# WangFeng18/3d-gaussian-splatting

Measured on NVIDIA H100. Metric: render+backward FPS @1080p (2.4M Gaussians), higher is better.
Workload: dtype f32

## Files before the change

3d-gaussian-splatting_b200/csrc/bindings.cpp:

```cpp
#include <ATen/cuda/CUDAContext.h>
#include <c10/cuda/CUDACachingAllocator.h>
#include <c10/cuda/CUDAGuard.h>
#include <torch/extension.h>

#include <string>
#include <vector>

#include "../../include/gs_b200.h"

namespace gsb200 {

#define GS_CHECK_F32(x)                                                                         \
  TORCH_CHECK((x).is_cuda(), #x " must be a CUDA tensor");                                      \
  TORCH_CHECK((x).is_contiguous(), #x " must be contiguous");                                   \
  TORCH_CHECK((x).scalar_type() == at::kFloat, #x " must be float32")
#define GS_CHECK_I32(x)                                                                         \
  TORCH_CHECK((x).is_cuda(), #x " must be a CUDA tensor");                                      \
  TORCH_CHECK((x).is_contiguous(), #x " must be contiguous");                                   \
  TORCH_CHECK((x).scalar_type() == at::kInt, #x " must be int32")
#define GS_CHECK_I64(x)                                                                         \
  TORCH_CHECK((x).is_cuda(), #x " must be a CUDA tensor");                                      \
  TORCH_CHECK((x).is_contiguous(), #x " must be contiguous");                                   \
  TORCH_CHECK((x).scalar_type() == at::kLong, #x " must be int64")

// ... 463 lines not shown
      GS_CHECK_F32(*g_pos); GS_CHECK_F32(*g_rgb); GS_CHECK_F32(*g_opa); GS_CHECK_F32(*g_quat); GS_CHECK_F32(*g_scale);
      TORCH_CHECK(g_pos->numel() == pos.numel() && g_rgb->numel() == rgb.numel() && g_opa->numel() == opa.numel() &&
                      g_quat->numel() == quat.numel() && g_scale->numel() == scale.numel(),
                  "RenderContext.backward_cam_into: gradient buffers must match their parameters");
      TORCH_CHECK(reinterpret_cast<uintptr_t>(g_quat->data_ptr()) % 16 == 0, "grad_quat must be 16-byte aligned");
    }
    auto opt = [](std::optional<torch::Tensor>& t) { return t ? fpm(*t) : nullptr; };
    c10::cuda::CUDAGuard guard(pos.device());
    auto gi = grad_image.contiguous();
    torch::Tensor ga;
    if (grad_aux) ga = grad_aux->contiguous();
    check_rc(gs_render_backward_cam(ctx, fp(pos), fp(rgb), fp(opa), fp(quat), fp(scale), fp(raw), fp(gi),
                                    grad_is_final ? 1 : 0, aux ? fp(*aux) : nullptr, grad_aux ? fp(ga) : nullptr, opt(g_pos),
                                    opt(g_rgb), opt(g_opa), opt(g_quat), opt(g_scale), fpm(grad_cam), cur_stream()),
             "gs_render_backward_cam");
  }

  int64_t last_instances() { return (int64_t)gs_frame_instances(ctx); }

  py::dict stats() {
    gs_frame_info fi{};
    check_rc(gs_frame_stats(ctx, &fi, cur_stream()), "gs_frame_stats");
    py::dict d;
    d["n_gaussians"] = fi.n_gaussians;
    d["n_visible"] = fi.n_visible;
    d["n_instances"] = fi.n_instances;
    d["n_instances_eff"] = fi.n_instances_eff;
    d["width_padded"] = fi.width_padded;
    d["height_padded"] = fi.height_padded;
    d["n_tiles"] = fi.n_tiles;
    d["max_tile_count"] = fi.max_tile_count;
    d["n_instances_eff_bwd"] = fi.n_instances_eff_bwd;
    return d;
  }

  std::tuple<torch::Tensor, torch::Tensor> sorted_instances() {
    gs_frame_info fi{};
    check_rc(gs_frame_stats(ctx, &fi, cur_stream()), "gs_frame_stats");
    auto opts = torch::TensorOptions().device(torch::kCUDA, device).dtype(at::kInt);
    auto idx = torch::empty({(int64_t)fi.n_instances}, opts);
    auto accum = torch::empty({(int64_t)fi.n_tiles + 1}, opts);
    check_rc(gs_frame_sorted(ctx, idx.data_ptr<int>(), fi.n_instances, accum.data_ptr<int>(), cur_stream()),
             "gs_frame_sorted");
    return {idx, accum};
  }

  torch::Tensor tile_consumed() {
    gs_frame_info fi{};
    check_rc(gs_frame_stats(ctx, &fi, cur_stream()), "gs_frame_stats");
    auto out = torch::empty({(int64_t)fi.n_tiles}, torch::TensorOptions().device(torch::kCUDA, device).dtype(at::kInt));
    check_rc(gs_frame_tile_consumed(ctx, out.data_ptr<int>(), cur_stream()), "gs_frame_tile_consumed");
    return out;
  }
};

void adam_step(torch::Tensor param, torch::Tensor grad, torch::Tensor exp_avg, torch::Tensor exp_avg_sq,
               std::vector<int64_t> seg_ends, std::vector<double> lrs, double beta1, double beta2, double eps,
               int64_t step) {
  GS_CHECK_F32(param); GS_CHECK_F32(grad); GS_CHECK_F32(exp_avg); GS_CHECK_F32(exp_avg_sq);
  int64_t n = param.numel();
  TORCH_CHECK(grad.numel() == n && exp_avg.numel() == n && exp_avg_sq.numel() == n, "adam_step: size mismatch");
  TORCH_CHECK(seg_ends.size() == lrs.size() && !seg_ends.empty() && seg_ends.back() == n,
              "adam_step: segments must cover the flat buffer");
  for (auto* t : {&param, &grad, &exp_avg, &exp_avg_sq})
    TORCH_CHECK(reinterpret_cast<uintptr_t>(t->data_ptr()) % 16 == 0, "adam_step: buffers must be 16-byte aligned");
  std::vector<long long> ends(seg_ends.begin(), seg_ends.end());
  std::vector<float> lr(lrs.begin(), lrs.end());
  c10::cuda::CUDAGuard guard(param.device());
  check_rc(gs_adam_step(fpm(param), fp(grad), fpm(exp_avg), fpm(exp_avg_sq), n, ends.data(), lr.data(), (int)ends.size(),
                        (float)beta1, (float)beta2, (float)eps, (int)step, cur_stream()),
           "gs_adam_step");
}

std::tuple<torch::Tensor, torch::Tensor> loss_l1_ssim(torch::Tensor image, torch::Tensor target, double w_l1,
                                                      double w_ssim, double bias, bool want_grad) {
  GS_CHECK_F32(image);
  TORCH_CHECK(target.is_cuda() && target.is_contiguous() &&
                  (target.scalar_type() == at::kFloat || target.scalar_type() == at::kHalf),
              "loss_l1_ssim: target must be a contiguous float32 / float16 CUDA tensor");
  TORCH_CHECK(image.dim() == 3 && image.size(2) == 3 && target.sizes() == image.sizes(),
              "loss_l1_ssim: image and target must both be [H, W, 3]");
  TORCH_CHECK(image.size(0) > 10 && image.size(1) > 10, "loss_l1_ssim: the image must be larger than the 11x11 window");
  c10::cuda::CUDAGuard guard(image.device());
  const int h = (int)image.size(0), w = (int)image.size(1);
  auto ws = torch::empty({(int64_t)gs_loss_workspace_bytes(h, w)}, image.options().dtype(at::kByte));
  auto out3 = torch::empty({3}, image.options());
  torch::Tensor grad = want_grad ? torch::empty_like(image) : torch::Tensor();
  check_rc(gs_loss_l1_ssim(fp(image), target.data_ptr(), target.scalar_type() == at::kHalf ? 1 : 0, h, w, (float)w_l1,
                           (float)w_ssim, (float)bias, want_grad ? fpm(grad) : nullptr, fpm(out3), ws.data_ptr(),
                           (size_t)ws.numel(), cur_stream()),
           "gs_loss_l1_ssim");
  return {out3, grad};
}

std::tuple<std::vector<torch::Tensor>, std::vector<int64_t>> densify(
    torch::Tensor pos, torch::Tensor rgb, torch::Tensor opa, torch::Tensor quat, torch::Tensor scale, torch::Tensor grad,
    int scale_activation, double opa_logit_min, double delete_thresh, double grad_thresh, bool grad_agg_max, double tau,
    bool use_clone, bool use_split, double clone_dt, c10::optional<at::Generator> gen) {
  GS_CHECK_F32(pos); GS_CHECK_F32(rgb); GS_CHECK_F32(opa); GS_CHECK_F32(quat); GS_CHECK_F32(scale); GS_CHECK_F32(grad);
  const int64_t n = pos.size(0);
  TORCH_CHECK(pos.dim() == 2 && pos.size(1) == 3 && rgb.dim() == 2 && rgb.size(0) == n && opa.numel() == n &&
                  quat.numel() == 4 * n && scale.numel() == 3 * n && grad.numel() == 3 * n && n < (int64_t(1) << 31),
              "densify: bad shapes");
  c10::cuda::CUDAGuard guard(pos.device());
  auto bopt = pos.options().dtype(at::kByte);
  auto code = torch::empty({n + 1}, bopt);
// ... 76 lines not shown
      .def_readwrite("left", &TilesPy::left)
      .def_readwrite("right", &TilesPy::right);

  py::class_<Gaussian3dsPy>(m, "Gaussian3ds")
      .def(py::init<>())
      .def_readwrite("pos", &Gaussian3dsPy::pos)
      .def_readwrite("rgb", &Gaussian3dsPy::rgb)
      .def_readwrite("opa", &Gaussian3dsPy::opa)
      .def_readwrite("quat", &Gaussian3dsPy::quat)
      .def_readwrite("scale", &Gaussian3dsPy::scale)
      .def_readwrite("cov", &Gaussian3dsPy::cov);

  m.def("calc_tile_list", &calc_tile_list, "calc tile list (CUDA)");
  m.def("gather_gaussians", &gather_gaussians, "gather gaussian (CUDA)");
  m.def("draw", &draw, "draw (CUDA)");
  m.def("draw_backward", &draw_backward, "draw backward (CUDA)");
  m.def("global_culling", &global_culling, "global culling (CUDA)");
  m.def("global_culling_backward", &global_culling_backward, "global culling backward (CUDA)");

  py::class_<RenderContext>(m, "RenderContext")
      .def(py::init<>())
      .def("forward", &RenderContext::forward)
      .def("backward", &RenderContext::backward)
      .def("backward_into", &RenderContext::backward_into, py::arg("pos"), py::arg("rgb"), py::arg("opa"),
           py::arg("quat"), py::arg("scale"), py::arg("image"), py::arg("grad_image"), py::arg("g_pos"),
           py::arg("g_rgb"), py::arg("g_opa"), py::arg("g_quat"), py::arg("g_scale"), py::arg("expected_frame") = -1)
      .def("forward_final", &RenderContext::forward_final)
      .def("backward_final_into", &RenderContext::backward_final_into, py::arg("pos"), py::arg("rgb"),
           py::arg("opa"), py::arg("quat"), py::arg("scale"), py::arg("raw"), py::arg("grad_final"),
           py::arg("g_pos"), py::arg("g_rgb"), py::arg("g_opa"), py::arg("g_quat"), py::arg("g_scale"),
           py::arg("expected_frame") = -1)
      .def("forward_aux", &RenderContext::forward_aux, py::arg("pos"), py::arg("rgb"), py::arg("opa"), py::arg("quat"),
           py::arg("scale"), py::arg("width"), py::arg("height"), py::arg("fx"), py::arg("fy"), py::arg("rot"),
           py::arg("tran"), py::arg("near"), py::arg("thresh"), py::arg("scale_activation"),
           py::arg("background") = py::none(), py::arg("final") = true)
      .def("backward_aux_into", &RenderContext::backward_aux_into, py::arg("pos"), py::arg("rgb"), py::arg("opa"),
           py::arg("quat"), py::arg("scale"), py::arg("raw"), py::arg("grad_image"), py::arg("grad_is_final"),
           py::arg("aux"), py::arg("grad_aux"), py::arg("g_pos"), py::arg("g_rgb"), py::arg("g_opa"),
           py::arg("g_quat"), py::arg("g_scale"), py::arg("expected_frame") = -1)
      .def("backward_cam_into", &RenderContext::backward_cam_into, py::arg("pos"), py::arg("rgb"), py::arg("opa"),
           py::arg("quat"), py::arg("scale"), py::arg("raw"), py::arg("grad_image"), py::arg("grad_is_final"),
           py::arg("aux"), py::arg("grad_aux"), py::arg("g_pos"), py::arg("g_rgb"), py::arg("g_opa"),
           py::arg("g_quat"), py::arg("g_scale"), py::arg("grad_cam"), py::arg("expected_frame") = -1)
      .def("frame_id", &RenderContext::frame_id)
      .def("last_instances", &RenderContext::last_instances)
      .def("stats", &RenderContext::stats)
      .def("set_sh_eval", &RenderContext::set_sh_eval, py::arg("mode"))
      .def("set_filter2d", &RenderContext::set_filter2d, py::arg("mode"), py::arg("variance") = 0.3)
      .def("set_timing", &RenderContext::set_timing)
      .def("set_grad_push", &RenderContext::set_grad_push)
      .def("clear_grad_push", &RenderContext::clear_grad_push)
      .def("stage_ms", &RenderContext::stage_ms)
      .def("sorted_instances", &RenderContext::sorted_instances)
      .def("tile_consumed", &RenderContext::tile_consumed);
  m.def("allreduce_push_finish", &allreduce_push_finish, "second half of the pushed gradient exchange");
  m.def("allreduce_push_finish_mc", &allreduce_push_finish_mc,
        "second half of the pushed gradient exchange, broadcast through the NVSwitch (multimem.st)");
  m.def("allreduce_p2p", &allreduce_p2p, "peer-to-peer two-shot in-place all-reduce of a symmetric buffer");
  m.def("allreduce_multimem", &allreduce_multimem, "NVLS multimem in-place all-reduce of a symmetric buffer");
  m.def("densify", &densify, "prune / clone / split on the device (reference splatter.py:122-228)", py::arg("pos"),
        py::arg("rgb"), py::arg("opa"), py::arg("quat"), py::arg("scale"), py::arg("grad"), py::arg("scale_activation"),
        py::arg("opa_logit_min"), py::arg("delete_thresh"), py::arg("grad_thresh"), py::arg("grad_agg_max"), py::arg("tau"),
        py::arg("use_clone"), py::arg("use_split"), py::arg("clone_dt"), py::arg("generator") = py::none());
  m.def("loss_l1_ssim", &loss_l1_ssim, "fused L1 + SSIM loss, forward + image gradient (CUDA)");
  m.def("adam_step", &adam_step, "fused Adam over flat parameter / gradient buffers (CUDA)");
  m.def("tune", [](const std::string& name, int value) { check_rc(gs_tune(name.c_str(), value), "gs_tune"); },
        "set an A/B tuning knob of the blend kernels (see include/gs_b200.h gs_tune)");
  m.def("kernel_launches", []() { return (int64_t)gs_kernel_launches(); },
        "kernels of libgs_b200 launched by this process so far");
  m.attr("abi_version") = gs_abi_version();
  m.attr("SH_EVAL_PIXEL") = GS_SH_EVAL_PIXEL;
  m.attr("SH_EVAL_GAUSSIAN") = GS_SH_EVAL_GAUSSIAN;
  m.attr("FILTER2D_NONE") = GS_FILTER2D_NONE;
  m.attr("FILTER2D_DILATE") = GS_FILTER2D_DILATE;
  m.attr("FILTER2D_ANTIALIAS") = GS_FILTER2D_ANTIALIAS;
}
```

3d-gaussian-splatting_b200/csrc/binning.cu:

```cuda
#include "internal.h"

namespace {

constexpr int kBlock = 256;

__device__ __forceinline__ void append_to_tile(int* tile_n_point, int* list, int max_per_tile, uint32_t tid,
                                               uint32_t pid) {
  int old = atomicAdd(tile_n_point + tid, 1);
  if (old < max_per_tile) list[(size_t)max_per_tile * tid + old] = (int)pid;
}

__global__ void tile_list_dist_kernel(const float* __restrict__ pos, const float* __restrict__ top,
                                      const float* __restrict__ bottom, const float* __restrict__ left,
                                      const float* __restrict__ right, int* tile_n_point, int* list, uint32_t n,
                                      uint32_t n_tiles, int max_per_tile, float thresh) {
  uint32_t pid = blockDim.x * blockIdx.x + threadIdx.x;
  uint32_t tid = blockDim.y * blockIdx.y + threadIdx.y;
  if (pid >= n || tid >= n_tiles) return;
  float cy = (top[tid] + bottom[tid]) / 2;
  float cx = (left[tid] + right[tid]) / 2;
  float d1 = pos[3 * pid] - cx, d2 = pos[3 * pid + 1] - cy;
  if (d1 * d1 + d2 * d2 < thresh) append_to_tile(tile_n_point, list, max_per_tile, tid, pid);
}

// ... 132 lines not shown
  const long long t = (long long)blockIdx.x * kBlock + threadIdx.x;
  const long long i = t >> 3;
  const int sub = (int)(t & 7);
  if (i >= m) return;
  const uint32_t tile = keys[i];
  const uint32_t g = vals[i];
  if (sub == 0) {
    if (i == 0) {
      for (uint32_t tt = 0; tt <= tile; ++tt) tile_accum[tt] = 0;
    } else {
      uint32_t prev = keys[i - 1];
      for (uint32_t tt = prev + 1; tt <= tile; ++tt) tile_accum[tt] = (int)i;
    }
    if (i == m - 1)
      for (uint32_t tt = tile + 1; tt <= (uint32_t)n_tiles; ++tt) tile_accum[tt] = (int)m;
    const GsRec* r = rec + g;
    float4 a = r->a, b = r->b, c = r->c;
    uint32_t rxy = __float_as_uint(c.z), rwh = __float_as_uint(c.w);
    uint32_t tx = tile % ntx, ty = tile / ntx;
    uint32_t slot = offsets_g[g] + (ty - (rxy >> 16)) * (rwh & 0xffffu) + (tx - (rxy & 0xffffu));
    pA[i] = a;
    pB[i] = make_float2(b.x, b.y);
    pS[(size_t)i * sw + d] = __uint_as_float(slot);
  }
  float* row = pS + (size_t)i * sw;
  const float* src = rgb + (size_t)g * d;
  for (int q = sub; q < d; q += 8) row[q] = src[q];
}

template <typename KeyT>
__global__ void __launch_bounds__(kBlock) tile_ranges_kernel(const KeyT* __restrict__ keys, long long m, int n_tiles,
                                                              int* __restrict__ tile_accum) {
  const long long i0 = ((long long)blockIdx.x * kBlock + threadIdx.x) * 8;
  if (i0 >= m) return;
  uint32_t prev = i0 > 0 ? (uint32_t)keys[i0 - 1] : 0u;
  if (i0 == 0) tile_accum[0] = 0;
#pragma unroll
  for (int u = 0; u < 8; ++u) {
    const long long i = i0 + u;
    if (i >= m) break;
    const uint32_t tile = keys[i];
    for (uint32_t t = prev + 1; t <= tile; ++t) tile_accum[t] = (int)i;
    if (i == 0)
      for (uint32_t t = 1; t <= tile; ++t) tile_accum[t] = 0;
    prev = tile;
    if (i == m - 1)
      for (uint32_t t = tile + 1; t <= (uint32_t)n_tiles; ++t) tile_accum[t] = (int)m;
  }
}

__global__ void __launch_bounds__(kBlock) iota_kernel(uint32_t* out, int n) {
  int i = blockIdx.x * kBlock + threadIdx.x;
  if (i < n) out[i] = (uint32_t)i;
}

}

cudaError_t gs_launch_pack_sorted_sh(const void* keys, int key_bytes, const uint32_t* vals, long long m, int n_tiles,
                                     int ntx, const GsRec* rec, const uint32_t* offsets_g, const float* rgb, int d,
                                     int sw, float4* pA, float2* pB, float* pS, int* tile_accum, cudaStream_t st) {
  if (m == 0) return cudaMemsetAsync(tile_accum, 0, sizeof(int) * (size_t)(n_tiles + 1), st);
  const unsigned grid = (unsigned)((m * 8 + kBlock - 1) / kBlock);
  if (key_bytes == 2)
    pack_sorted_sh_kernel<uint16_t><<<grid, kBlock, 0, st>>>(static_cast<const uint16_t*>(keys), vals, m, n_tiles,
                                                             ntx, rec, offsets_g, rgb, d, sw, pA, pB, pS, tile_accum);
  else
    pack_sorted_sh_kernel<uint32_t><<<grid, kBlock, 0, st>>>(static_cast<const uint32_t*>(keys), vals, m, n_tiles,
                                                             ntx, rec, offsets_g, rgb, d, sw, pA, pB, pS, tile_accum);
  return cudaGetLastError();
}

cudaError_t gs_launch_iota(uint32_t* out, int n, cudaStream_t st) {
  if (n == 0) return cudaSuccess;
  iota_kernel<<<(n + kBlock - 1) / kBlock, kBlock, 0, st>>>(out, n);
  return cudaGetLastError();
}

extern "C" int gs_tile_list(const float* pos, const float* cov, int n, const float* tile_top,
                            const float* tile_bottom, const float* tile_left, const float* tile_right, int n_tiles,
                            int* tile_n_point, int* tile_gaussian_list, int max_per_tile, float thresh, int method,
                            float tile_length_x, float tile_length_y, int n_tiles_x, int n_tiles_y, float leftmost,
                            float topmost, gs_stream_t stream) {
  if (n < 0 || n_tiles < 0 || max_per_tile < 0) return gs_set_error_msg(GS_ERR_INVALID_ARG, "gs_tile_list: negative size");
  if (n == 0 || n_tiles == 0) return 0;
  cudaStream_t st = (cudaStream_t)stream;
  if (method == 0 || method == 1) {
    dim3 block(32, 8), grid((n + 31) / 32, (n_tiles + 7) / 8);
    if (grid.y > 65535) return gs_set_error_msg(GS_ERR_INVALID_ARG, "gs_tile_list: too many tiles for method 0/1");
    if (method == 0)
      tile_list_dist_kernel<<<grid, block, 0, st>>>(pos, tile_top, tile_bottom, tile_left, tile_right, tile_n_point,
                                                    tile_gaussian_list, n, n_tiles, max_per_tile, thresh);
    else
      tile_list_prob_kernel<<<grid, block, 0, st>>>(pos, cov, tile_top, tile_bottom, tile_left, tile_right,
                                                    tile_n_point, tile_gaussian_list, n, n_tiles, max_per_tile,
                                                    thresh);
  } else {
    GsTileGrid g;
    g.lx = tile_length_x;
    g.ly = tile_length_y;
    g.leftmost = leftmost;
    g.topmost = topmost;
    g.t2 = 0.f;
    g.ntx = n_tiles_x;
    g.nty = n_tiles_y;
    tile_list_prob2_kernel<<<(n + kBlock - 1) / kBlock, kBlock, 0, st>>>(pos, cov, g, tile_n_point,
                                                                        tile_gaussian_list, n, max_per_tile, thresh);
// ... 3 lines not shown
  return 0;
}

extern "C" int gs_gather(const int* tile_n_point_accum, const int* tile_gaussian_list, int n_tiles, int list_stride,
                         int max_points_for_tile, int* gathered_list, int* tile_ids_for_points,
                         gs_stream_t stream) {
  (void)max_points_for_tile;
  if (n_tiles < 0) return gs_set_error_msg(GS_ERR_INVALID_ARG, "gs_gather: n_tiles < 0");
  if (n_tiles == 0) return 0;
  int warps = kBlock / 32;
  gather_kernel<<<(n_tiles + warps - 1) / warps, kBlock, 0, (cudaStream_t)stream>>>(
      tile_n_point_accum, tile_gaussian_list, n_tiles, list_stride, gathered_list, tile_ids_for_points);
  GS_CUDA_TRY(cudaGetLastError());
  gs_count_launch();
  return 0;
}

cudaError_t gs_launch_emit_keys(const GsRec* rec, const uint32_t* perm, const uint32_t* offsets_sorted, int n, int ntx,
                                void* keys, int key_bytes, uint32_t* vals, cudaStream_t st) {
  if (n == 0) return cudaSuccess;
  if (key_bytes == 2)
    emit_keys_kernel<uint16_t><<<(n + kBlock - 1) / kBlock, kBlock, 0, st>>>(rec, perm, offsets_sorted, n, ntx,
                                                                             static_cast<uint16_t*>(keys), vals);
  else
    emit_keys_kernel<uint32_t><<<(n + kBlock - 1) / kBlock, kBlock, 0, st>>>(rec, perm, offsets_sorted, n, ntx,
                                                                             static_cast<uint32_t*>(keys), vals);
  return cudaGetLastError();
}

cudaError_t gs_launch_tile_ranges(const void* keys, int key_bytes, long long m, int n_tiles, int* tile_accum,
                                  cudaStream_t st) {
  if (m == 0) return cudaMemsetAsync(tile_accum, 0, sizeof(int) * (size_t)(n_tiles + 1), st);
  const unsigned grid = (unsigned)((m + 8LL * kBlock - 1) / (8LL * kBlock));
  if (key_bytes == 2)
    tile_ranges_kernel<uint16_t><<<grid, kBlock, 0, st>>>(static_cast<const uint16_t*>(keys), m, n_tiles, tile_accum);
  else
    tile_ranges_kernel<uint32_t><<<grid, kBlock, 0, st>>>(static_cast<const uint32_t*>(keys), m, n_tiles, tile_accum);
  return cudaGetLastError();
}

cudaError_t gs_launch_pack_sorted(const void* keys, int key_bytes, const uint32_t* vals, long long m, int n_tiles,
                                  int ntx, const GsRec* rec, const uint32_t* offsets_g, float4* pA, float2* pB,
                                  float4* pC, int* tile_accum, cudaStream_t st) {
  if (m == 0) return cudaMemsetAsync(tile_accum, 0, sizeof(int) * (size_t)(n_tiles + 1), st);
  const unsigned grid = (unsigned)((m + kBlock - 1) / kBlock);
  if (key_bytes == 2)
    pack_sorted_kernel<uint16_t><<<grid, kBlock, 0, st>>>(static_cast<const uint16_t*>(keys), vals, m, n_tiles, ntx,
                                                          rec, offsets_g, pA, pB, pC, tile_accum);
  else
    pack_sorted_kernel<uint32_t><<<grid, kBlock, 0, st>>>(static_cast<const uint32_t*>(keys), vals, m, n_tiles, ntx,
                                                          rec, offsets_g, pA, pB, pC, tile_accum);
  return cudaGetLastError();
}
```

3d-gaussian-splatting_b200/csrc/blend.cu:

```cuda
#include <cstdlib>
#include <type_traits>

#include "internal.h"

namespace {

constexpr int FWD_THREADS = 64;
constexpr int FWD_PX = 4;
constexpr int FWD_STAGES = 2;

template <int FWD_CH>
struct FwdSmem {
  float4 A[FWD_STAGES][FWD_CH];
  float4 C[FWD_STAGES][FWD_CH];
  float2 B[FWD_STAGES][FWD_CH + 2];
  uint64_t full[FWD_STAGES];
};

template <typename SM, int CH>
__device__ __forceinline__ void issue_chunk(SM& sm, int stage, const float4* __restrict__ pA,
                                            const float2* __restrict__ pB, const float4* __restrict__ pC,
                                            int base, int n, int shift) {
  uint32_t bytes_a = (uint32_t)n * 16u;
  uint32_t nb = (uint32_t)(n + shift + 1) & ~1u;
// ... 37 lines not shown
    return off + ((uint32_t)ty - (rxy >> 16)) * (rwh & 0xffffu) + ((uint32_t)tx - (rxy & 0xffffu));
  }
};

template <int CH, int STAGES, int RECW>
struct GatherRing {
  float4 rec[STAGES][CH * RECW];
  uint64_t full[STAGES];
};

template <int NT, int CH>
struct GatherIds {
  uint32_t id[(CH + NT - 1) / NT];
  __device__ __forceinline__ void load(const uint32_t* __restrict__ ids, int base, int n, int tid) {
#pragma unroll
    for (int u = 0; u < (CH + NT - 1) / NT; ++u) {
      const int i = tid + u * NT;
      id[u] = i < n ? __ldg(ids + base + i) : 0u;
    }
  }
};

template <typename SM, int NT, int CH, int RECW>
__device__ __forceinline__ void gather_issue(SM& sm, int stage, const GsRec* __restrict__ grec,
                                             const uint32_t* __restrict__ goff, const GatherIds<NT, CH>& g, int n,
                                             int tid) {
#pragma unroll
  for (int u = 0; u < (CH + NT - 1) / NT; ++u) {
    const int i = tid + u * NT;
    if (i < n) {
      const float4* src = reinterpret_cast<const float4*>(grec + g.id[u]);
      const uint32_t dst = gs_smem_u32(&sm.rec[stage][i * RECW]);
#pragma unroll
      for (int q = 0; q < 3; ++q)
        asm volatile("cp.async.cg.shared.global [%0], [%1], 16;" ::"r"(dst + 16u * q), "l"(src + q) : "memory");
      if (RECW == 4)
        asm volatile("cp.async.ca.shared.global [%0], [%1], 4;" ::"r"(dst + 48u), "l"(goff + g.id[u]) : "memory");
    }
  }
  asm volatile("cp.async.mbarrier.arrive.noinc.shared::cta.b64 [%0];" ::"r"(gs_smem_u32(&sm.full[stage])) : "memory");
}

template <int FWD_CH, int PX, bool GATHER, bool AUX = false>
__global__ void __launch_bounds__(256 / PX) blend_fwd_kernel(const float4* __restrict__ pA,
                                                                 const float2* __restrict__ pB,
                                                                 const float4* __restrict__ pC,
                                                                 const GsRec* __restrict__ grec,
                                                                 const uint32_t* __restrict__ ids,
                                                                 const int* __restrict__ tile_accum, int wp, int hp,
                                                                 int ntx, float fx, float fy,
                                                                 float* __restrict__ image,
                                                                 int* __restrict__ tile_neff,
                                                                 float* __restrict__ final_img, GsCrop crop,
                                                                 GsAuxOut aux) {
  static_assert(!AUX || GATHER, "the aux outputs read |p_c| from the gathered records");
  using Smem = typename std::conditional<GATHER, GatherRing<FWD_CH, FWD_STAGES, 3>, FwdSmem<FWD_CH>>::type;
  __shared__ __align__(16) Smem sm;
  const int tile = blockIdx.x;
  const int tid = threadIdx.x;
  const int tx = tile % ntx, ty = tile / ntx;
  constexpr int FWD_PX = PX, TPR = GS_TILE / PX, NTHREADS = 256 / PX;
  const int ix0 = tx * GS_TILE + (tid % TPR) * FWD_PX;
  const int iy = ty * GS_TILE + (tid / TPR);
  float px[FWD_PX];
#pragma unroll
  for (int p = 0; p < FWD_PX; ++p) px[p] = gs_pixel_coord(ix0 + p, wp, fx);
  const float py = gs_pixel_coord(iy, hp, fy);

  const int start = tile_accum[tile];
  const int cnt = tile_accum[tile + 1] - start;
  const int shift = start & 1;
  const int nchunks = (cnt + FWD_CH - 1) / FWD_CH;

  if (tid == 0) {
    for (int s = 0; s < FWD_STAGES; ++s) gs_mbar_init(&sm.full[s], GATHER ? NTHREADS : 1);
    gs_fence_barrier_init();
  }
  __syncthreads();
  GatherIds<NTHREADS, FWD_CH> gid;
  if constexpr (GATHER) {
    for (int k = 0; k < FWD_STAGES && k < nchunks; ++k) {
      gid.load(ids, start + k * FWD_CH, min(FWD_CH, cnt - k * FWD_CH), tid);
      gather_issue<Smem, NTHREADS, FWD_CH, 3>(sm, k, grec, nullptr, gid, min(FWD_CH, cnt - k * FWD_CH), tid);
    }
    if (FWD_STAGES < nchunks) gid.load(ids, start + FWD_STAGES * FWD_CH, min(FWD_CH, cnt - FWD_STAGES * FWD_CH), tid);
  } else if (tid == 0) {
    for (int k = 0; k < FWD_STAGES && k < nchunks; ++k)
      issue_chunk<Smem, FWD_CH>(sm, k, pA, pB, pC, start + k * FWD_CH, min(FWD_CH, cnt - k * FWD_CH), shift);
  }

  float T[FWD_PX], cr[FWD_PX], cg[FWD_PX], cb[FWD_PX], dep[FWD_PX];
#pragma unroll
  for (int p = 0; p < FWD_PX; ++p) {
    T[p] = 1.f;
    cr[p] = cg[p] = cb[p] = 0.f;
    dep[p] = 0.f;
  }
  int consumed = cnt;
  int k = 0;
  for (; k < nchunks; ++k) {
    const int stage = k % FWD_STAGES;
    gs_mbar_wait(&sm.full[stage], (uint32_t)((k / FWD_STAGES) & 1));
    const int n = min(FWD_CH, cnt - k * FWD_CH);
    StageView<GATHER> sv;
    if constexpr (GATHER) {
      sv.R = sm.rec[stage];
      sv.recw = 3;
    } else {
      sv.A = sm.A[stage];
      sv.C = sm.C[stage];
      sv.B = sm.B[stage] + shift;
// ... 79 lines not shown
      for (int q = 0; q < FWD_PX / 2; ++q) o[q] = make_float4(ab[4 * q], ab[4 * q + 1], ab[4 * q + 2], ab[4 * q + 3]);
    }
    if (aux.aux_final) {
#pragma unroll
      for (int p = 0; p < FWD_PX; ++p) {
        const int x = ix0 + p - crop.left, y = iy - crop.top;
        if (x >= 0 && x < crop.width && y >= 0 && y < crop.height)
          *reinterpret_cast<float2*>(aux.aux_final + ((size_t)y * crop.width + x) * 2) = make_float2(ab[2 * p], ab[2 * p + 1]);
      }
    }
  }
  {
    float ob[FWD_PX * 3];
#pragma unroll
    for (int p = 0; p < FWD_PX; ++p) {
      ob[3 * p] = cr[p];
      ob[3 * p + 1] = cg[p];
      ob[3 * p + 2] = cb[p];
    }
    float4* o = reinterpret_cast<float4*>(image + ((size_t)iy * wp + ix0) * 3);
#pragma unroll
    for (int q = 0; q < FWD_PX * 3 / 4; ++q) o[q] = make_float4(ob[4 * q], ob[4 * q + 1], ob[4 * q + 2], ob[4 * q + 3]);
  }
  if (final_img) {
#pragma unroll
    for (int p = 0; p < FWD_PX; ++p)
      gs_store_final(final_img, ix0 + p, iy, crop.left, crop.top, crop.width, crop.height, cr[p], cg[p], cb[p]);
  }
  if (tile_neff && tid == 0) tile_neff[tile] = consumed;
}

constexpr int BWD_STAGES = 2;
constexpr int BWD_NV = 9;

template <int WARPS, int BWD_CH>
struct BwdSmem {
  float4 A[BWD_STAGES][BWD_CH];
  float4 C[BWD_STAGES][BWD_CH];
  float2 B[BWD_STAGES][BWD_CH + 2];
  uint64_t full[BWD_STAGES];
  float partial[WARPS][BWD_CH * BWD_NV];
};

template <int WARPS, int BWD_CH>
__global__ void __launch_bounds__(32 * WARPS) blend_bwd_kernel(const float4* __restrict__ pA,
                                                                const float2* __restrict__ pB,
                                                                const float4* __restrict__ pC,
                                                                const int* __restrict__ tile_accum, int wp, int hp,
                                                                int ntx, float fx, float fy,
                                                                const float* __restrict__ image,
                                                                const float* __restrict__ grad_image,
                                                                float* __restrict__ grad_inst, int grad_is_final,
                                                                GsCrop crop, uint32_t* __restrict__ row_epoch,
                                                                uint32_t epoch, int* __restrict__ tile_neff_b) {
  constexpr int THREADS = 32 * WARPS;
  constexpr int PX = 256 / THREADS;
  constexpr int TPR = GS_TILE / PX;
  using Smem = BwdSmem<WARPS, BWD_CH>;
  __shared__ __align__(16) Smem sm;
  const int tile = blockIdx.x;
  const int tid = threadIdx.x, warp = tid >> 5, lane = tid & 31;
  const int tx = tile % ntx, ty = tile / ntx;
  const int start = tile_accum[tile];
  const int cnt = tile_accum[tile + 1] - start;
  if (cnt == 0) return;
  const int shift = start & 1;
  const int nchunks = (cnt + BWD_CH - 1) / BWD_CH;

  const int ix0 = tx * GS_TILE + (tid % TPR) * PX;
  const int iy = ty * GS_TILE + (tid / TPR);
  float px[PX];
#pragma unroll
  for (int p = 0; p < PX; ++p) px[p] = gs_pixel_coord(ix0 + p, wp, fx);
  const float py = gs_pixel_coord(iy, hp, fy);

  float T[PX], R[PX], gr[PX], gg[PX], gb[PX];
  {
    const size_t off = ((size_t)iy * wp + ix0) * 3;
    const float4* im = reinterpret_cast<const float4*>(image + off);
    float gbuf[PX * 3], ibuf[PX * 3];
#pragma unroll
    for (int q = 0; q < PX * 3 / 4; ++q) {
      const float4 i4 = im[q];
      ibuf[4 * q] = i4.x; ibuf[4 * q + 1] = i4.y; ibuf[4 * q + 2] = i4.z; ibuf[4 * q + 3] = i4.w;
    }
    if (!grad_is_final) {
      const float4* gi = reinterpret_cast<const float4*>(grad_image + off);
#pragma unroll
      for (int q = 0; q < PX * 3 / 4; ++q) {
        const float4 g4 = gi[q];
        gbuf[4 * q] = g4.x; gbuf[4 * q + 1] = g4.y; gbuf[4 * q + 2] = g4.z; gbuf[4 * q + 3] = g4.w;
      }
    } else {
#pragma unroll
      for (int p = 0; p < PX; ++p)
        gs_load_final_grad(grad_image, ibuf + 3 * p, ix0 + p, iy, crop.left, crop.top, crop.width, crop.height,
                           gbuf[3 * p], gbuf[3 * p + 1], gbuf[3 * p + 2]);
    }
#pragma unroll
    for (int p = 0; p < PX; ++p) {
      gr[p] = gbuf[3 * p];
      gg[p] = gbuf[3 * p + 1];
      gb[p] = gbuf[3 * p + 2];
      R[p] = gr[p] * ibuf[3 * p] + gg[p] * ibuf[3 * p + 1] + gb[p] * ibuf[3 * p + 2];
      T[p] = 1.f;
    }
  }

  if (tid == 0) {
    for (int s = 0; s < BWD_STAGES; ++s) gs_mbar_init(&sm.full[s], 1);
    gs_fence_barrier_init();
  }
  __syncthreads();
// ... 141 lines not shown
}

constexpr int WS_CH = 64;

template <int STAGES>
struct WsRing {
  float4 A[STAGES][WS_CH];
  float4 C[STAGES][WS_CH];
  float2 B[STAGES][WS_CH + 2];
  uint64_t full[STAGES], empty[STAGES], done;
  volatile int stop, consumed_chunks;
};

template <typename SM, int STAGES>
__device__ __forceinline__ void ws_init(SM& sm, int tid) {
  if (tid == 0) {
    for (int s = 0; s < STAGES; ++s) {
      gs_mbar_init(&sm.full[s], 1);
      gs_mbar_init(&sm.empty[s], 1);
    }
    gs_mbar_init(&sm.done, 1);
    sm.stop = 0;
    sm.consumed_chunks = 0;
    gs_fence_barrier_init();
  }
  __syncthreads();
}

template <typename SM, int STAGES>
__device__ __forceinline__ void ws_producer(SM& sm, const float4* __restrict__ pA, const float2* __restrict__ pB,
                                            const float4* __restrict__ pC, int start, int cnt, int nchunks) {
  const int shift = start & 1;
  int k = 0;
  for (; k < nchunks; ++k) {
    const int s = k % STAGES;
    if (k >= STAGES) gs_mbar_wait(&sm.empty[s], (uint32_t)(((k / STAGES) - 1) & 1));
    if (sm.stop) break;
    issue_chunk<SM, WS_CH>(sm, s, pA, pB, pC, start + k * WS_CH, min(WS_CH, cnt - k * WS_CH), shift);
  }
  gs_mbar_wait(&sm.done, 0u);
  for (int kk = sm.consumed_chunks; kk < k; ++kk) gs_mbar_wait(&sm.full[kk % STAGES], (uint32_t)((kk / STAGES) & 1));
}

constexpr int WSF_STAGES = 4;
constexpr int WSF_CONS = 64;

__global__ void __launch_bounds__(WSF_CONS + 32) blend_fwd_ws_kernel(const float4* __restrict__ pA,
                                                                      const float2* __restrict__ pB,
                                                                      const float4* __restrict__ pC,
                                                                      const int* __restrict__ tile_accum, int wp,
                                                                      int hp, int ntx, float fx, float fy,
                                                                      float* __restrict__ image,
                                                                      int* __restrict__ tile_neff,
                                                                      float* __restrict__ final_img, GsCrop crop) {
  using Smem = WsRing<WSF_STAGES>;
  __shared__ __align__(16) Smem sm;
  const int tile = blockIdx.x;
  const int tid = threadIdx.x;
  const int start = tile_accum[tile];
  const int cnt = tile_accum[tile + 1] - start;
  const int nchunks = (cnt + WS_CH - 1) / WS_CH;
  ws_init<Smem, WSF_STAGES>(sm, tid);
  if (tid >= WSF_CONS) {
    if (tid == WSF_CONS && nchunks > 0) ws_producer<Smem, WSF_STAGES>(sm, pA, pB, pC, start, cnt, nchunks);
    return;
  }
  const int tx = tile % ntx, ty = tile / ntx;
  const int ix0 = tx * GS_TILE + (tid & 3) * FWD_PX;
  const int iy = ty * GS_TILE + (tid >> 2);
  float px[FWD_PX];
#pragma unroll
  for (int p = 0; p < FWD_PX; ++p) px[p] = gs_pixel_coord(ix0 + p, wp, fx);
  const float py = gs_pixel_coord(iy, hp, fy);
  const int shift = start & 1;

  float T[FWD_PX], cr[FWD_PX], cg[FWD_PX], cb[FWD_PX];
#pragma unroll
  for (int p = 0; p < FWD_PX; ++p) {
    T[p] = 1.f;
    cr[p] = cg[p] = cb[p] = 0.f;
  }
  int consumed = cnt;
  for (int k = 0; k < nchunks; ++k) {
    const int stage = k % WSF_STAGES;
    gs_mbar_wait(&sm.full[stage], (uint32_t)((k / WSF_STAGES) & 1));
    const int n = min(WS_CH, cnt - k * WS_CH);
    const float4* __restrict__ sA = sm.A[stage];
    const float4* __restrict__ sC = sm.C[stage];
    const float2* __restrict__ sB = sm.B[stage] + shift;
#define GS_FWD_BODY(J)                                                                      \
  {                                                                                         \
    const float4 a = sA[J];                                                                 \
    const float2 b = sB[J];                                                                 \
    const float4 c = sC[J];                                                                 \
    const float dy = py - a.y;                                                              \
    const float m1 = a.w * dy;                                                              \
    const float ev = fmaf(-b.x * dy, dy, b.y);                                              \
    _Pragma("unroll") for (int p = 0; p < FWD_PX; ++p) {                                    \
      const float dx = px[p] - a.x;                                                         \
      const float eu = fmaf(a.z, dx, -m1);                                                  \
      const float alpha = gs_ex2(fmaf(-dx, eu, ev));                                        \
      const float w = (T[p] > GS_T_STOP) ? alpha * T[p] : 0.f;                              \
      cr[p] = fmaf(c.x, w, cr[p]);                                                          \
      cg[p] = fmaf(c.y, w, cg[p]);                                                          \
      cb[p] = fmaf(c.z, w, cb[p]);                                                          \
      T[p] -= w;                                                                            \
    }                                                                                       \
  }
    int j = 0;
    bool warp_dead = false;
// ... 160 lines not shown
    }
  lsrc[lane] = 0;
  lcnt[lane] = 0;
  lrow[lane] = GS_TILE;
  lpy[lane] = 0.f;
  const int nl = (live + ns - 1) / ns;
  int sc = (nl << 16) | live;
#pragma unroll
  for (int o = 1; o < 32; o <<= 1) {
    const int t = __shfl_up_sync(0xffffffffu, sc, o);
    if (lane >= o) sc += t;
  }
  sc -= (nl << 16) | live;
  __syncwarp();
  for (int q = 0; q < nl; ++q) {
    const int l = (sc >> 16) + q;
    lsrc[l] = (sc & 0xffff) + q * ns;
    lcnt[l] = min(ns, live - q * ns);
    lrow[l] = lane;
    lpy[l] = pyt[lane];
  }
  __syncwarp();
  const int src = lsrc[lane], n = lcnt[lane];
  prow = lrow[lane];
  py = lpy[lane];
#pragma unroll
  for (int p = 0; p < PX; ++p) {
    const bool v = p < n;
    px[p] = v ? st[src + p] : 0.f;
    T[p] = v ? st[256 + src + p] : 0.f;
    Rr[p] = v ? st[512 + src + p] : 0.f;
    gr[p] = v ? st[768 + src + p] : 0.f;
    gg[p] = v ? st[1024 + src + p] : 0.f;
    gb[p] = v ? st[1280 + src + p] : 0.f;
    if constexpr (AUX) {
      gD[p] = v ? st[1536 + src + p] : 0.f;
      gA[p] = v ? st[1792 + src + p] : 0.f;
    }
  }
  __syncwarp();
  st[bwd_lane_y<SQ, QS>(lane)] = py;
  S = ns;
}

template <int PX, bool WS, int UNR, int STAGES, int MINB, int RQ, bool GATHER, int CH, bool AUX = false,
          bool REPACK = false>
__global__ void __launch_bounds__(256 / PX + (WS ? 32 : 0), MINB)
    blend_bwd2_kernel(const float4* __restrict__ pA, const float2* __restrict__ pB, const float4* __restrict__ pC,
                      const GsRec* __restrict__ grec, const uint32_t* __restrict__ ids,
                      const uint32_t* __restrict__ goff, const int* __restrict__ tile_accum, int wp, int hp, int ntx, float fx, float fy,
                      const float* __restrict__ image, const float* __restrict__ grad_image,
                      float* __restrict__ grad_inst, int grad_is_final, GsCrop crop, uint32_t* __restrict__ row_epoch,
                      uint32_t epoch, int* __restrict__ tile_neff_b, const float* __restrict__ aux,
                      const float* __restrict__ grad_aux) {
  using Cfg = Bwd2Cfg<PX, STAGES, RQ>;
  constexpr int NT = Cfg::NT, TPR = Cfg::TPR, R = Cfg::R, SQ = Cfg::SQ, QS = Cfg::QS, IS = Cfg::IS, ROWS = Cfg::ROWS;
  static_assert(IS % 2 == 0 && QS % 2 == 0 && IS % 32 == 2 && QS % 32 == 32 / RQ, "partial buffer strides");
  static_assert(!(WS && GATHER), "the gather path issues its copies from all consumer threads");
  static_assert(GATHER || CH == WS_CH, "the packed ring is sized for CH instances per stage");
  static_assert(!AUX || GATHER, "the aux terms read |p_c| from the gathered records");
  static_assert(!REPACK || (NT == 32 && PX == 8), "the repack deals one warp's 256 pixels into slots of at most 8");
  static_assert(!REPACK || R * IS >= RP_END, "the partial buffer holds the repack's planes and tables");
  using Smem = typename std::conditional<AUX, Bwd2SmemAux<PX, STAGES, RQ, GATHER, CH>,
                                         Bwd2Smem<PX, STAGES, RQ, GATHER, CH>>::type;
  __shared__ __align__(16) Smem sm;
  const int tile = blockIdx.x;
  const int tid = threadIdx.x, warp = tid >> 5, lane = tid & 31;
  const int start = tile_accum[tile];
  const int cnt = tile_accum[tile + 1] - start;
  if (cnt == 0) return;
  const int nchunks = (cnt + CH - 1) / CH;
  const int tx = tile % ntx, ty = tile / ntx;
  const int shift = start & 1;
  if (tid < GS_TILE) sm.pyt[tid] = gs_pixel_coord(ty * GS_TILE + tid, hp, fy);
  if constexpr (GATHER) {
    if (tid == 0) {
      for (int s = 0; s < STAGES; ++s) gs_mbar_init(&sm.full[s], NT);
      gs_fence_barrier_init();
    }
    __syncthreads();
  } else {
    ws_init<Smem, STAGES>(sm, tid);
    if (WS) {
      if (tid >= NT) {
        if (tid == NT) ws_producer<Smem, STAGES>(sm, pA, pB, pC, start, cnt, nchunks);
        return;
      }
    } else if (tid == 0) {
      for (int k = 0; k < STAGES && k < nchunks; ++k)
        issue_chunk<Smem, CH>(sm, k, pA, pB, pC, start + k * CH, min(CH, cnt - k * CH), shift);
    }
  }
  GatherIds<NT, CH> gid;
  if constexpr (GATHER) {
    for (int k = 0; k < STAGES && k < nchunks; ++k) {
      gid.load(ids, start + k * CH, min(CH, cnt - k * CH), tid);
      gather_issue<Smem, NT, CH, 4>(sm, k, grec, goff, gid, min(CH, cnt - k * CH), tid);
    }
    if (STAGES < nchunks) gid.load(ids, start + STAGES * CH, min(CH, cnt - STAGES * CH), tid);
  }
  const int ix0 = tx * GS_TILE + (tid % TPR) * PX;
  const int iy = ty * GS_TILE + (tid / TPR);
  float px[PX];
#pragma unroll
  for (int p = 0; p < PX; ++p) px[p] = gs_pixel_coord(ix0 + p, wp, fx);
  float py = sm.pyt[tid / TPR];
  int S = PX, prow = tid / TPR;

  float T[PX], Rr[PX], gr[PX], gg[PX], gb[PX];
  {
    const size_t off = ((size_t)iy * wp + ix0) * 3;
    const float4* im = reinterpret_cast<const float4*>(image + off);
    float gbuf[PX * 3], ibuf[PX * 3];
#pragma unroll
    for (int q = 0; q < PX * 3 / 4; ++q) {
      const float4 i4 = im[q];
      ibuf[4 * q] = i4.x; ibuf[4 * q + 1] = i4.y; ibuf[4 * q + 2] = i4.z; ibuf[4 * q + 3] = i4.w;
    }
    if (!grad_is_final) {
// ... 332 lines not shown
  int i = blockIdx.x * 256 + threadIdx.x;
  if (i >= m) return;
  const float* row = grad_inst + (size_t)i * gw;
  float4 cv = reinterpret_cast<const float4*>(cov)[i];
  float det = cv.x * cv.w - cv.y * cv.z;
  double pn = 2.0 * (double)det + 1e-14;
  float sc = (float)((double)GS_LOG2E / pn);
  float kk = 2.f * sc * sc / GS_LOG2E;
  float d_ca = row[2], d_cb = row[3], d_cc = row[4];
  float gsc = d_ca * cv.w + d_cb * (cv.y + cv.z) + d_cc * cv.x;
  g_pos[3 * i] = row[0];
  g_pos[3 * i + 1] = row[1];
  reinterpret_cast<float4*>(g_cov)[i] = make_float4(d_cc * sc - gsc * kk * cv.w, d_cb * sc + gsc * kk * cv.z,
                                                    d_cb * sc + gsc * kk * cv.y, d_ca * sc - gsc * kk * cv.x);
  g_opa[i] = opa[i] > 0.f ? row[5] / (opa[i] * GS_LN2) : 0.f;
  for (int q = 0; q < d; ++q) g_rgb[(size_t)i * d + q] = row[6 + q];
}

struct LegacyWs {
  float4* pA;
  float2* pB;
  float4* pC;
  float* grad_inst;
};

inline size_t align_up(size_t x, size_t a) { return (x + a - 1) / a * a; }

inline size_t legacy_ws_layout(int m, int d, LegacyWs* ws, char* base) {
  size_t off = 0;
  size_t mm = (size_t)(m > 0 ? m : 0);
  size_t crow = d == 3 ? 16 : (size_t)gs_sh_stream_width(d) * 4;
  size_t grow = d == 3 ? (size_t)GS_GREC * 4 : (size_t)gs_sh_grad_width(d) * 4;
  if (ws) ws->pA = reinterpret_cast<float4*>(base + off);
  off += align_up(mm * 16, 256);
  if (ws) ws->pC = reinterpret_cast<float4*>(base + off);
  off += align_up(mm * crow + 16, 256);
  if (ws) ws->pB = reinterpret_cast<float2*>(base + off);
  off += align_up((mm + 2) * 8, 256);
  if (ws) ws->grad_inst = reinterpret_cast<float*>(base + off);
  off += align_up(mm * grow, 256);
  return off;
}

}

cudaError_t gs_launch_blend_fwd(const float4* pA, const float2* pB, const float4* pC, const GsRec* grec,
                                const uint32_t* ids, const int* tile_accum, const GsFrameGeom& g, float* image,
                                int* tile_neff, float* final_img, const GsCrop& crop, cudaStream_t st,
                                const GsAuxOut* aux) {
  const GsTuning& tn = gs_tuning();
  const bool gather = grec != nullptr;
  if (aux) {
    blend_fwd_kernel<128, 4, true, true><<<g.n_tiles, 64, 0, st>>>(pA, pB, pC, grec, ids, tile_accum, g.wp, g.hp, g.ntx,
                                                                  g.fx, g.fy, image, tile_neff, final_img, crop, *aux);
    return cudaGetLastError();
  }
  if (!gather && tn.fwd_kernel != 0) {
    blend_fwd_ws_kernel<<<g.n_tiles, WSF_CONS + 32, 0, st>>>(pA, pB, pC, tile_accum, g.wp, g.hp, g.ntx, g.fx, g.fy, image,
                                                             tile_neff, final_img, crop);
    return cudaGetLastError();
  }
  const int ch = tn.fwd_ch;
#define GS_FWD_LAUNCH(CH, PX, GA)                                                                                   \
  blend_fwd_kernel<CH, PX, GA><<<g.n_tiles, 256 / PX, 0, st>>>(pA, pB, pC, grec, ids, tile_accum, g.wp, g.hp, g.ntx, \
                                                               g.fx, g.fy, image, tile_neff, final_img, crop, GsAuxOut{})
#define GS_FWD_CH(PX, GA)                     \
  if (ch == 64) GS_FWD_LAUNCH(64, PX, GA);    \
  else if (ch == 256) GS_FWD_LAUNCH(256, PX, GA); \
  else GS_FWD_LAUNCH(128, PX, GA)
  if (gather) {
    if (tn.fwd_px == 8) { GS_FWD_CH(8, true); } else { GS_FWD_CH(4, true); }
  } else {
    if (tn.fwd_px == 8) { GS_FWD_CH(8, false); } else { GS_FWD_CH(4, false); }
  }
#undef GS_FWD_CH
#undef GS_FWD_LAUNCH
  return cudaGetLastError();
}

cudaError_t gs_launch_blend_bwd(const float4* pA, const float2* pB, const float4* pC, const GsRec* grec,
                                const uint32_t* ids, const uint32_t* goff, const int* tile_accum, const GsFrameGeom& g,
                                const float* image,
                                const float* grad_image, float* grad_inst, int grad_is_final, const GsCrop& crop,
                                uint32_t* row_epoch, uint32_t epoch, int* tile_neff_b, cudaStream_t st,
                                const float* aux, const float* grad_aux) {
  const GsTuning& tn = gs_tuning();
  const bool gather = grec != nullptr;
  if (gather && !row_epoch) return cudaErrorInvalidValue;
  if (grad_aux) {
    if (!gather || !aux) return cudaErrorInvalidValue;
#define GS_BWD2_AUX(RP)                                                                                            \
  blend_bwd2_kernel<8, false, 4, 3, 10, 4, true, 32, true, RP><<<g.n_tiles, 32, 0, st>>>(                           \
      pA, pB, pC, grec, ids, goff, tile_accum, g.wp, g.hp, g.ntx, g.fx, g.fy, image, grad_image, grad_inst,         \
      grad_is_final, crop, row_epoch, epoch, tile_neff_b, aux, grad_aux)
    if (tn.blend_repack) GS_BWD2_AUX(true);
    else GS_BWD2_AUX(false);
#undef GS_BWD2_AUX
    return cudaGetLastError();
  }
  if (tn.bwd_kernel != 0 || gather) {
#define GS_BWD2C(PX, WS, UNR, ST, MINB, RQ, GA, CH)                                                                 \
  blend_bwd2_kernel<PX, WS, UNR, ST, MINB, RQ, GA, CH><<<g.n_tiles, 256 / PX + (WS ? 32 : 0), 0, st>>>(              \
      pA, pB, pC, grec, ids, goff, tile_accum, g.wp, g.hp, g.ntx, g.fx, g.fy, image, grad_image, grad_inst,          \
      grad_is_final,                                                                                                 \
      crop, row_epoch, epoch, tile_neff_b, nullptr, nullptr)
#define GS_BWD2(PX, WS, UNR, ST, MINB, RQ, GA) GS_BWD2C(PX, WS, UNR, ST, MINB, RQ, GA, 64)
    const int key = ((((tn.bwd_px * 10 + tn.bwd_ws) * 10 + tn.bwd_unroll) * 10 + tn.bwd_stages) * 10 + tn.bwd_rq) * 100 +
                    tn.bwd_minb;
    if (gather && tn.bwd_ch == 32) {
#define GS_BWD2_SHIPPED()                                                                                          \
  if (tn.blend_repack)                                                                                             \
    blend_bwd2_kernel<8, false, 4, 3, 10, 4, true, 32, false, true><<<g.n_tiles, 32, 0, st>>>(                      \
        pA, pB, pC, grec, ids, goff, tile_accum, g.wp, g.hp, g.ntx, g.fx, g.fy, image, grad_image, grad_inst,       \
        grad_is_final, crop, row_epoch, epoch, tile_neff_b, nullptr, nullptr);                                     \
  else                                                                                                             \
    GS_BWD2C(8, false, 4, 3, 10, 4, true, 32)
      switch (key) {
        case 8022416: GS_BWD2C(8, false, 2, 2, 16, 4, true, 32); break;
        case 8023416: GS_BWD2C(8, false, 2, 3, 16, 4, true, 32); break;
        case 8042410: GS_BWD2C(8, false, 4, 2, 10, 4, true, 32); break;
        case 8043410: GS_BWD2_SHIPPED(); break;
        default:
          if (gs_tuning().strict) return cudaErrorInvalidValue;
          GS_BWD2_SHIPPED();
          break;
      }
#undef GS_BWD2_SHIPPED
      return cudaGetLastError();
    }
    if (gather) {
      switch (key) {
        case 8012410: GS_BWD2(8, false, 1, 2, 10, 4, true); break;
        case 8022416: GS_BWD2(8, false, 2, 2, 16, 4, true); break;
        case 8022410: GS_BWD2(8, false, 2, 2, 10, 4, true); break;
        case 8042410: GS_BWD2(8, false, 4, 2, 10, 4, true); break;
        case 8023416: GS_BWD2(8, false, 2, 3, 16, 4, true); break;
        case 8012416: GS_BWD2(8, false, 1, 2, 16, 4, true); break;
        case 8012420: GS_BWD2(8, false, 1, 2, 20, 4, true); break;
        case 8012820: GS_BWD2(8, false, 1, 2, 20, 8, true); break;
        case 8013416: GS_BWD2(8, false, 1, 3, 16, 4, true); break;
        case 4012401: GS_BWD2(4, false, 1, 2, 1, 4, true); break;
        case 4042401: GS_BWD2(4, false, 4, 2, 1, 4, true); break;
        default: return gs_tuning().strict ? cudaErrorInvalidValue : (GS_BWD2(8, false, 2, 2, 16, 4, true), cudaGetLastError());
      }
      return cudaGetLastError();
    }
    switch (key) {
      case 4113401: GS_BWD2(4, true, 1, 3, 1, 4, false); break;
      case 4143408: GS_BWD2(4, true, 4, 3, 8, 4, false); break;
      case 4012401: GS_BWD2(4, false, 1, 2, 1, 4, false); break;
      case 4042401: GS_BWD2(4, false, 4, 2, 1, 4, false); break;
      case 4042810: GS_BWD2(4, false, 4, 2, 10, 8, false); break;
      case 8012410: GS_BWD2(8, false, 1, 2, 10, 4, false); break;
      case 8012416: GS_BWD2(8, false, 1, 2, 16, 4, false); break;
      case 8012420: GS_BWD2(8, false, 1, 2, 20, 4, false); break;
      case 8013416: GS_BWD2(8, false, 1, 3, 16, 4, false); break;
      case 8022416: GS_BWD2(8, false, 2, 2, 16, 4, false); break;
      case 8022410: GS_BWD2(8, false, 2, 2, 10, 4, false); break;
      case 8042410: GS_BWD2(8, false, 4, 2, 10, 4, false); break;
      case 8012816: GS_BWD2(8, false, 1, 2, 16, 8, false); break;
      case 8012820: GS_BWD2(8, false, 1, 2, 20, 8, false); break;
      case 8112410: GS_BWD2(8, true, 1, 2, 10, 4, false); break;
      case 8012424: GS_BWD2(8, false, 1, 2, 24, 4, false); break;
      case 8012824: GS_BWD2(8, false, 1, 2, 24, 8, false); break;
      default: return gs_tuning().strict ? cudaErrorInvalidValue : (GS_BWD2(8, false, 2, 2, 16, 4, false), cudaGetLastError());
    }
#undef GS_BWD2
#undef GS_BWD2C
    return cudaGetLastError();
  }
  const int warps = tn.bwd_px == 8 ? 1 : 2;
  const int ch = 64;
#define GS_BWD_LAUNCH(W, CH)                                                                                         \
  blend_bwd_kernel<W, CH><<<g.n_tiles, 32 * W, 0, st>>>(pA, pB, pC, tile_accum, g.wp, g.hp, g.ntx, g.fx, g.fy, image, \
                                                        grad_image, grad_inst, grad_is_final, crop, row_epoch, epoch, \
                                                        tile_neff_b)
  if (warps == 1) GS_BWD_LAUNCH(1, 64);
  else if (ch == 32) GS_BWD_LAUNCH(2, 32);
  else if (ch == 128) GS_BWD_LAUNCH(2, 128);
  else GS_BWD_LAUNCH(2, 64);
#undef GS_BWD_LAUNCH
  return cudaGetLastError();
}

int gs_blend_aux_supported(int d, bool forward, bool backward) {
  const GsTuning& tn = gs_tuning();
  if (!tn.gather)
    return gs_set_error_msg(GS_ERR_UNSUPPORTED, "depth / alpha / background: the packed path (gs_tune(\"gather\", 0)) has no aux kernel");
  if (d != 3) {
    if (backward && (gs_sh_tc_mode(d) & 6) == 6)
      return gs_set_error_msg(GS_ERR_UNSUPPORTED,
                              "depth / alpha gradients: the two-pixel tensor-core SH backward (sh_tc bit 2) has no aux kernel");
    return 0;
  }
  if (forward && (tn.fwd_kernel != 0 || tn.fwd_ch != 128 || tn.fwd_px != 4))
    return gs_set_error_msg(GS_ERR_UNSUPPORTED,
                            "depth / alpha / background: only the shipped forward blend knobs (fwd_kernel 0, fwd_ch 128, fwd_px 4) have an aux kernel");
  if (backward && (tn.bwd_kernel == 0 || tn.bwd_px != 8 || tn.bwd_ws != 0 || tn.bwd_unroll != 4 || tn.bwd_stages != 3 ||
                   tn.bwd_rq != 4 || tn.bwd_minb != 10 || tn.bwd_ch != 32))
    return gs_set_error_msg(GS_ERR_UNSUPPORTED,
                            "depth / alpha gradients: only the shipped backward blend knobs have an aux kernel");
  return 0;
}

extern "C" size_t gs_draw_workspace_bytes(int m, int d) {
  if (d != 3 && gs_sh_basis_count(d) == 0) return 0;
  return legacy_ws_layout(m, d, nullptr, nullptr);
}

static int check_draw_args(const char* fn, int m, int d, int wp, int hp, int weight_normalize, int sigmoid,
                           size_t ws_bytes, void* ws) {
  if (m < 0 || wp <= 0 || hp <= 0 || (wp % GS_TILE) || (hp % GS_TILE))
    return gs_set_error_msg(GS_ERR_INVALID_ARG, fn);
  if (weight_normalize || sigmoid || (d != 3 && gs_sh_basis_count(d) == 0)) return gs_set_error_msg(GS_ERR_UNSUPPORTED, fn);
  if (m > 0 && (ws == nullptr || ws_bytes < gs_draw_workspace_bytes(m, d)))
    return gs_set_error_msg(GS_ERR_INVALID_ARG, fn);
  return 0;
}

extern "C" int gs_draw_fwd(const float* pos, const float* rgb, const float* opa, const float* cov,
                           const int* tile_n_point_accum, int m, int d, int width_padded, int height_padded,
                           float focal_x, float focal_y, int weight_normalize, int sigmoid, const float* rays_o,
                           const float* lefttop, const float* vec_dx, const float* vec_dy, float* image,
                           void* workspace, size_t workspace_bytes, gs_stream_t stream) {
  int rc = check_draw_args("gs_draw_fwd: bad/unsupported arguments", m, d, width_padded, height_padded,
                           weight_normalize, sigmoid, workspace_bytes, workspace);
  if (rc) return rc;
  if (d != 3 && (!rays_o || !lefttop || !vec_dx || !vec_dy))
    return gs_set_error_msg(GS_ERR_INVALID_ARG, "gs_draw_fwd: SH colour needs rays_o / lefttop / vec_dx / vec_dy");
// ... 83 lines not shown
```

3d-gaussian-splatting_b200/csrc/blend_sh.cu:

```cuda
#include <type_traits>

#include "internal.h"
#include "sh_common.cuh"

namespace {

using namespace gs_sh;

template <int K, int CH, int STAGES>
struct ShStage {
  float4 A[STAGES][CH];
  float2 B[STAGES][CH + 2];
  float S[STAGES][CH * sh_sw(K)];
  uint64_t full[STAGES];
};

template <int K, typename SM>
__device__ __forceinline__ void issue_sh(SM& sm, int stage, const float4* __restrict__ pA,
                                         const float2* __restrict__ pB, const float* __restrict__ pS, int base,
                                         int n, int shift) {
  const uint32_t bytes_a = (uint32_t)n * 16u;
  const uint32_t bytes_s = (uint32_t)n * (uint32_t)(sh_sw(K) * 4);
  const uint32_t nb = (uint32_t)(n + shift + 1) & ~1u;
  const uint32_t bytes_b = nb * 8u;
// ... 30 lines not shown
      for (int q = 0; q < D / 4; ++q)
        asm volatile("cp.async.cg.shared.global [%0], [%1], 16;" ::"r"(ds + 16u * q), "l"(src + 4 * q) : "memory");
    } else {
#pragma unroll
      for (int q = 0; q < D; ++q)
        asm volatile("cp.async.ca.shared.global [%0], [%1], 4;" ::"r"(ds + 4u * q), "l"(src + q) : "memory");
    }
  }
  asm volatile("cp.async.mbarrier.arrive.noinc.shared::cta.b64 [%0];" ::"r"(gs_smem_u32(&sm.full[stage])) : "memory");
}

template <int K, bool GATHER>
struct ShView;
template <int K>
struct ShView<K, false> {
  const float4* A;
  const float2* B;
  const float* S;
  __device__ __forceinline__ float4 a(int j) const { return A[j]; }
  __device__ __forceinline__ float2 b(int j) const { return B[j]; }
  __device__ __forceinline__ const float* coef(int j) const { return S + j * sh_sw(K); }
  __device__ __forceinline__ uint32_t slot(int j, int, int) const { return __float_as_uint(S[j * sh_sw(K) + 3 * K]); }
};
template <int K>
struct ShView<K, true> {
  const float4* R;
  const float* S;
  __device__ __forceinline__ float4 a(int j) const { return R[4 * j]; }
  __device__ __forceinline__ float2 b(int j) const {
    const float4 t = R[4 * j + 1];
    return make_float2(t.x, t.y);
  }
  __device__ __forceinline__ const float* coef(int j) const { return S + j * sh_sw(K); }
  __device__ __forceinline__ float depth(int j) const { return R[4 * j + 2].y; }
  __device__ __forceinline__ uint32_t slot(int j, int tx, int ty) const {
    const float4 cc = R[4 * j + 2];
    const uint32_t rxy = __float_as_uint(cc.z), rwh = __float_as_uint(cc.w);
    return __float_as_uint(R[4 * j + 3].x) + ((uint32_t)ty - (rxy >> 16)) * (rwh & 0xffffu) + ((uint32_t)tx - (rxy & 0xffffu));
  }
};

template <int K, bool GATHER, bool AUX = false>
__global__ void __launch_bounds__(64) blend_sh_fwd_kernel(const float4* __restrict__ pA, const float2* __restrict__ pB,
                                                           const float* __restrict__ pS,
                                                           const GsRec* __restrict__ grec, const float* __restrict__ rgb,
                                                           const uint32_t* __restrict__ ids,
                                                           const uint32_t* __restrict__ goff,
                                                           const int* __restrict__ tile_accum, int wp, int hp, int ntx,
                                                           float fx, float fy, const float* __restrict__ rays_o,
                                                           const float* __restrict__ lefttop,
                                                           const float* __restrict__ vdx,
                                                           const float* __restrict__ vdy, float* __restrict__ image,
                                                           int* __restrict__ tile_neff,
                                                           float* __restrict__ final_img, GsCrop crop, GsAuxOut aux) {
  constexpr int CH = 64, STAGES = 2, PX = 4, SW = sh_sw(K), NT = 64;
  static_assert(!AUX || GATHER, "the aux outputs read |p_c| from the gathered records");
  using SM = typename std::conditional<GATHER, ShGatherStage<K, CH, STAGES>, ShStage<K, CH, STAGES>>::type;
  __shared__ __align__(16) SM sm;
  const int tile = blockIdx.x, tid = threadIdx.x;
  const int tx = tile % ntx, ty = tile / ntx;
  const int ix0 = tx * GS_TILE + (tid & 3) * PX;
  const int iy = ty * GS_TILE + (tid >> 2);
  float px[PX], sh[PX][K];
#pragma unroll
  for (int p = 0; p < PX; ++p) {
    px[p] = gs_pixel_coord(ix0 + p, wp, fx);
    pixel_sh<K>(ix0 + p, iy, rays_o, lefttop, vdx, vdy, sh[p]);
  }
  const float py = gs_pixel_coord(iy, hp, fy);
  const int start = tile_accum[tile];
  const int cnt = tile_accum[tile + 1] - start;
  const int shift = start & 1;
  const int nchunks = (cnt + CH - 1) / CH;
  if (tid == 0) {
    for (int s = 0; s < STAGES; ++s) gs_mbar_init(&sm.full[s], GATHER ? NT : 1);
    gs_fence_barrier_init();
  }
  __syncthreads();
  if constexpr (GATHER) {
    for (int k = 0; k < STAGES && k < nchunks; ++k)
      issue_sh_gather<K, NT>(sm, k, grec, rgb, ids, goff, start + k * CH, min(CH, cnt - k * CH), tid);
  } else if (tid == 0) {
    for (int k = 0; k < STAGES && k < nchunks; ++k)
      issue_sh<K>(sm, k, pA, pB, pS, start + k * CH, min(CH, cnt - k * CH), shift);
  }

  float T[PX], cr[PX], cg[PX], cb[PX], dep[PX];
#pragma unroll
  for (int p = 0; p < PX; ++p) {
    T[p] = 1.f;
    cr[p] = cg[p] = cb[p] = 0.f;
    dep[p] = 0.f;
  }
  int consumed = cnt, k = 0;
  for (; k < nchunks; ++k) {
    const int stage = k % STAGES;
    gs_mbar_wait(&sm.full[stage], (uint32_t)((k / STAGES) & 1));
    const int n = min(CH, cnt - k * CH);
    ShView<K, GATHER> sv;
    if constexpr (GATHER) {
      sv.R = sm.R[stage];
    } else {
      sv.A = sm.A[stage];
      sv.B = sm.B[stage] + shift;
    }
    sv.S = sm.S[stage];
    for (int j = 0; j < n; ++j) {
      if ((j & 3) == 0) {
        const bool dead = !(T[0] > GS_T_STOP) && !(T[1] > GS_T_STOP) && !(T[2] > GS_T_STOP) && !(T[3] > GS_T_STOP);
        if (__all_sync(0xffffffffu, dead)) break;
      }
      const float4 a = sv.a(j);
// ... 57 lines not shown
      if constexpr (GATHER)
        issue_sh_gather<K, NT>(sm, stage, grec, rgb, ids, goff, start + kn * CH, min(CH, cnt - kn * CH), tid);
      else if (tid == 0)
        issue_sh<K>(sm, stage, pA, pB, pS, start + kn * CH, min(CH, cnt - kn * CH), shift);
    }
  }
  if (tid == 0 && k < nchunks)
    for (int kk = k + 1; kk < nchunks && kk < k + STAGES; ++kk)
      gs_mbar_wait(&sm.full[kk % STAGES], (uint32_t)((kk / STAGES) & 1));
  if constexpr (AUX) {
#pragma unroll
    for (int p = 0; p < PX; ++p) {
      cr[p] = fmaf(T[p], aux.bg[0], cr[p]);
      cg[p] = fmaf(T[p], aux.bg[1], cg[p]);
      cb[p] = fmaf(T[p], aux.bg[2], cb[p]);
      gs_store_aux(aux, ix0 + p, iy, wp, crop, dep[p], 1.f - T[p]);
    }
  }
  float4* o = reinterpret_cast<float4*>(image + ((size_t)iy * wp + ix0) * 3);
  o[0] = make_float4(cr[0], cg[0], cb[0], cr[1]);
  o[1] = make_float4(cg[1], cb[1], cr[2], cg[2]);
  o[2] = make_float4(cb[2], cr[3], cg[3], cb[3]);
  if (final_img) {
#pragma unroll
    for (int p = 0; p < PX; ++p)
      gs_store_final(final_img, ix0 + p, iy, crop.left, crop.top, crop.width, crop.height, cr[p], cg[p], cb[p]);
  }
  if (tile_neff && tid == 0) tile_neff[tile] = consumed;
}

template <int K, bool GATHER>
struct ShBwdSmem {
  typename std::conditional<GATHER, ShGatherStage<K, 32, 2>, ShStage<K, 32, 2>>::type st;
  float partial[2][32 * sh_nvp(K)];
};

template <int K, bool GATHER, bool AUX = false>
__global__ void __launch_bounds__(64) blend_sh_bwd_kernel(const float4* __restrict__ pA, const float2* __restrict__ pB,
                                                           const float* __restrict__ pS,
                                                           const GsRec* __restrict__ grec, const float* __restrict__ rgb,
                                                           const uint32_t* __restrict__ ids,
                                                           const uint32_t* __restrict__ goff,
                                                           const int* __restrict__ tile_accum, int wp, int hp, int ntx,
                                                           float fx, float fy, const float* __restrict__ rays_o,
                                                           const float* __restrict__ lefttop,
                                                           const float* __restrict__ vdx,
                                                           const float* __restrict__ vdy,
                                                           const float* __restrict__ image,
                                                           const float* __restrict__ grad_image,
                                                           float* __restrict__ grad_inst, int grad_is_final,
                                                           GsCrop crop, uint32_t* __restrict__ row_epoch,
                                                           uint32_t epoch, int* __restrict__ tile_neff_b,
                                                           const float* __restrict__ aux,
                                                           const float* __restrict__ grad_aux) {
  constexpr int CH = 32, STAGES = 2, PX = 4, SW = sh_sw(K), NV = sh_nv(K), NVP = sh_nvp(K), THREADS = 64;
  constexpr int GREC = (NV + 3) / 4 * 4;
  static_assert(!AUX || (GATHER && NV < NVP && NV < GREC), "d_t needs a pad slot in the partial and gradient rows");
  __shared__ __align__(16) ShBwdSmem<K, GATHER> smem;
  auto& sm = smem.st;
  const int tile = blockIdx.x, tid = threadIdx.x, warp = tid >> 5, lane = tid & 31;
  const int tx = tile % ntx, ty = tile / ntx;
  const int start = tile_accum[tile];
  const int cnt = tile_accum[tile + 1] - start;
  if (cnt == 0) return;
  const int shift = start & 1;
  const int nchunks = (cnt + CH - 1) / CH;
  const int ix0 = tx * GS_TILE + (tid & 3) * PX;
  const int iy = ty * GS_TILE + (tid >> 2);
  float px[PX], sh[PX][K];
#pragma unroll
  for (int p = 0; p < PX; ++p) {
    px[p] = gs_pixel_coord(ix0 + p, wp, fx);
    pixel_sh<K>(ix0 + p, iy, rays_o, lefttop, vdx, vdy, sh[p]);
  }
  const float py = gs_pixel_coord(iy, hp, fy);
  float T[PX], R[PX], gr[PX], gg[PX], gb[PX];
  {
    const size_t off = ((size_t)iy * wp + ix0) * 3;
    const float4* im = reinterpret_cast<const float4*>(image + off);
    const float4 i0 = im[0], i1 = im[1], i2 = im[2];
    if (!grad_is_final) {
      const float4* gi = reinterpret_cast<const float4*>(grad_image + off);
      const float4 g0 = gi[0], g1 = gi[1], g2 = gi[2];
      gr[0] = g0.x; gg[0] = g0.y; gb[0] = g0.z; gr[1] = g0.w;
      gg[1] = g1.x; gb[1] = g1.y; gr[2] = g1.z; gg[2] = g1.w;
      gb[2] = g2.x; gr[3] = g2.y; gg[3] = g2.z; gb[3] = g2.w;
    } else {
      const float raw[12] = {i0.x, i0.y, i0.z, i0.w, i1.x, i1.y, i1.z, i1.w, i2.x, i2.y, i2.z, i2.w};
#pragma unroll
      for (int p = 0; p < PX; ++p)
        gs_load_final_grad(grad_image, raw + 3 * p, ix0 + p, iy, crop.left, crop.top, crop.width, crop.height, gr[p],
                           gg[p], gb[p]);
    }
    R[0] = gr[0] * i0.x + gg[0] * i0.y + gb[0] * i0.z;
    R[1] = gr[1] * i0.w + gg[1] * i1.x + gb[1] * i1.y;
    R[2] = gr[2] * i1.z + gg[2] * i1.w + gb[2] * i2.x;
    R[3] = gr[3] * i2.y + gg[3] * i2.z + gb[3] * i2.w;
#pragma unroll
    for (int p = 0; p < PX; ++p) T[p] = 1.f;
  }
  float gD[PX], gA[PX];
  if constexpr (AUX) gs_load_aux_grad<PX>(aux, grad_aux, grad_is_final, ix0, iy, wp, crop, gD, gA, R);
  if (tid == 0) {
    for (int s = 0; s < STAGES; ++s) gs_mbar_init(&sm.full[s], GATHER ? THREADS : 1);
    gs_fence_barrier_init();
  }
  __syncthreads();
  if constexpr (GATHER) {
    for (int k = 0; k < STAGES && k < nchunks; ++k)
      issue_sh_gather<K, THREADS>(sm, k, grec, rgb, ids, goff, start + k * CH, min(CH, cnt - k * CH), tid);
  } else if (tid == 0) {
    for (int k = 0; k < STAGES && k < nchunks; ++k)
      issue_sh<K>(sm, k, pA, pB, pS, start + k * CH, min(CH, cnt - k * CH), shift);
// ... 107 lines not shown
      out[0] = GS_LN2 * (2.f * a.z * s[0] - a.w * s[1]);
      out[1] = GS_LN2 * (2.f * b.x * s[1] - a.w * s[0]);
      out[2] = -GS_LN2 * s[2];
      out[3] = GS_LN2 * s[3];
      out[4] = -GS_LN2 * s[4];
      out[5] = GS_LN2 * s[5];
      for (int u = 6; u < NV; ++u) out[u] = p0[u] + p1[u];
      if constexpr (AUX) out[NV] = p0[NV] + p1[NV];
      if (row_epoch) row_epoch[slot] = epoch;
    }
    const bool dead = !(T[0] > GS_T_STOP) && !(T[1] > GS_T_STOP) && !(T[2] > GS_T_STOP) && !(T[3] > GS_T_STOP);
    if (__syncthreads_and(dead)) {
      consumed = min(cnt, (k + 1) * CH);
      break;
    }
    if (k + STAGES < nchunks) {
      const int kn = k + STAGES;
      if constexpr (GATHER)
        issue_sh_gather<K, THREADS>(sm, stage, grec, rgb, ids, goff, start + kn * CH, min(CH, cnt - kn * CH), tid);
      else if (tid == 0)
        issue_sh<K>(sm, stage, pA, pB, pS, start + kn * CH, min(CH, cnt - kn * CH), shift);
    }
  }
  if (tid == 0 && k < nchunks)
    for (int kk = k + 1; kk < nchunks && kk < k + STAGES; ++kk)
      gs_mbar_wait(&sm.full[kk % STAGES], (uint32_t)((kk / STAGES) & 1));
  if (tile_neff_b && tid == 0) tile_neff_b[tile] = consumed;
  if (row_epoch || GATHER) return;
  for (int t = consumed + tid; t < cnt; t += THREADS) {
    const uint32_t slot = __float_as_uint(pS[(size_t)(start + t) * SW + 3 * K]);
    float* out = grad_inst + (size_t)slot * GREC;
    for (int u = 0; u < NV; ++u) out[u] = 0.f;
  }
}

}

int gs_sh_basis_count(int d) { return d == 27 ? 9 : (d == 48 ? 16 : 0); }
int gs_sh_stream_width(int d) { return d == 27 ? sh_sw(9) : sh_sw(16); }
int gs_sh_grad_width(int d) { return d == 27 ? (sh_nv(9) + 3) / 4 * 4 : (sh_nv(16) + 3) / 4 * 4; }
int gs_sh_tc_mode(int d) {
  const int t = gs_tuning().sh_tc;
  return t >= 0 ? t : (d == 48 ? 3 : 0);
}

cudaError_t gs_launch_blend_sh_fwd(const float4* pA, const float2* pB, const float* pS, const GsRec* grec,
                                   const float* rgb, const uint32_t* ids, const uint32_t* goff, int d,
                                   const int* tile_accum,
                                   const GsFrameGeom& g, const GsRayPtrs& r, float* image, int* tile_neff,
                                   float* final_img, const GsCrop& crop, cudaStream_t st, const GsAuxOut* aux) {
#define GS_SHF_A(K, GA, AX, AV)                                                                                     \
  blend_sh_fwd_kernel<K, GA, AX><<<g.n_tiles, 64, 0, st>>>(pA, pB, pS, grec, rgb, ids, goff, tile_accum, g.wp, g.hp,   \
                                                           g.ntx, g.fx, g.fy, r.rays_o, r.lefttop, r.dx, r.dy, image,  \
                                                           tile_neff, final_img, crop, AV)
#define GS_SHF(K, GA) GS_SHF_A(K, GA, false, GsAuxOut{})
  if ((grec || aux) && (gs_sh_tc_mode(d) & 1))
    return gs_launch_blend_sh_fwd_tc(grec, rgb, ids, d, tile_accum, g, r, image, tile_neff, final_img, crop, st, aux);
  if (aux) {
    if (d == 27) GS_SHF_A(9, true, true, *aux); else GS_SHF_A(16, true, true, *aux);
  } else if (grec) {
    if (d == 27) GS_SHF(9, true); else GS_SHF(16, true);
  } else {
    if (d == 27) GS_SHF(9, false); else GS_SHF(16, false);
  }
#undef GS_SHF
#undef GS_SHF_A
  return cudaGetLastError();
}

cudaError_t gs_launch_blend_sh_bwd(const float4* pA, const float2* pB, const float* pS, const GsRec* grec,
                                   const float* rgb, const uint32_t* ids, const uint32_t* goff, int d,
                                   const int* tile_accum,
                                   const GsFrameGeom& g, const GsRayPtrs& r, const float* image,
                                   const float* grad_image, float* grad_inst, int grad_is_final, const GsCrop& crop,
                                   uint32_t* row_epoch, uint32_t epoch, int* tile_neff_b, cudaStream_t st,
                                   const float* aux, const float* grad_aux) {
  if (grec && !row_epoch) return cudaErrorInvalidValue;
  if (grad_aux && (!grec || !aux)) return cudaErrorInvalidValue;
  if (grec && (gs_sh_tc_mode(d) & 2))
    return gs_launch_blend_sh_bwd_tc(grec, rgb, ids, goff, d, tile_accum, g, r, image, grad_image, grad_inst, grad_is_final,
                                     crop, row_epoch, epoch, tile_neff_b, st, aux, grad_aux);
#define GS_SHB_A(K, GA, AX)                                                                                         \
  blend_sh_bwd_kernel<K, GA, AX><<<g.n_tiles, 64, 0, st>>>(pA, pB, pS, grec, rgb, ids, goff, tile_accum, g.wp, g.hp,   \
                                                           g.ntx, g.fx, g.fy, r.rays_o, r.lefttop, r.dx, r.dy, image,  \
                                                           grad_image, grad_inst, grad_is_final, crop, row_epoch,      \
                                                           epoch, tile_neff_b, aux, grad_aux)
#define GS_SHB(K, GA) GS_SHB_A(K, GA, false)
  if (grad_aux) {
    if (d == 27) GS_SHB_A(9, true, true); else GS_SHB_A(16, true, true);
  } else if (grec) {
    if (d == 27) GS_SHB(9, true); else GS_SHB(16, true);
  } else {
    if (d == 27) GS_SHB(9, false); else GS_SHB(16, false);
  }
#undef GS_SHB
#undef GS_SHB_A
  return cudaGetLastError();
}
```

3d-gaussian-splatting_b200/csrc/blend_sh_tc.cu:

```cuda
#include <cstddef>

#include "internal.h"
#include "sh_common.cuh"
#include "tc_common.cuh"

namespace {

using namespace gs_sh;
using namespace gs_tc;

constexpr int TC_J = 16;
constexpr int TC_NT = 256;
constexpr int TC_LGS = 24;

__device__ __forceinline__ int tc_lgs_off(int row, int col) {
  return row * TC_LGS + (((col >> 2) ^ ((row >> 2) & 1)) << 2) + (col & 3);
}

__device__ __forceinline__ int tc_row(int p) {
  return (p >> 7) * 128 + ((p >> 4) & 1) * 64 + ((p >> 5) & 3) * 16 + (p & 15);
}

template <int K, int STAGES>
struct TcStage {
// ... 97 lines not shown
#pragma unroll
  for (int b = 0; b < NB; ++b)
#pragma unroll
    for (int r = 0; r < 2; ++r) {
      const int row = (b0 + b) * 64 + wq * 16 + (lane >> 2) + 8 * r;
#pragma unroll
      for (int c = 0; c < 3; ++c)
        *reinterpret_cast<float2*>(lgs + tc_lgs_off(row, c * 8 + 2 * (lane & 3))) =
            make_float2(acc[b][4 * c + 2 * r], acc[b][4 * c + 2 * r + 1]);
    }
  __syncwarp();
}

__device__ __forceinline__ void tc_read_logits(const float* lgs, int row, float* lr, float* lg, float* lb) {
  float* dst[3] = {lr, lg, lb};
#pragma unroll
  for (int c = 0; c < 3; ++c) {
    const float4 u = *reinterpret_cast<const float4*>(lgs + tc_lgs_off(row, c * 8));
    const float4 v = *reinterpret_cast<const float4*>(lgs + tc_lgs_off(row, c * 8 + 4));
    dst[c][0] = u.x; dst[c][1] = u.y; dst[c][2] = u.z; dst[c][3] = u.w;
    dst[c][4] = v.x; dst[c][5] = v.y; dst[c][6] = v.z; dst[c][7] = v.w;
  }
}

__device__ __forceinline__ void tc_colours(float v0, float v1, float v2, float* col) {
  const float d0 = 1.f + gs_ex2(fminf(v0, 40.f)), d1 = 1.f + gs_ex2(fminf(v1, 40.f)), d2 = 1.f + gs_ex2(fminf(v2, 40.f));
  const float d01 = d0 * d1;
  const float r = gs_rcp(d01 * d2);
  col[2] = r * d01;
  const float r2 = r * d2;
  col[0] = r2 * d1;
  col[1] = r2 * d0;
}

template <int K>
struct TcFwdSmem {
  uint4 img_hi[2 * 256];
  uint4 img_lo[2 * 256];
  uint4 bc_hi[2][2 * 48];
  uint4 bc_lo[2][2 * 48];
  float lgs[256 * TC_LGS];
  TcStage<K, 4> st;
};

template <int K, bool AUX = false>
__global__ void __launch_bounds__(TC_NT) blend_sh_fwd_tc_kernel(const GsRec* __restrict__ grec, const float* __restrict__ rgb,
                                                                const uint32_t* __restrict__ ids,
                                                                const int* __restrict__ tile_accum, int wp, int hp, int ntx,
                                                                float fx, float fy, const float* __restrict__ rays_o,
                                                                const float* __restrict__ lefttop,
                                                                const float* __restrict__ vdx, const float* __restrict__ vdy,
                                                                float* __restrict__ image, int* __restrict__ tile_neff,
                                                                float* __restrict__ final_img, GsCrop crop,
                                                                GsAuxOut aux) {
  constexpr int STAGES = 4;
  extern __shared__ __align__(128) uint8_t tc_smem_raw[];
  TcFwdSmem<K>& sm = *reinterpret_cast<TcFwdSmem<K>*>(tc_smem_raw);
  const int tile = blockIdx.x, tid = threadIdx.x, warp = tid >> 5, lane = tid & 31;
  const int tx = tile % ntx, ty = tile / ntx;
  const int ix = tx * GS_TILE + (tid & 15), iy = ty * GS_TILE + (tid >> 4);
  const int start = tile_accum[tile];
  const int cnt = tile_accum[tile + 1] - start;
  float T = 1.f, cr = 0.f, cg = 0.f, cb = 0.f, dep = 0.f;
  int consumed = cnt;
  if (cnt > 0) {
    const int nchunks = (cnt + TC_J - 1) / TC_J;
    if (tid == 0) {
      for (int s = 0; s < STAGES; ++s) gs_mbar_init(&sm.st.full[s], TC_NT);
      gs_fence_barrier_init();
    }
    {
      float sh[16];
      pixel_sh<K>(ix, iy, rays_o, lefttop, vdx, vdy, sh);
      tc_store_basis<K>(sh, sm.img_hi, sm.img_lo, tid);
    }
    if (tid < 192) {
      sm.bc_hi[tid / 96][tid % 96] = make_uint4(0, 0, 0, 0);
      sm.bc_lo[tid / 96][tid % 96] = make_uint4(0, 0, 0, 0);
    }
    __syncthreads();
    const int row = tc_row(tid);
    const float px = gs_pixel_coord(ix, wp, fx), py = gs_pixel_coord(iy, hp, fy);
    for (int k = 0; k < STAGES - 1 && k < nchunks; ++k)
      tc_gather<K, STAGES, false>(sm.st, k, grec, rgb, ids, nullptr, start + k * TC_J, min(TC_J, cnt - k * TC_J), tid);

    for (int k = 0; k < nchunks; ++k) {
      const int stage = k % STAGES;
      gs_mbar_wait(&sm.st.full[stage], (uint32_t)((k / STAGES) & 1));
      const int n = min(TC_J, cnt - k * TC_J);
      uint4* bc_hi = sm.bc_hi[k & 1];
      uint4* bc_lo = sm.bc_lo[k & 1];
      tc_split_coefs<K>(sm.st.S[stage], bc_hi, bc_lo, tid);
      fence_smem_to_async();
      if (__syncthreads_and(!(T > GS_T_STOP))) {
        consumed = k * TC_J;
        break;
      }
      if (k + STAGES - 1 < nchunks) {
        const int kn = k + STAGES - 1;
        tc_gather<K, STAGES, false>(sm.st, kn % STAGES, grec, rgb, ids, nullptr, start + kn * TC_J,
                                    min(TC_J, cnt - kn * TC_J), tid);
      }
      const float4* R = sm.st.R[stage];
#pragma unroll 1
      for (int h = 0; h < 2; ++h) {
        if (h * 8 >= n) break;
        tc_logits_half<2>(2 * (warp >> 2), h, sm.img_hi, sm.img_lo, bc_hi, bc_lo, sm.lgs, warp & 3, lane);
        if (__all_sync(0xffffffffu, !(T > GS_T_STOP))) continue;
        float lr[8], lg[8], lb[8];
        tc_read_logits(sm.lgs, row, lr, lg, lb);
        const float4* Rh = R + 32 * h;
// ... 118 lines not shown
    }
  }
}

template <int NW, int GREC, int DT = 0>
__device__ __forceinline__ void tc_geom_row(int j, const float (*part)[TC_J][8], const float4* Rr, int tx, int ty,
                                            float* __restrict__ grad_inst, uint32_t* __restrict__ row_epoch,
                                            uint32_t epoch) {
  float s[6];
#pragma unroll
  for (int u = 0; u < 6; ++u) {
    float t = 0.f;
#pragma unroll
    for (int w8 = 0; w8 < NW; ++w8) t += part[w8][j][u];
    s[u] = t;
  }
  const float4 a = Rr[4 * j];
  const float4 b4 = Rr[4 * j + 1];
  const float4 cc = Rr[4 * j + 2];
  const uint32_t rxy = __float_as_uint(cc.z), rwh = __float_as_uint(cc.w);
  const uint32_t slot = __float_as_uint(Rr[4 * j + 3].x) + ((uint32_t)ty - (rxy >> 16)) * (rwh & 0xffffu) +
                        ((uint32_t)tx - (rxy & 0xffffu));
  float* out = grad_inst + (size_t)slot * GREC;
  out[0] = GS_LN2 * (2.f * a.z * s[0] - a.w * s[1]);
  out[1] = GS_LN2 * (2.f * b4.x * s[1] - a.w * s[0]);
  out[2] = -GS_LN2 * s[2];
  out[3] = GS_LN2 * s[3];
  out[4] = -GS_LN2 * s[4];
  out[5] = GS_LN2 * s[5];
  if constexpr (DT > 0) {
    static_assert(DT < GREC, "d_t needs a pad column");
    float t = 0.f;
#pragma unroll
    for (int w8 = 0; w8 < NW; ++w8) t += part[w8][j][6];
    out[DT] = t;
  }
  row_epoch[slot] = epoch;
}


template <int K, bool AUX = false>
__global__ void __launch_bounds__(TC_NT, 2) blend_sh_bwd_tc_kernel(const GsRec* __restrict__ grec, const float* __restrict__ rgb,
                                                                const uint32_t* __restrict__ ids,
                                                                const uint32_t* __restrict__ goff,
                                                                const int* __restrict__ tile_accum, int wp, int hp, int ntx,
                                                                float fx, float fy, const float* __restrict__ rays_o,
                                                                const float* __restrict__ lefttop,
                                                                const float* __restrict__ vdx, const float* __restrict__ vdy,
                                                                const float* __restrict__ image,
                                                                const float* __restrict__ grad_image,
                                                                float* __restrict__ grad_inst, int grad_is_final, GsCrop crop,
                                                                uint32_t* __restrict__ row_epoch, uint32_t epoch,
                                                                int* __restrict__ tile_neff_b, const float* __restrict__ aux,
                                                                const float* __restrict__ grad_aux) {
  constexpr int STAGES = 3, NV = sh_nv(K), GREC = (NV + 3) / 4 * 4;
  static_assert(offsetof(TcBwdSmem<K>, img_hi) == 12 * 256 * 16 && offsetof(TcBwdSmem<K>, img_lo) == 14 * 256 * 16,
                "the basis image must follow the gradient operand: descriptors address both as one region");
  extern __shared__ __align__(128) uint8_t tc_smem_raw[];
  TcBwdSmem<K>& sm = *reinterpret_cast<TcBwdSmem<K>*>(tc_smem_raw);
  const int tile = blockIdx.x, tid = threadIdx.x, warp = tid >> 5, lane = tid & 31, wg = warp >> 2, wq = warp & 3;
  const int tx = tile % ntx, ty = tile / ntx;
  const int ix = tx * GS_TILE + (tid & 15), iy = ty * GS_TILE + (tid >> 4);
  const int start = tile_accum[tile];
  const int cnt = tile_accum[tile + 1] - start;
  if (cnt == 0) return;
  const int nchunks = (cnt + TC_J - 1) / TC_J;
  if (tid == 0) {
    for (int s = 0; s < STAGES; ++s) gs_mbar_init(&sm.st.full[s], TC_NT);
    gs_fence_barrier_init();
  }
  {
    float sh[16];
    pixel_sh<K>(ix, iy, rays_o, lefttop, vdx, vdy, sh);
    tc_store_basis<K>(sh, sm.img_hi, sm.img_lo, tid);
  }
  if (tid < 96) {
    sm.bc_hi[tid] = make_uint4(0, 0, 0, 0);
    sm.bc_lo[tid] = make_uint4(0, 0, 0, 0);
  }
  float T = 1.f, R, gr, gg, gb;
  {
    const size_t off = ((size_t)iy * wp + ix) * 3;
    const float raw[3] = {image[off], image[off + 1], image[off + 2]};
    if (!grad_is_final) {
      gr = grad_image[off];
      gg = grad_image[off + 1];
      gb = grad_image[off + 2];
    } else {
      gs_load_final_grad(grad_image, raw, ix, iy, crop.left, crop.top, crop.width, crop.height, gr, gg, gb);
    }
    R = gr * raw[0] + gg * raw[1] + gb * raw[2];
  }
  float gD = 0.f, gA = 0.f;
  if constexpr (AUX) {
    float gd1[1], ga1[1], r1[1] = {R};
    gs_load_aux_grad<1>(aux, grad_aux, grad_is_final, ix, iy, wp, crop, gd1, ga1, r1);
    gD = gd1[0];
    gA = ga1[0];
    R = r1[0];
  }
  __syncthreads();
  const int row = tc_row(tid);
  const float px = gs_pixel_coord(ix, wp, fx), py = gs_pixel_coord(iy, hp, fy);
  for (int k = 0; k < STAGES - 1 && k < nchunks; ++k)
    tc_gather<K, STAGES, true>(sm.st, k, grec, rgb, ids, goff, start + k * TC_J, min(TC_J, cnt - k * TC_J), tid);

  auto pair = [&](const float4 a, const float4 b4, float l0, float l1, float l2, float* dc, float* v, float t) {
    const float dx = px - a.x, dy = py - a.y;
    const float eu = fmaf(a.z, dx, -a.w * dy);
    const float ev = fmaf(-b4.x * dy, dy, b4.y);
    const float alpha = gs_ex2(fmaf(-dx, eu, ev));
    const bool live = T > GS_T_STOP;
    const float w = live ? alpha * T : 0.f;
// ... 79 lines not shown
        }
      } else {
#pragma unroll
        for (int c = 0; c < 3; ++c)
#pragma unroll
          for (int q = 0; q < 4; ++q) hw[c][q] = lw[c][q] = 0u;
        part[h * 8 + (lane >> 2)][lane & 3] = 0.f;
        part[h * 8 + (lane >> 2)][4 + (lane & 3)] = 0.f;
      }
#pragma unroll
      for (int c = 0; c < 3; ++c) {
        sm.dct[(c * 2 + h) * 256 + row] = make_uint4(hw[c][0], hw[c][1], hw[c][2], hw[c][3]);
        sm.dct[(6 + c * 2 + h) * 256 + row] = make_uint4(lw[c][0], lw[c][1], lw[c][2], lw[c][3]);
      }
    }
    fence_smem_to_async();
    const bool done = __syncthreads_and(!(T > GS_T_STOP)) != 0;
    float acc[1][16];
    tc_contract_issue<1>(wg, sm.dct, sm.img_hi, acc);
    if (tid >= 128 && tid < 128 + n)
      tc_geom_row<8, GREC, AUX ? NV : 0>(tid - 128, sm.part, Rr, tx, ty, grad_inst, row_epoch, epoch);
    n_prev = n;
    st_prev = stage;
    if (!done && k + STAGES - 1 < nchunks) {
      const int kn = k + STAGES - 1;
      tc_gather<K, STAGES, true>(sm.st, kn % STAGES, grec, rgb, ids, goff, start + kn * TC_J, min(TC_J, cnt - kn * TC_J),
                                 tid);
    }
    tc_contract_finish<1>(wg, acc, sm.epi, hs, wq, lane);
    if (done) {
      consumed = min(cnt, (k + 1) * TC_J);
      break;
    }
  }
  __syncthreads();
  if (n_prev > 0 && tid < 96) tc_coef_rows<K, GREC>(n_prev, sm.st.R[st_prev], sm.epi, hs, wq, lane, tx, ty, grad_inst);
  asm volatile("cp.async.wait_all;" ::: "memory");
  if (tile_neff_b && tid == 0) tile_neff_b[tile] = consumed;
}


template <int K>
__global__ void __launch_bounds__(128) blend_sh_bwd_tc2_kernel(const GsRec* __restrict__ grec, const float* __restrict__ rgb,
                                                               const uint32_t* __restrict__ ids,
                                                               const uint32_t* __restrict__ goff,
                                                               const int* __restrict__ tile_accum, int wp, int hp, int ntx,
                                                               float fx, float fy, const float* __restrict__ rays_o,
                                                               const float* __restrict__ lefttop,
                                                               const float* __restrict__ vdx, const float* __restrict__ vdy,
                                                               const float* __restrict__ image,
                                                               const float* __restrict__ grad_image,
                                                               float* __restrict__ grad_inst, int grad_is_final, GsCrop crop,
                                                               uint32_t* __restrict__ row_epoch, uint32_t epoch,
                                                               int* __restrict__ tile_neff_b) {
  constexpr int NT = 128, STAGES = 3, NV = sh_nv(K), GREC = (NV + 3) / 4 * 4;
  extern __shared__ __align__(128) uint8_t tc_smem_raw[];
  TcBwdSmem<K>& sm = *reinterpret_cast<TcBwdSmem<K>*>(tc_smem_raw);
  const int tile = blockIdx.x, tid = threadIdx.x, warp = tid >> 5, lane = tid & 31;
  const int tx = tile % ntx, ty = tile / ntx;
  const int ix = tx * GS_TILE + (tid & 15), iy0 = ty * GS_TILE + (tid >> 4), iy1 = iy0 + 8;
  const int start = tile_accum[tile];
  const int cnt = tile_accum[tile + 1] - start;
  if (cnt == 0) return;
  const int nchunks = (cnt + TC_J - 1) / TC_J;
  if (tid == 0) {
    for (int s = 0; s < STAGES; ++s) gs_mbar_init(&sm.st.full[s], NT);
    gs_fence_barrier_init();
  }
  {
    float sh[16];
    pixel_sh<K>(ix, iy0, rays_o, lefttop, vdx, vdy, sh);
    tc_store_basis<K>(sh, sm.img_hi, sm.img_lo, tid);
    pixel_sh<K>(ix, iy1, rays_o, lefttop, vdx, vdy, sh);
    tc_store_basis<K>(sh, sm.img_hi, sm.img_lo, tid + 128);
  }
  if (tid < 96) {
    sm.bc_hi[tid] = make_uint4(0, 0, 0, 0);
    sm.bc_lo[tid] = make_uint4(0, 0, 0, 0);
  }
  float T[2] = {1.f, 1.f}, R[2], gr[2], gg[2], gb[2];
#pragma unroll
  for (int p = 0; p < 2; ++p) {
    const int iy = p ? iy1 : iy0;
    const size_t off = ((size_t)iy * wp + ix) * 3;
    const float raw[3] = {image[off], image[off + 1], image[off + 2]};
    if (!grad_is_final) {
      gr[p] = grad_image[off];
      gg[p] = grad_image[off + 1];
      gb[p] = grad_image[off + 2];
    } else {
      gs_load_final_grad(grad_image, raw, ix, iy, crop.left, crop.top, crop.width, crop.height, gr[p], gg[p], gb[p]);
    }
    R[p] = gr[p] * raw[0] + gg[p] * raw[1] + gb[p] * raw[2];
  }
  __syncthreads();
  const int row[2] = {tc_row(tid), tc_row(tid + 128)};
  const float px = gs_pixel_coord(ix, wp, fx);
  const float py[2] = {gs_pixel_coord(iy0, hp, fy), gs_pixel_coord(iy1, hp, fy)};
  for (int k = 0; k < STAGES - 1 && k < nchunks; ++k)
    tc_gather<K, STAGES, true, NT>(sm.st, k, grec, rgb, ids, goff, start + k * TC_J, min(TC_J, cnt - k * TC_J), tid);

  auto pair2 = [&](const float4 a, const float4 b4, const float* l0, const float* l1, float (*dc)[3], float* v) {
    const float dx = px - a.x;
    const float adx = a.z * dx;
    float e2[2], ey2[2];
#pragma unroll
    for (int p = 0; p < 2; ++p) {
      const float dy = py[p] - a.y;
      const float eu = fmaf(-a.w, dy, adx);
      const float ev = fmaf(-b4.x * dy, dy, b4.y);
      const float alpha = gs_ex2(fmaf(-dx, eu, ev));
// ... 78 lines not shown
#pragma unroll
          for (int c = 0; c < 3; ++c)
#pragma unroll
            for (int q = 0; q < 4; ++q) hw[p][c][q] = lw[p][c][q] = 0u;
        part[h * 8 + (lane >> 2)][lane & 3] = 0.f;
        part[h * 8 + (lane >> 2)][4 + (lane & 3)] = 0.f;
      }
#pragma unroll
      for (int p = 0; p < 2; ++p)
#pragma unroll
        for (int c = 0; c < 3; ++c) {
          sm.dct[(c * 2 + h) * 256 + row[p]] = make_uint4(hw[p][c][0], hw[p][c][1], hw[p][c][2], hw[p][c][3]);
          sm.dct[(6 + c * 2 + h) * 256 + row[p]] = make_uint4(lw[p][c][0], lw[p][c][1], lw[p][c][2], lw[p][c][3]);
        }
    }
    fence_smem_to_async();
    const bool done = __syncthreads_and(!(T[0] > GS_T_STOP) && !(T[1] > GS_T_STOP)) != 0;
    float acc[2][16];
    tc_contract_issue<2>(0, sm.dct, sm.img_hi, acc);
    if (tid >= 96 && tid < 96 + n) tc_geom_row<4, GREC>(tid - 96, sm.part, Rr, tx, ty, grad_inst, row_epoch, epoch);
    n_prev = n;
    st_prev = stage;
    if (!done && k + STAGES - 1 < nchunks) {
      const int kn = k + STAGES - 1;
      tc_gather<K, STAGES, true, NT>(sm.st, kn % STAGES, grec, rgb, ids, goff, start + kn * TC_J, min(TC_J, cnt - kn * TC_J),
                                     tid);
    }
    tc_contract_finish<2>(0, acc, sm.epi, hs, warp, lane);
    if (done) {
      consumed = min(cnt, (k + 1) * TC_J);
      break;
    }
  }
  __syncthreads();
  if (n_prev > 0 && tid < 96) tc_coef_rows<K, GREC>(n_prev, sm.st.R[st_prev], sm.epi, hs, warp, lane, tx, ty, grad_inst);
  asm volatile("cp.async.wait_all;" ::: "memory");
  if (tile_neff_b && tid == 0) tile_neff_b[tile] = consumed;
}

}

cudaError_t gs_launch_blend_sh_fwd_tc(const GsRec* grec, const float* rgb, const uint32_t* ids, int d,
                                      const int* tile_accum, const GsFrameGeom& g, const GsRayPtrs& r, float* image,
                                      int* tile_neff, float* final_img, const GsCrop& crop, cudaStream_t st,
                                      const GsAuxOut* aux) {
#define GS_SHF_TC(K, AX)                                                                                              \
  do {                                                                                                                \
                            \
    cudaError_t e = cudaFuncSetAttribute(blend_sh_fwd_tc_kernel<K, AX>, cudaFuncAttributeMaxDynamicSharedMemorySize,  \
                                         (int)sizeof(TcFwdSmem<K>));                                                  \
    if (e != cudaSuccess) return e;                                                                                   \
    blend_sh_fwd_tc_kernel<K, AX><<<g.n_tiles, TC_NT, sizeof(TcFwdSmem<K>), st>>>(                                     \
        grec, rgb, ids, tile_accum, g.wp, g.hp, g.ntx, g.fx, g.fy, r.rays_o, r.lefttop, r.dx, r.dy, image, tile_neff,  \
        final_img, crop, aux ? *aux : GsAuxOut{});                                                                    \
  } while (0)
  if (aux) {
    if (d == 27) GS_SHF_TC(9, true); else GS_SHF_TC(16, true);
  } else {
    if (d == 27) GS_SHF_TC(9, false); else GS_SHF_TC(16, false);
  }
#undef GS_SHF_TC
  return cudaGetLastError();
}

cudaError_t gs_launch_blend_sh_bwd_tc(const GsRec* grec, const float* rgb, const uint32_t* ids, const uint32_t* goff, int d,
                                      const int* tile_accum, const GsFrameGeom& g, const GsRayPtrs& r, const float* image,
                                      const float* grad_image, float* grad_inst, int grad_is_final, const GsCrop& crop,
                                      uint32_t* row_epoch, uint32_t epoch, int* tile_neff_b, cudaStream_t st,
                                      const float* aux, const float* grad_aux) {
  if (!row_epoch) return cudaErrorInvalidValue;
  const bool two_px = (gs_sh_tc_mode(d) & 4) != 0;
  if (grad_aux) {
    if (two_px || !aux) return cudaErrorInvalidValue;
#define GS_SHB_TC_AUX(K)                                                                                              \
  do {                                                                                                                \
    cudaError_t e = cudaFuncSetAttribute(blend_sh_bwd_tc_kernel<K, true>, cudaFuncAttributeMaxDynamicSharedMemorySize, \
                                         (int)sizeof(TcBwdSmem<K>));                                                  \
    if (e != cudaSuccess) return e;                                                                                   \
    blend_sh_bwd_tc_kernel<K, true><<<g.n_tiles, TC_NT, sizeof(TcBwdSmem<K>), st>>>(                                   \
        grec, rgb, ids, goff, tile_accum, g.wp, g.hp, g.ntx, g.fx, g.fy, r.rays_o, r.lefttop, r.dx, r.dy, image,       \
        grad_image, grad_inst, grad_is_final, crop, row_epoch, epoch, tile_neff_b, aux, grad_aux);                    \
  } while (0)
    if (d == 27) GS_SHB_TC_AUX(9); else GS_SHB_TC_AUX(16);
#undef GS_SHB_TC_AUX
    return cudaGetLastError();
  }
#define GS_SHB_TC(K)                                                                                                  \
  do {                                                                                                                \
    cudaError_t e = two_px ? cudaFuncSetAttribute(blend_sh_bwd_tc2_kernel<K>, cudaFuncAttributeMaxDynamicSharedMemorySize, \
                                                  (int)sizeof(TcBwdSmem<K>))                                          \
                           : cudaFuncSetAttribute(blend_sh_bwd_tc_kernel<K>, cudaFuncAttributeMaxDynamicSharedMemorySize, \
                                                  (int)sizeof(TcBwdSmem<K>));                                         \
    if (e != cudaSuccess) return e;                                                                                   \
    if (two_px)                                                                                                       \
      blend_sh_bwd_tc2_kernel<K><<<g.n_tiles, 128, sizeof(TcBwdSmem<K>), st>>>(                                        \
          grec, rgb, ids, goff, tile_accum, g.wp, g.hp, g.ntx, g.fx, g.fy, r.rays_o, r.lefttop, r.dx, r.dy, image,     \
          grad_image, grad_inst, grad_is_final, crop, row_epoch, epoch, tile_neff_b);                                 \
    else                                                                                                              \
      blend_sh_bwd_tc_kernel<K><<<g.n_tiles, TC_NT, sizeof(TcBwdSmem<K>), st>>>(                                        \
          grec, rgb, ids, goff, tile_accum, g.wp, g.hp, g.ntx, g.fx, g.fy, r.rays_o, r.lefttop, r.dx, r.dy, image,     \
          grad_image, grad_inst, grad_is_final, crop, row_epoch, epoch, tile_neff_b, nullptr, nullptr);               \
  } while (0)
  if (d == 27) GS_SHB_TC(9); else GS_SHB_TC(16);
#undef GS_SHB_TC
  return cudaGetLastError();
}
```

3d-gaussian-splatting_b200/csrc/internal.h:

```cpp
#pragma once
#include <cuda_runtime.h>
#include <stdint.h>

#include "../../include/gs_b200.h"
#include "project.cuh"

#define GS_GREC 12

struct GsFrameGeom {
  int width, height, wp, hp, ntx, nty, n_tiles;
  float fx, fy;
};

struct GsCrop {
  int left, top, width, height;
};

struct GsAuxOut {
  float bg[3];
  float* aux;
  float* aux_final;
};

#ifdef __CUDACC__
__device__ __forceinline__ void gs_store_aux(const GsAuxOut& ax, int ix, int iy, int wp, const GsCrop& crop,
                                             float depth, float alpha) {
  if (ax.aux) *reinterpret_cast<float2*>(ax.aux + ((size_t)iy * wp + ix) * 2) = make_float2(depth, alpha);
  const int x = ix - crop.left, y = iy - crop.top;
  if (ax.aux_final && x >= 0 && x < crop.width && y >= 0 && y < crop.height)
    *reinterpret_cast<float2*>(ax.aux_final + ((size_t)y * crop.width + x) * 2) = make_float2(depth, alpha);
}
template <int PX>
__device__ __forceinline__ void gs_load_aux_grad(const float* __restrict__ aux, const float* __restrict__ grad_aux,
                                                 int grad_is_final, int ix0, int iy, int wp, const GsCrop& crop,
                                                 float (&gD)[PX], float (&gA)[PX], float (&R)[PX]) {
#pragma unroll
  for (int p = 0; p < PX; ++p) {
    const size_t off = ((size_t)iy * wp + ix0 + p) * 2;
    const float2 da = *reinterpret_cast<const float2*>(aux + off);
    float2 g = make_float2(0.f, 0.f);
    if (!grad_is_final) {
      g = *reinterpret_cast<const float2*>(grad_aux + off);
    } else {
      const int x = ix0 + p - crop.left, y = iy - crop.top;
      if (x >= 0 && x < crop.width && y >= 0 && y < crop.height)
        g = *reinterpret_cast<const float2*>(grad_aux + ((size_t)y * crop.width + x) * 2);
    }
    gD[p] = g.x;
    gA[p] = g.y;
    R[p] = fmaf(g.x, da.x, fmaf(g.y, da.y, R[p]));
  }
}
#endif

struct GsRayPtrs {
  const float *rays_o, *lefttop, *dx, *dy;
};

struct GsTuning {
  int fwd_kernel;
  int fwd_ch;
  int bwd_kernel;
  int bwd_px;
  int bwd_ws;
  int bwd_unroll;
  int bwd_stages;
  int bwd_minb;
  int bwd_rq;
  int fwd_px;
  int bwd_ch;
  int strict;
  int gather;
  int sh_tc;
  int blend_repack;
};
GsTuning& gs_tuning();

void gs_count_launch(int n = 1);

int gs_sh_basis_count(int d);
int gs_sh_stream_width(int d);
int gs_sh_grad_width(int d);
int gs_sh_tc_mode(int d);
cudaError_t gs_launch_blend_sh_fwd(const float4* pA, const float2* pB, const float* pS, const GsRec* grec,
                                   const float* rgb, const uint32_t* ids, const uint32_t* goff , int d,
                                   const int* tile_accum,
                                   const GsFrameGeom& g, const GsRayPtrs& r, float* image, int* tile_neff,
                                   float* final_img, const GsCrop& crop, cudaStream_t st,
                                   const GsAuxOut* aux = nullptr );
cudaError_t gs_launch_blend_sh_bwd(const float4* pA, const float2* pB, const float* pS, const GsRec* grec,
                                   const float* rgb, const uint32_t* ids, const uint32_t* goff , int d,
                                   const int* tile_accum,
                                   const GsFrameGeom& g, const GsRayPtrs& r, const float* image,
                                   const float* grad_image, float* grad_inst, int grad_is_final, const GsCrop& crop,
                                   uint32_t* row_epoch, uint32_t epoch, int* tile_neff_b, cudaStream_t st,
                                   const float* aux = nullptr, const float* grad_aux = nullptr );

cudaError_t gs_launch_blend_sh_fwd_tc(const GsRec* grec, const float* rgb, const uint32_t* ids, int d,
                                      const int* tile_accum, const GsFrameGeom& g, const GsRayPtrs& r, float* image,
                                      int* tile_neff, float* final_img, const GsCrop& crop, cudaStream_t st,
                                      const GsAuxOut* aux = nullptr);
cudaError_t gs_launch_blend_sh_bwd_tc(const GsRec* grec, const float* rgb, const uint32_t* ids, const uint32_t* goff, int d,
                                      const int* tile_accum, const GsFrameGeom& g, const GsRayPtrs& r, const float* image,
                                      const float* grad_image, float* grad_inst, int grad_is_final, const GsCrop& crop,
                                      uint32_t* row_epoch, uint32_t epoch, int* tile_neff_b, cudaStream_t st,
                                      const float* aux = nullptr, const float* grad_aux = nullptr);

cudaError_t gs_launch_fused_project(const float* pos, const float* rgb, const float* opa, const float* quat,
                                    const float* scale, int n, int d, int scale_act, const GsCam& cam,
                                    const GsTileGrid& grid, float near_plane, float half_w, float half_h,
                                    GsRec* rec, uint32_t* count, uint32_t* dkey, int64_t* mask,
                                    unsigned int* n_visible, cudaStream_t st,
                                    bool sh_gaussian = false ,
                                    const GsFilter2d* filt = nullptr );

struct GsGradPush {
  float* bucket;
  float* staging[GS_MAX_PEERS];
  uint32_t per;
  int rank, world;
};

cudaError_t gs_launch_fused_project_bwd(const float* pos, const float* rgb, const float* opa, const float* quat,
                                        const float* scale, int n, int d, int scale_act, const GsCam& cam,
                                        float near_plane, float half_w, float half_h, const uint32_t* offsets_g,
                                        const uint32_t* count, const float* grad_inst, const uint32_t* row_epoch, uint32_t epoch,
                                        float* g_pos, float* g_rgb, float* g_opa,
                                        float* g_quat, float* g_scale, const GsGradPush& push, cudaStream_t st,
                                        bool depth_grad = false ,
                                        bool sh_gaussian = false ,
                                        const GsFilter2d* filt = nullptr );
size_t gs_cam_grad_workspace_bytes(int n);
cudaError_t gs_launch_fused_project_bwd_cam(const float* pos, const float* rgb, const float* opa, const float* quat,
                                            const float* scale, int n, int d, int scale_act, const GsCam& cam,
                                            float near_plane, float half_w, float half_h, const uint32_t* offsets_g,
                                            const uint32_t* count, const float* grad_inst, const uint32_t* row_epoch,
                                            uint32_t epoch, float* g_pos, float* g_rgb, float* g_opa, float* g_quat,
                                            float* g_scale, float* cam_part, float* grad_cam, cudaStream_t st,
                                            bool depth_grad, bool sh_gaussian, const GsFilter2d* filt = nullptr);

cudaError_t gs_launch_emit_keys(const GsRec* rec, const uint32_t* perm, const uint32_t* offsets_sorted, int n, int ntx,
                                void* keys, int key_bytes, uint32_t* vals, cudaStream_t st);
cudaError_t gs_launch_tile_ranges(const void* keys, int key_bytes, long long m, int n_tiles, int* tile_accum,
                                  cudaStream_t st);

cudaError_t gs_launch_pack_sorted(const void* keys, int key_bytes, const uint32_t* vals, long long m, int n_tiles,
                                  int ntx, const GsRec* rec, const uint32_t* offsets_g, float4* pA, float2* pB, float4* pC,
                                  int* tile_accum, cudaStream_t st);

cudaError_t gs_launch_pack_sorted_sh(const void* keys, int key_bytes, const uint32_t* vals, long long m, int n_tiles,
                                     int ntx, const GsRec* rec, const uint32_t* offsets_g, const float* rgb, int d, int sw,
                                     float4* pA, float2* pB, float* pS, int* tile_accum, cudaStream_t st);
cudaError_t gs_launch_iota(uint32_t* out, int n, cudaStream_t st);

cudaError_t gs_launch_blend_fwd(const float4* pA, const float2* pB, const float4* pC, const GsRec* grec,
                                const uint32_t* ids, const int* tile_accum, const GsFrameGeom& g, float* image,
                                int* tile_neff, float* final_img, const GsCrop& crop, cudaStream_t st,
                                const GsAuxOut* aux = nullptr );

cudaError_t gs_launch_blend_bwd(const float4* pA, const float2* pB, const float4* pC, const GsRec* grec,
                                const uint32_t* ids, const uint32_t* goff ,
                                const int* tile_accum, const GsFrameGeom& g, const float* image,
                                const float* grad_image, float* grad_inst ,
                                int grad_is_final, const GsCrop& crop, uint32_t* row_epoch ,
                                uint32_t epoch, int* tile_neff_b ,
                                cudaStream_t st, const float* aux = nullptr ,
                                const float* grad_aux = nullptr );
int gs_blend_aux_supported(int d, bool forward, bool backward);
```

3d-gaussian-splatting_b200/csrc/render.cu:

```cuda
#include <cub/device/device_radix_sort.cuh>
#include <cub/device/device_scan.cuh>
#include <cub/iterator/counting_input_iterator.cuh>
#include <cub/iterator/transform_input_iterator.cuh>

#include <cmath>
#include <cstdio>
#include <cstdlib>
#include <cstring>
#include <new>

#include "internal.h"

struct GsCountInSortedOrder {
  const uint32_t* count;
  const uint32_t* perm;
  uint32_t n;
  __host__ __device__ __forceinline__ uint32_t operator()(uint32_t i) const { return i < n ? count[perm[i]] : 0u; }
};

static thread_local char g_err[512] = {0};

int gs_set_error(cudaError_t e, const char* what) {
  snprintf(g_err, sizeof(g_err), "CUDA error %d (%s) at %s", (int)e, cudaGetErrorString(e), what);
  return (int)e;
}
int gs_set_error_msg(int code, const char* what) {
  snprintf(g_err, sizeof(g_err), "%s", what);
  return code;
}
extern "C" const char* gs_last_error(void) { return g_err; }
extern "C" int gs_abi_version(void) { return 2; }

static int tune_env(const char* name, int dflt) {
  const char* e = getenv(name);
  return e ? atoi(e) : dflt;
}
GsTuning& gs_tuning() {
  static GsTuning t = {tune_env("GS_TUNE_FWD_KERNEL", 0),  tune_env("GS_TUNE_FWD_CH", 128),   tune_env("GS_TUNE_BWD_KERNEL", 1),
                       tune_env("GS_TUNE_BWD_PX", 8),      tune_env("GS_TUNE_BWD_WS", 0),     tune_env("GS_TUNE_BWD_UNROLL", 4),
                       tune_env("GS_TUNE_BWD_STAGES", 3),  tune_env("GS_TUNE_BWD_MINB", 10),  tune_env("GS_TUNE_BWD_RQ", 4),
                       tune_env("GS_TUNE_FWD_PX", 4),      tune_env("GS_TUNE_BWD_CH", 32),    tune_env("GS_TUNE_STRICT", 0),
                       tune_env("GS_TUNE_GATHER", 1),      tune_env("GS_TUNE_SH_TC", -1),     tune_env("GS_TUNE_BLEND_REPACK", 1)};
  return t;
}
extern "C" int gs_tune(const char* name, int value) {
  if (!name) return gs_set_error_msg(GS_ERR_INVALID_ARG, "gs_tune: null name");
  GsTuning& t = gs_tuning();
  struct { const char* k; int* v; } tab[] = {{"fwd_kernel", &t.fwd_kernel}, {"fwd_ch", &t.fwd_ch},
                                             {"bwd_kernel", &t.bwd_kernel}, {"bwd_px", &t.bwd_px},
                                             {"bwd_ws", &t.bwd_ws},         {"bwd_unroll", &t.bwd_unroll},
                                             {"bwd_stages", &t.bwd_stages}, {"bwd_minb", &t.bwd_minb},
                                             {"bwd_rq", &t.bwd_rq},         {"fwd_px", &t.fwd_px},
                                             {"gather", &t.gather},         {"bwd_ch", &t.bwd_ch},
                                             {"strict", &t.strict},         {"sh_tc", &t.sh_tc},
                                             {"blend_repack", &t.blend_repack}};
  for (auto& e : tab)
    if (!strcmp(e.k, name)) {
      *e.v = value;
      return 0;
    }
  return gs_set_error_msg(GS_ERR_INVALID_ARG, "gs_tune: unknown knob");
}

#include <atomic>
static std::atomic<unsigned long long> g_launches{0};
void gs_count_launch(int n) { g_launches.fetch_add((unsigned long long)n, std::memory_order_relaxed); }
extern "C" unsigned long long gs_kernel_launches(void) { return g_launches.load(std::memory_order_relaxed); }

struct GsAllocator {
  gs_alloc_fn alloc = nullptr;
  gs_free_fn free = nullptr;
  void* user = nullptr;
};
static thread_local const GsAllocator* g_cur_alloc = nullptr;

struct DevBuf {
  void* p = nullptr;
  size_t cap = 0;
  const GsAllocator* owner = nullptr;
  void drop(cudaStream_t st, bool sync) {
    if (!p) return;
    if (owner && owner->free) {
      owner->free(p, owner->user);
    } else {
      if (sync) cudaStreamSynchronize(st);
      cudaFree(p);
    }
    p = nullptr;
    cap = 0;
  }
  cudaError_t reserve(size_t bytes, cudaStream_t st) {
    if (bytes <= cap) return cudaSuccess;
    drop(st, true);
    size_t want = bytes + bytes / 8 + 256;
    const GsAllocator* a = g_cur_alloc;
    if (a && a->alloc) {
      p = a->alloc(want, a->user, (gs_stream_t)st);
      if (!p) return cudaErrorMemoryAllocation;
      owner = a;
    } else {
      cudaError_t e = cudaMalloc(&p, want);
      if (e != cudaSuccess) return e;
      owner = nullptr;
    }
    cap = want;
    return cudaSuccess;
  }
  void release() { drop(nullptr, false); }
  template <typename T>
  T* as() const { return static_cast<T*>(p); }
};

struct gs_ctx {
  int device = 0;
  GsAllocator allocator{};
  DevBuf rec, count, offsets, dkey_in, dkey_out, perm, iota, offsets_g;
  size_t iota_n = 0;
  DevBuf keys_in, keys_out, vals_in, vals_out, pA, pB, pC, grad_inst, row_epoch;
  uint32_t epoch = 0;
  DevBuf tile_accum, tile_neff, tile_neff_b, cub_tmp, counters, img_dev, gimg_dev, rays;
  DevBuf cam_part;
  float* host_rays = nullptr;
  unsigned long long* host_m = nullptr;
  cudaEvent_t ev_m = nullptr;
  bool have_forward = false, have_backward = false, gather = false;
  bool have_aux = false;
  bool sh_gaussian = false;
  int n = 0, d = 3, scale_act = 0;
  long long m = 0;
  GsCam cam{};
  GsTileGrid grid{};
  GsFrameGeom geom{};
  float near_plane = 0.f, half_w = 0.f, half_h = 0.f;
  int64_t* mask_ptr = nullptr;
  bool timing = false;
  cudaEvent_t ev[GS_N_STAGES + 2] = {};
  bool ev_ok = false;
  bool ev_fwd_valid = false, ev_bwd_valid = false;
  GsGradPush push{};
  int sh_eval = GS_SH_EVAL_PIXEL;
  int filter2d = GS_FILTER2D_NONE;
  float filter2d_var = 0.3f;
  bool filt_on = false;
  GsFilter2d filt{};
};

static inline void gs_mark(gs_ctx* c, int i, cudaStream_t st) {
  if (c->timing && c->ev_ok) cudaEventRecord(c->ev[i], st);
}

extern "C" int gs_ctx_create(gs_ctx** out) {
  if (!out) return gs_set_error_msg(GS_ERR_INVALID_ARG, "gs_ctx_create: null out");
  gs_ctx* c = new (std::nothrow) gs_ctx();
  if (!c) return gs_set_error_msg(GS_ERR_INVALID_ARG, "gs_ctx_create: out of host memory");
  GS_CUDA_TRY(cudaGetDevice(&c->device));
  cudaError_t e = cudaMallocHost(reinterpret_cast<void**>(&c->host_m), 64);
  if (e == cudaSuccess) e = cudaMallocHost(reinterpret_cast<void**>(&c->host_rays), 64);
  if (e == cudaSuccess) e = cudaEventCreateWithFlags(&c->ev_m, cudaEventDisableTiming);
  if (e != cudaSuccess) {
    delete c;
    return gs_set_error(e, "cudaMallocHost");
  }
  *out = c;
  return 0;
}

extern "C" void gs_ctx_destroy(gs_ctx* c) {
  if (!c) return;
  int cur = -1;
  const bool switched = cudaGetDevice(&cur) == cudaSuccess && cur != c->device && cudaSetDevice(c->device) == cudaSuccess;
  cudaDeviceSynchronize();
  DevBuf* bufs[] = {&c->rec, &c->count, &c->offsets, &c->dkey_in, &c->dkey_out, &c->perm, &c->iota, &c->offsets_g, &c->keys_in, &c->keys_out,
                    &c->vals_in, &c->vals_out, &c->pA, &c->pB, &c->pC, &c->grad_inst, &c->row_epoch, &c->tile_accum, &c->tile_neff,
                    &c->tile_neff_b, &c->cub_tmp, &c->counters, &c->img_dev, &c->gimg_dev, &c->rays, &c->cam_part};
  for (DevBuf* b : bufs) b->release();
  if (c->host_m) cudaFreeHost(c->host_m);
  if (c->host_rays) cudaFreeHost(c->host_rays);
  if (c->ev_m) cudaEventDestroy(c->ev_m);
  if (c->ev_ok)
    for (cudaEvent_t e : c->ev) cudaEventDestroy(e);
  if (switched) cudaSetDevice(cur);
  delete c;
}

static int gs_check_device(int want, const char* who) {
  int dev = -1;
  GS_CUDA_TRY(cudaGetDevice(&dev));
  if (dev != want) {
    char msg[160];
    snprintf(msg, sizeof(msg), "%s: ctx belongs to device %d but device %d is current", who, want, dev);
    return gs_set_error_msg(GS_ERR_INVALID_ARG, msg);
  }
  return 0;
}

static int ceil_log2(unsigned v) {
  int b = 0;
  while ((1u << b) < v) ++b;
  return b;
}

static int render_forward_impl(gs_ctx* c, const float* pos, const float* rgb, const float* opa, const float* quat,
                               const float* scale, int n, int d, int scale_activation, const gs_camera* cam,
                               float* image, float* final_img, int64_t* culling_mask, gs_stream_t stream,
                               const gs_render_aux* ax = nullptr) {
  if (!c || !cam || n < 0) return gs_set_error_msg(GS_ERR_INVALID_ARG, "gs_render_forward: bad arguments");
  if (d != 3 && gs_sh_basis_count(d) == 0)
    return gs_set_error_msg(GS_ERR_UNSUPPORTED, "gs_render_forward: colour width must be 3 (RGB), 27 (SH deg 2) or 48 (SH deg 3)");
  if (cam->width <= 0 || cam->height <= 0 || !(cam->focal_x > 0.f) || !(cam->focal_y > 0.f))
    return gs_set_error_msg(GS_ERR_INVALID_ARG, "gs_render_forward: bad camera");
  if (!(cam->tile_thresh > 0.f && cam->tile_thresh < 1.f))
    return gs_set_error_msg(GS_ERR_INVALID_ARG, "gs_render_forward: tile_thresh must be in (0, 1)");
  if (!image || (n > 0 && (!pos || !rgb || !opa || !quat || !scale)))
    return gs_set_error_msg(GS_ERR_INVALID_ARG, "gs_render_forward: null tensor pointer");
  const bool sh_gaussian = d != 3 && c->sh_eval == GS_SH_EVAL_GAUSSIAN;
  const int blend_d = sh_gaussian ? 3 : d;
  const bool filt_on = c->filter2d != GS_FILTER2D_NONE;
  GsFilter2d filt{};
  if (filt_on) {
    filt.ex = (float)((double)c->filter2d_var / ((double)cam->focal_x * (double)cam->focal_x));
    filt.ey = (float)((double)c->filter2d_var / ((double)cam->focal_y * (double)cam->focal_y));
    filt.compensate = c->filter2d == GS_FILTER2D_ANTIALIAS;
  }
  GsAuxOut aux_out{};
  const bool use_aux = ax && (ax->background || ax->aux || ax->aux_final);
  if (use_aux) {
    if (ax->aux_final && !final_img)
      return gs_set_error_msg(GS_ERR_INVALID_ARG, "gs_render_forward_aux: aux_final needs image_final");
    if (ax->background) {
      for (int k = 0; k < 3; ++k) {
        if (!std::isfinite(ax->background[k]))
          return gs_set_error_msg(GS_ERR_INVALID_ARG, "gs_render_forward_aux: background must be finite");
        aux_out.bg[k] = ax->background[k];
      }
    }
    aux_out.aux = ax->aux;
    aux_out.aux_final = ax->aux_final;
    if (int rc = gs_blend_aux_supported(blend_d, true, ax->aux != nullptr)) return rc;
  }
  if (int rc = gs_check_device(c->device, "gs_render_forward")) return rc;
  g_cur_alloc = &c->allocator;
  cudaStream_t st = (cudaStream_t)stream;
  c->have_forward = false;
  c->have_backward = false;
  c->have_aux = false;

  GsFrameGeom g{};
  g.width = cam->width;
  g.height = cam->height;
  g.wp = (cam->width + GS_TILE - 1) / GS_TILE * GS_TILE;
  g.hp = (cam->height + GS_TILE - 1) / GS_TILE * GS_TILE;
  g.ntx = g.wp / GS_TILE;
  g.nty = g.hp / GS_TILE;
  g.n_tiles = g.ntx * g.nty;
  g.fx = cam->focal_x;
  g.fy = cam->focal_y;
  if (g.ntx > 65535 || g.nty > 65535) return gs_set_error_msg(GS_ERR_INVALID_ARG, "gs_render_forward: image too large");

  GsTileGrid grid{};
  grid.lx = (float)(16.0 / (double)cam->focal_x);
  grid.ly = (float)(16.0 / (double)cam->focal_y);
  grid.leftmost = (float)(-(double)g.wp / 2.0 / (double)cam->focal_x);
  grid.topmost = (float)(-(double)g.hp / 2.0 / (double)cam->focal_y);
  grid.t2 = -2.f * logf(cam->tile_thresh);
  grid.ntx = g.ntx;
  grid.nty = g.nty;
  GsCam dc{};
  memcpy(dc.r, cam->rot, sizeof(dc.r));
  memcpy(dc.t, cam->tran, sizeof(dc.t));
  float half_w = (float)((double)cam->width * 1.2 / 2.0 / (double)cam->focal_x);
  float half_h = (float)((double)cam->height * 1.2 / 2.0 / (double)cam->focal_y);

  size_t N = (size_t)n;
  GS_CUDA_TRY(c->rec.reserve(N * sizeof(GsRec), st));
  GS_CUDA_TRY(c->count.reserve((N + 1) * 4, st));
  GS_CUDA_TRY(c->offsets.reserve((N + 1) * 4, st));
  GS_CUDA_TRY(c->dkey_in.reserve(N * 4 + 4, st));
  GS_CUDA_TRY(c->dkey_out.reserve(N * 4 + 4, st));
  GS_CUDA_TRY(c->perm.reserve(N * 4 + 4, st));
  GS_CUDA_TRY(c->offsets_g.reserve((N + 1) * 4, st));
  GS_CUDA_TRY(c->tile_accum.reserve((size_t)(g.n_tiles + 1) * 4, st));
  GS_CUDA_TRY(c->tile_neff.reserve((size_t)g.n_tiles * 4, st));
  GS_CUDA_TRY(c->tile_neff_b.reserve((size_t)g.n_tiles * 4, st));
  GS_CUDA_TRY(c->counters.reserve(64, st));
  if (c->iota_n < N) {
    GS_CUDA_TRY(c->iota.reserve(N * 4 + 4, st));
    GS_CUDA_TRY(gs_launch_iota(c->iota.as<uint32_t>(), n, st));
    gs_count_launch();
    c->iota_n = N;
  }

  if (blend_d != 3) {
    GS_CUDA_TRY(c->rays.reserve(64, st));
    double m3[9], inv[9];
    for (int k = 0; k < 9; ++k) m3[k] = cam->rot[k];
    double det3 = m3[0] * (m3[4] * m3[8] - m3[5] * m3[7]) - m3[1] * (m3[3] * m3[8] - m3[5] * m3[6]) +
                  m3[2] * (m3[3] * m3[7] - m3[4] * m3[6]);
    inv[0] = (m3[4] * m3[8] - m3[5] * m3[7]) / det3;
    inv[1] = (m3[2] * m3[7] - m3[1] * m3[8]) / det3;
    inv[2] = (m3[1] * m3[5] - m3[2] * m3[4]) / det3;
    inv[3] = (m3[5] * m3[6] - m3[3] * m3[8]) / det3;
    inv[4] = (m3[0] * m3[8] - m3[2] * m3[6]) / det3;
    inv[5] = (m3[2] * m3[3] - m3[0] * m3[5]) / det3;
    inv[6] = (m3[3] * m3[7] - m3[4] * m3[6]) / det3;
    inv[7] = (m3[1] * m3[6] - m3[0] * m3[7]) / det3;
    inv[8] = (m3[0] * m3[4] - m3[1] * m3[3]) / det3;
    double lt[3] = {(-(double)g.wp / 2 + 0.5) / cam->focal_x - cam->tran[0],
                    (-(double)g.hp / 2 + 0.5) / cam->focal_y - cam->tran[1], 1.0 - cam->tran[2]};
    for (int k = 0; k < 3; ++k) {
      c->host_rays[k] = (float)(-(inv[3 * k] * cam->tran[0] + inv[3 * k + 1] * cam->tran[1] + inv[3 * k + 2] * cam->tran[2]));
      c->host_rays[3 + k] = (float)(inv[3 * k] * lt[0] + inv[3 * k + 1] * lt[1] + inv[3 * k + 2] * lt[2]);
      c->host_rays[6 + k] = (float)(inv[3 * k] / cam->focal_x);
      c->host_rays[9 + k] = (float)(inv[3 * k + 1] / cam->focal_y);
    }
    GS_CUDA_TRY(cudaMemcpyAsync(c->rays.p, c->host_rays, 48, cudaMemcpyHostToDevice, st));
  }
  c->ev_fwd_valid = false;
  gs_mark(c, 0, st);
  GS_CUDA_TRY(cudaMemsetAsync(c->counters.p, 0, 64, st));
  GS_CUDA_TRY(cudaMemsetAsync(c->count.as<uint32_t>() + N, 0, 4, st));
  GS_CUDA_TRY(gs_launch_fused_project(pos, rgb, opa, quat, scale, n, d, scale_activation, dc, grid, cam->near_plane,
                                      half_w, half_h, c->rec.as<GsRec>(), c->count.as<uint32_t>(),
                                      c->dkey_in.as<uint32_t>(), culling_mask, c->counters.as<unsigned int>(), st,
                                      sh_gaussian, filt_on ? &filt : nullptr));
  if (n > 0) gs_count_launch();
  gs_mark(c, 1, st);
  size_t tmp_bytes = 0, tmp2 = 0, tmp3 = 0;
  if (n > 0)
    GS_CUDA_TRY(cub::DeviceRadixSort::SortPairs(nullptr, tmp_bytes, c->dkey_in.as<uint32_t>(),
                                                c->dkey_out.as<uint32_t>(), c->iota.as<uint32_t>(),
                                                c->perm.as<uint32_t>(), n, 0, 32, st));
  GsCountInSortedOrder cnt_it_fn{c->count.as<uint32_t>(), c->perm.as<uint32_t>(), (uint32_t)n};
  cub::CountingInputIterator<uint32_t> idx_it(0);
  cub::TransformInputIterator<uint32_t, GsCountInSortedOrder, cub::CountingInputIterator<uint32_t>> cnt_it(idx_it,
                                                                                                            cnt_it_fn);
  GS_CUDA_TRY(cub::DeviceScan::ExclusiveSum(nullptr, tmp2, cnt_it, c->offsets.as<uint32_t>(), n + 1, st));
// ... 25 lines not shown
  const size_t crow = blend_d == 3 ? 16 : (size_t)gs_sh_stream_width(d) * 4;
  if (!gather) {
    GS_CUDA_TRY(c->pA.reserve(M * 16 + 16, st));
    GS_CUDA_TRY(c->pC.reserve(M * crow + 16, st));
    GS_CUDA_TRY(c->pB.reserve((M + 2) * 8, st));
  }
  if (m > 0) {
    GS_CUDA_TRY(c->keys_in.reserve(M * 4 + 16, st));
    GS_CUDA_TRY(c->keys_out.reserve(M * 4 + 16, st));
    GS_CUDA_TRY(c->vals_in.reserve(M * 4, st));
    GS_CUDA_TRY(c->vals_out.reserve(M * 4, st));
    GS_CUDA_TRY(gs_launch_emit_keys(c->rec.as<GsRec>(), c->perm.as<uint32_t>(), c->offsets.as<uint32_t>(), n, g.ntx,
                                    c->keys_in.p, key_bytes, c->vals_in.as<uint32_t>(), st));
    gs_count_launch();
    gs_mark(c, 3, st);
    int end_bit = ceil_log2((unsigned)g.n_tiles);
    if (end_bit < 1) end_bit = 1;
    size_t sort_tmp = 0;
    if (key_bytes == 2) {
      GS_CUDA_TRY(cub::DeviceRadixSort::SortPairs(nullptr, sort_tmp, c->keys_in.as<uint16_t>(),
                                                  c->keys_out.as<uint16_t>(), c->vals_in.as<uint32_t>(),
                                                  c->vals_out.as<uint32_t>(), (int)m, 0, end_bit, st));
      GS_CUDA_TRY(c->cub_tmp.reserve(sort_tmp, st));
      GS_CUDA_TRY(cub::DeviceRadixSort::SortPairs(c->cub_tmp.p, sort_tmp, c->keys_in.as<uint16_t>(),
                                                  c->keys_out.as<uint16_t>(), c->vals_in.as<uint32_t>(),
                                                  c->vals_out.as<uint32_t>(), (int)m, 0, end_bit, st));
    } else {
      GS_CUDA_TRY(cub::DeviceRadixSort::SortPairs(nullptr, sort_tmp, c->keys_in.as<uint32_t>(),
                                                  c->keys_out.as<uint32_t>(), c->vals_in.as<uint32_t>(),
                                                  c->vals_out.as<uint32_t>(), (int)m, 0, end_bit, st));
      GS_CUDA_TRY(c->cub_tmp.reserve(sort_tmp, st));
      GS_CUDA_TRY(cub::DeviceRadixSort::SortPairs(c->cub_tmp.p, sort_tmp, c->keys_in.as<uint32_t>(),
                                                  c->keys_out.as<uint32_t>(), c->vals_in.as<uint32_t>(),
                                                  c->vals_out.as<uint32_t>(), (int)m, 0, end_bit, st));
    }
  }
  if (m == 0) gs_mark(c, 3, st);
  gs_mark(c, 4, st);
  if (gather) {
    GS_CUDA_TRY(gs_launch_tile_ranges(c->keys_out.p, key_bytes, m, g.n_tiles, c->tile_accum.as<int>(), st));
  } else if (blend_d == 3) {
    GS_CUDA_TRY(gs_launch_pack_sorted(c->keys_out.p, key_bytes, c->vals_out.as<uint32_t>(), m, g.n_tiles, g.ntx,
                                      c->rec.as<GsRec>(), c->offsets_g.as<uint32_t>(), c->pA.as<float4>(),
                                      c->pB.as<float2>(), c->pC.as<float4>(), c->tile_accum.as<int>(), st));
  } else {
    GS_CUDA_TRY(gs_launch_pack_sorted_sh(c->keys_out.p, key_bytes, c->vals_out.as<uint32_t>(), m, g.n_tiles, g.ntx,
                                         c->rec.as<GsRec>(), c->offsets_g.as<uint32_t>(), rgb, d,
                                         gs_sh_stream_width(d), c->pA.as<float4>(), c->pB.as<float2>(),
                                         c->pC.as<float>(), c->tile_accum.as<int>(), st));
  }
  if (m > 0) gs_count_launch();
  GsCrop crop{(g.wp - g.width) / 2, (g.hp - g.height) / 2, g.width, g.height};
  gs_mark(c, 5, st);
  if (blend_d == 3) {
    GS_CUDA_TRY(gs_launch_blend_fwd(c->pA.as<float4>(), c->pB.as<float2>(), c->pC.as<float4>(),
                                    gather ? c->rec.as<GsRec>() : nullptr, c->vals_out.as<uint32_t>(),
                                    c->tile_accum.as<int>(), g, image, c->tile_neff.as<int>(), final_img, crop, st,
                                    use_aux ? &aux_out : nullptr));
  } else {
    const float* rp = c->rays.as<float>();
    GsRayPtrs rays{rp, rp + 3, rp + 6, rp + 9};
    GS_CUDA_TRY(gs_launch_blend_sh_fwd(c->pA.as<float4>(), c->pB.as<float2>(), c->pC.as<float>(),
                                       gather ? c->rec.as<GsRec>() : nullptr, rgb, c->vals_out.as<uint32_t>(),
                                       c->offsets_g.as<uint32_t>(), d,
                                       c->tile_accum.as<int>(), g, rays, image, c->tile_neff.as<int>(), final_img,
                                       crop, st, use_aux ? &aux_out : nullptr));
  }
  gs_count_launch();
  gs_mark(c, 6, st);
  c->ev_fwd_valid = c->timing && c->ev_ok;

  c->have_forward = true;
  c->have_aux = aux_out.aux != nullptr;
  c->sh_gaussian = sh_gaussian;
  c->filt_on = filt_on;
  c->filt = filt;
  c->gather = gather;
  c->n = n;
  c->d = d;
  c->scale_act = scale_activation;
  c->m = m;
  c->cam = dc;
  c->grid = grid;
  c->geom = g;
  c->near_plane = cam->near_plane;
  c->half_w = half_w;
  c->half_h = half_h;
  return 0;
}

extern "C" int gs_render_forward(gs_ctx* c, const float* pos, const float* rgb, const float* opa, const float* quat,
                                 const float* scale, int n, int d, int scale_activation, const gs_camera* cam,
                                 float* image, int64_t* culling_mask, gs_stream_t stream) {
  return render_forward_impl(c, pos, rgb, opa, quat, scale, n, d, scale_activation, cam, image, nullptr, culling_mask,
                             stream);
}

extern "C" int gs_render_forward_final(gs_ctx* c, const float* pos, const float* rgb, const float* opa,
                                       const float* quat, const float* scale, int n, int d, int scale_activation,
                                       const gs_camera* cam, float* image_raw_padded, float* image_final,
                                       int64_t* culling_mask, gs_stream_t stream) {
  if (!image_final) return gs_set_error_msg(GS_ERR_INVALID_ARG, "gs_render_forward_final: null image_final");
  return render_forward_impl(c, pos, rgb, opa, quat, scale, n, d, scale_activation, cam, image_raw_padded, image_final,
                             culling_mask, stream);
}

static int render_backward_impl(gs_ctx* c, const float* pos, const float* rgb, const float* opa, const float* quat,
                                const float* scale, const float* image, const float* grad_image, int grad_is_final,
                                float* grad_pos, float* grad_rgb, float* grad_opa, float* grad_quat,
                                float* grad_scale, gs_stream_t stream, const float* aux = nullptr,
                                const float* grad_aux = nullptr, float* grad_cam = nullptr) {
  if (!c) return gs_set_error_msg(GS_ERR_INVALID_ARG, "gs_render_backward: null ctx");
  if (!c->have_forward) return gs_set_error_msg(GS_ERR_NO_FORWARD, "gs_render_backward: no forward on this ctx");
  const bool cam_only = grad_cam && !grad_pos;
  if (!image || !grad_image || (!cam_only && (!grad_pos || !grad_rgb || !grad_opa || !grad_quat || !grad_scale)) ||
      (c->n > 0 && (!pos || !rgb || !opa || !quat || !scale)))
    return gs_set_error_msg(GS_ERR_INVALID_ARG, "gs_render_backward: null tensor pointer");
  if (grad_cam) {
    if (c->d != 3 && !c->sh_gaussian)
      return gs_set_error_msg(GS_ERR_UNSUPPORTED, "gs_render_backward_cam: SH colour evaluated per pixel has no camera "
                                                  "gradient (use GS_SH_EVAL_GAUSSIAN)");
    if (c->push.world)
      return gs_set_error_msg(GS_ERR_UNSUPPORTED, "gs_render_backward_cam: not available with a gradient push configured");
  }
  if (grad_aux) {
    if (!c->have_aux)
      return gs_set_error_msg(GS_ERR_INVALID_ARG, "gs_render_backward_aux: grad_aux given but the forward wrote no aux");
    if (!aux) return gs_set_error_msg(GS_ERR_INVALID_ARG, "gs_render_backward_aux: grad_aux needs the forward's aux");
    if (int rc = gs_blend_aux_supported(c->sh_gaussian ? 3 : c->d, false, true)) return rc;
  }
  if (int rc = gs_check_device(c->device, "gs_render_backward")) return rc;
  g_cur_alloc = &c->allocator;
  cudaStream_t st = (cudaStream_t)stream;
  size_t M = (size_t)c->m;
  const int d = c->d;
  const int blend_d = c->sh_gaussian ? 3 : d;
  const size_t grow = blend_d == 3 ? (size_t)GS_GREC * 4 : (size_t)gs_sh_grad_width(d) * 4;
  GS_CUDA_TRY(c->grad_inst.reserve(M * grow + 16, st));
  {
    const size_t before = c->row_epoch.cap;
    GS_CUDA_TRY(c->row_epoch.reserve(M * 4 + 16, st));
    if (c->row_epoch.cap != before || c->epoch == 0xffffffffu) {
      GS_CUDA_TRY(cudaMemsetAsync(c->row_epoch.p, 0, c->row_epoch.cap, st));
      c->epoch = 0;
    }
    ++c->epoch;
  }
  c->ev_bwd_valid = false;
  GsCrop crop{(c->geom.wp - c->geom.width) / 2, (c->geom.hp - c->geom.height) / 2, c->geom.width, c->geom.height};
  gs_mark(c, 7, st);
  if (c->m > 0) {
    if (blend_d == 3) {
      GS_CUDA_TRY(gs_launch_blend_bwd(c->pA.as<float4>(), c->pB.as<float2>(), c->pC.as<float4>(),
                                      c->gather ? c->rec.as<GsRec>() : nullptr, c->vals_out.as<uint32_t>(),
                                      c->offsets_g.as<uint32_t>(), c->tile_accum.as<int>(), c->geom, image, grad_image,
                                      c->grad_inst.as<float>(),
                                      grad_is_final, crop, c->row_epoch.as<uint32_t>(), c->epoch,
                                      c->tile_neff_b.as<int>(), st, aux, grad_aux));
    } else {
      const float* rp = c->rays.as<float>();
      GsRayPtrs rays{rp, rp + 3, rp + 6, rp + 9};
      GS_CUDA_TRY(gs_launch_blend_sh_bwd(c->pA.as<float4>(), c->pB.as<float2>(), c->pC.as<float>(),
                                         c->gather ? c->rec.as<GsRec>() : nullptr, rgb, c->vals_out.as<uint32_t>(),
                                         c->offsets_g.as<uint32_t>(), d,
                                         c->tile_accum.as<int>(), c->geom, rays, image, grad_image,
                                         c->grad_inst.as<float>(), grad_is_final, crop,
                                         c->row_epoch.as<uint32_t>(), c->epoch, c->tile_neff_b.as<int>(), st, aux,
                                         grad_aux));
    }
    gs_count_launch();
    c->have_backward = true;
  }
  gs_mark(c, 8, st);
  if (c->push.world) {
    const float* lo = c->push.bucket;
    const float* hi = lo + (size_t)c->push.world * c->push.per;
    const size_t nn = (size_t)c->n;
    const float* seg[5] = {grad_pos, grad_rgb, grad_opa, grad_quat, grad_scale};
    const size_t len[5] = {3 * nn, (size_t)d * nn, nn, 4 * nn, 3 * nn};
    for (int k = 0; k < 5; ++k)
      if (seg[k] < lo || seg[k] + len[k] > hi)
        return gs_set_error_msg(GS_ERR_INVALID_ARG, "gs_render_backward: gradient buffers are not inside the push bucket");
    if ((grad_quat - lo) % 4)
      return gs_set_error_msg(GS_ERR_INVALID_ARG, "gs_render_backward: grad_quat must sit on a 16-byte bucket offset");
  }
  if (grad_cam) {
    GS_CUDA_TRY(c->cam_part.reserve(gs_cam_grad_workspace_bytes(c->n) + 16, st));
    GS_CUDA_TRY(gs_launch_fused_project_bwd_cam(pos, rgb, opa, quat, scale, c->n, d, c->scale_act, c->cam,
                                                c->near_plane, c->half_w, c->half_h, c->offsets_g.as<uint32_t>(),
                                                c->count.as<uint32_t>(), c->grad_inst.as<float>(),
                                                c->row_epoch.as<uint32_t>(), c->epoch, grad_pos, grad_rgb, grad_opa,
                                                grad_quat, grad_scale, c->cam_part.as<float>(), grad_cam, st,
                                                grad_aux != nullptr, c->sh_gaussian, c->filt_on ? &c->filt : nullptr));
    gs_count_launch(c->n > 0 ? 2 : 1);
  } else {
    GS_CUDA_TRY(gs_launch_fused_project_bwd(pos, rgb, opa, quat, scale, c->n, d, c->scale_act, c->cam, c->near_plane,
                                            c->half_w, c->half_h, c->offsets_g.as<uint32_t>(), c->count.as<uint32_t>(),
                                            c->grad_inst.as<float>(), c->row_epoch.as<uint32_t>(), c->epoch,
                                            grad_pos, grad_rgb, grad_opa, grad_quat, grad_scale, c->push, st,
                                            grad_aux != nullptr, c->sh_gaussian, c->filt_on ? &c->filt : nullptr));
    if (c->n > 0) gs_count_launch();
  }
  gs_mark(c, 9, st);
  c->ev_bwd_valid = c->timing && c->ev_ok;
  return 0;
}

extern "C" int gs_render_backward(gs_ctx* c, const float* pos, const float* rgb, const float* opa, const float* quat,
                                  const float* scale, const float* image, const float* grad_image, float* grad_pos,
                                  float* grad_rgb, float* grad_opa, float* grad_quat, float* grad_scale,
                                  gs_stream_t stream) {
  return render_backward_impl(c, pos, rgb, opa, quat, scale, image, grad_image, 0, grad_pos, grad_rgb, grad_opa,
                              grad_quat, grad_scale, stream);
}

extern "C" int gs_render_backward_final(gs_ctx* c, const float* pos, const float* rgb, const float* opa,
                                        const float* quat, const float* scale, const float* image_raw_padded,
                                        const float* grad_final, float* grad_pos, float* grad_rgb, float* grad_opa,
// ... 99 lines not shown
  unsigned int nvis = 0;
  cudaError_t e = cudaMemcpyAsync(h, c->tile_accum.p, sizeof(int) * (size_t)(T + 1), cudaMemcpyDeviceToHost, st);
  if (e == cudaSuccess)
    e = cudaMemcpyAsync(h + T + 1, c->tile_neff.p, sizeof(int) * (size_t)T, cudaMemcpyDeviceToHost, st);
  if (e == cudaSuccess && c->have_backward)
    e = cudaMemcpyAsync(h + 2 * T + 1, c->tile_neff_b.p, sizeof(int) * (size_t)T, cudaMemcpyDeviceToHost, st);
  if (e == cudaSuccess) e = cudaMemcpyAsync(&nvis, c->counters.p, 4, cudaMemcpyDeviceToHost, st);
  if (e == cudaSuccess) e = cudaStreamSynchronize(st);
  if (e != cudaSuccess) {
    free(h);
    return gs_set_error(e, "gs_frame_stats copy");
  }
  long long meff = 0, meff_b = 0;
  int mx = 0;
  for (int t = 0; t < T; ++t) {
    int cnt = h[t + 1] - h[t];
    if (cnt > mx) mx = cnt;
    meff += h[T + 1 + t];
    if (c->have_backward && cnt > 0) meff_b += h[2 * T + 1 + t];
  }
  free(h);
  out->n_gaussians = c->n;
  out->n_visible = (int)nvis;
  out->n_instances = c->m;
  out->n_instances_eff = meff;
  out->n_instances_eff_bwd = c->have_backward ? meff_b : -1;
  out->width_padded = c->geom.wp;
  out->height_padded = c->geom.hp;
  out->n_tiles = T;
  out->max_tile_count = mx;
  return 0;
}

extern "C" int gs_frame_sorted(gs_ctx* c, int* gauss_idx, long long capacity, int* tile_accum, gs_stream_t stream) {
  if (!c) return gs_set_error_msg(GS_ERR_INVALID_ARG, "gs_frame_sorted: null ctx");
  if (!c->have_forward) return gs_set_error_msg(GS_ERR_NO_FORWARD, "gs_frame_sorted: no forward on this ctx");
  cudaStream_t st = (cudaStream_t)stream;
  if (gauss_idx && c->m > 0) {
    long long k = capacity < c->m ? capacity : c->m;
    if (k > 0)
      GS_CUDA_TRY(cudaMemcpyAsync(gauss_idx, c->vals_out.p, sizeof(int) * (size_t)k, cudaMemcpyDeviceToDevice, st));
  }
  if (tile_accum)
    GS_CUDA_TRY(cudaMemcpyAsync(tile_accum, c->tile_accum.p, sizeof(int) * (size_t)(c->geom.n_tiles + 1),
                                cudaMemcpyDeviceToDevice, st));
  return 0;
}

extern "C" int gs_frame_tile_consumed(gs_ctx* c, int* tile_consumed, gs_stream_t stream) {
  if (!c || !tile_consumed) return gs_set_error_msg(GS_ERR_INVALID_ARG, "gs_frame_tile_consumed: null argument");
  if (!c->have_forward) return gs_set_error_msg(GS_ERR_NO_FORWARD, "gs_frame_tile_consumed: no forward on this ctx");
  GS_CUDA_TRY(cudaMemcpyAsync(tile_consumed, c->tile_neff.p, sizeof(int) * (size_t)c->geom.n_tiles,
                              cudaMemcpyDeviceToDevice, (cudaStream_t)stream));
  return 0;
}

extern "C" int gs_render_forward_backward_host(gs_ctx* c, const float* pos, const float* rgb, const float* opa,
                                               const float* quat, const float* scale, int n, int d,
                                               int scale_activation, const gs_camera* cam,
                                               const float* grad_image_host, float* image_host, float* grad_pos,
                                               float* grad_rgb, float* grad_opa, float* grad_quat, float* grad_scale,
                                               gs_stream_t stream) {
  if (!c || !cam || !grad_image_host || !image_host)
    return gs_set_error_msg(GS_ERR_INVALID_ARG, "gs_render_forward_backward_host: null argument");
  if (cam->width <= 0 || cam->height <= 0)
    return gs_set_error_msg(GS_ERR_INVALID_ARG, "gs_render_forward_backward_host: bad camera");
  cudaStream_t st = (cudaStream_t)stream;
  g_cur_alloc = &c->allocator;
  int wp = (cam->width + GS_TILE - 1) / GS_TILE * GS_TILE, hp = (cam->height + GS_TILE - 1) / GS_TILE * GS_TILE;
  size_t img_bytes = (size_t)wp * hp * 3 * sizeof(float);
  DevBuf& img_dev = c->img_dev;
  DevBuf& gimg_dev = c->gimg_dev;
  GS_CUDA_TRY(img_dev.reserve(img_bytes, st));
  GS_CUDA_TRY(gimg_dev.reserve(img_bytes, st));
  GS_CUDA_TRY(cudaMemcpyAsync(gimg_dev.p, grad_image_host, img_bytes, cudaMemcpyHostToDevice, st));
  int rc = gs_render_forward(c, pos, rgb, opa, quat, scale, n, d, scale_activation, cam, img_dev.as<float>(), nullptr,
                             stream);
  if (rc) return rc;
  rc = gs_render_backward(c, pos, rgb, opa, quat, scale, img_dev.as<float>(), gimg_dev.as<float>(), grad_pos, grad_rgb,
                          grad_opa, grad_quat, grad_scale, stream);
  if (rc) return rc;
  GS_CUDA_TRY(cudaMemcpyAsync(image_host, img_dev.p, img_bytes, cudaMemcpyDeviceToHost, st));
  GS_CUDA_TRY(cudaStreamSynchronize(st));
  return 0;
}

extern "C" int gs_ctx_set_timing(gs_ctx* c, int enable) {
  if (!c) return gs_set_error_msg(GS_ERR_INVALID_ARG, "gs_ctx_set_timing: null ctx");
  if (enable && !c->ev_ok) {
    for (cudaEvent_t& e : c->ev) GS_CUDA_TRY(cudaEventCreate(&e));
    c->ev_ok = true;
  }
  c->timing = enable != 0;
  c->ev_fwd_valid = c->ev_bwd_valid = false;
  return 0;
}

extern "C" int gs_frame_stage_ms(gs_ctx* c, float* out, gs_stream_t stream) {
  if (!c || !out) return gs_set_error_msg(GS_ERR_INVALID_ARG, "gs_frame_stage_ms: null argument");
  for (int i = 0; i < GS_N_STAGES; ++i) out[i] = -1.f;
  if (!c->ev_ok) return 0;
  GS_CUDA_TRY(cudaStreamSynchronize((cudaStream_t)stream));
  if (c->ev_fwd_valid)
    for (int i = 0; i < 6; ++i) GS_CUDA_TRY(cudaEventElapsedTime(&out[i], c->ev[i], c->ev[i + 1]));
  if (c->ev_bwd_valid)
    for (int i = 6; i < 8; ++i) GS_CUDA_TRY(cudaEventElapsedTime(&out[i], c->ev[i + 1], c->ev[i + 2]));
// ... 3 lines not shown
```

include/gs_b200.h:

```cpp
#ifndef GS_B200_H
#define GS_B200_H

#include <stddef.h>
#include <stdint.h>

#ifdef __cplusplus
extern "C" {
#endif

typedef void* gs_stream_t;

#define GS_ERR_INVALID_ARG (-1)
#define GS_ERR_UNSUPPORTED (-2)
#define GS_ERR_NO_FORWARD (-3)

int gs_abi_version(void);
const char* gs_last_error(void);
int gs_tune(const char* name, int value);
unsigned long long gs_kernel_launches(void);


int gs_project_fwd(const float* pos, const float* quat, const float* scale, const float* rot,
                   const float* tran, int n, float near_plane, float half_width, float half_height,
                   float* res_pos, float* res_cov, int64_t* mask, gs_stream_t stream);
// ... 76 lines not shown

int gs_render_forward_final(gs_ctx* ctx, const float* pos, const float* rgb, const float* opa,
                            const float* quat, const float* scale, int n, int d, int scale_activation,
                            const gs_camera* cam_host, float* image_raw_padded, float* image_final,
                            int64_t* culling_mask, gs_stream_t stream);
int gs_render_backward_final(gs_ctx* ctx, const float* pos, const float* rgb, const float* opa,
                             const float* quat, const float* scale, const float* image_raw_padded,
                             const float* grad_final, float* grad_pos, float* grad_rgb, float* grad_opa,
                             float* grad_quat, float* grad_scale, gs_stream_t stream);

typedef struct gs_render_aux {
  const float* background;
  float* aux;
  float* aux_final;
} gs_render_aux;
int gs_render_forward_aux(gs_ctx* ctx, const float* pos, const float* rgb, const float* opa,
                          const float* quat, const float* scale, int n, int d, int scale_activation,
                          const gs_camera* cam_host, float* image_raw_padded, float* image_final,
                          int64_t* culling_mask, const gs_render_aux* aux, gs_stream_t stream);
int gs_render_backward_aux(gs_ctx* ctx, const float* pos, const float* rgb, const float* opa,
                           const float* quat, const float* scale, const float* image_raw_padded,
                           const float* grad_image, int grad_is_final, const float* aux, const float* grad_aux,
                           float* grad_pos, float* grad_rgb, float* grad_opa, float* grad_quat, float* grad_scale,
                           gs_stream_t stream);

int gs_render_backward_cam(gs_ctx* ctx, const float* pos, const float* rgb, const float* opa, const float* quat,
                           const float* scale, const float* image_raw_padded, const float* grad_image,
                           int grad_is_final, const float* aux, const float* grad_aux,
                           float* grad_pos, float* grad_rgb, float* grad_opa, float* grad_quat, float* grad_scale,
                           float* grad_cam ,
                           gs_stream_t stream);

#define GS_SH_EVAL_PIXEL 0
#define GS_SH_EVAL_GAUSSIAN 1
int gs_ctx_set_sh_eval(gs_ctx* ctx, int mode);

#define GS_FILTER2D_NONE 0
#define GS_FILTER2D_DILATE 1
#define GS_FILTER2D_ANTIALIAS 2
int gs_ctx_set_filter2d(gs_ctx* ctx, int mode, float variance_px2);

#define GS_N_STAGES 8
int gs_ctx_set_timing(gs_ctx* ctx, int enable);
int gs_frame_stage_ms(gs_ctx* ctx, float* out_host, gs_stream_t stream);

long long gs_frame_instances(gs_ctx* ctx);

int gs_frame_stats(gs_ctx* ctx, gs_frame_info* out_host, gs_stream_t stream);

int gs_frame_sorted(gs_ctx* ctx, int* gauss_idx, long long capacity, int* tile_accum, gs_stream_t stream);

int gs_frame_tile_consumed(gs_ctx* ctx, int* tile_consumed, gs_stream_t stream);

int gs_render_forward_backward_host(gs_ctx* ctx, const float* pos, const float* rgb, const float* opa,
                                    const float* quat, const float* scale, int n, int d,
                                    int scale_activation, const gs_camera* cam_host,
                                    const float* grad_image_host, float* image_host,
                                    float* grad_pos, float* grad_rgb, float* grad_opa,
                                    float* grad_quat, float* grad_scale, gs_stream_t stream);

int gs_adam_step(float* param, const float* grad, float* exp_avg, float* exp_avg_sq, long long n,
                 const long long* seg_end_host, const float* lr_host, int n_seg, float beta1, float beta2,
                 float eps, int step, gs_stream_t stream);

size_t gs_densify_workspace_bytes(int n);
int gs_densify_plan(const float* opa, const float* scale, const float* grad, int n, int scale_activation,
                    float opa_logit_min, float delete_thresh, float grad_thresh, int grad_agg_max, float tau,
                    int use_clone, int use_split, unsigned char* code, int* dst, void* workspace,
                    size_t workspace_bytes, gs_stream_t stream);
int gs_densify_apply(const float* pos, const float* rgb, const float* opa, const float* quat, const float* scale,
                     int n, int d, const unsigned char* code, const int* dst, const float* grad, float clone_dt,
                     const float* normals, int n_keep, int n_clone, int n_split, int scale_activation,
                     float* out_pos, float* out_rgb, float* out_opa, float* out_quat, float* out_scale,
                     gs_stream_t stream);

size_t gs_loss_workspace_bytes(int height, int width);
int gs_loss_l1_ssim(const float* image, const void* target, int target_is_half, int height, int width,
                    float w_l1, float w_ssim, float bias, float* grad_image, float* out3, void* workspace,
                    size_t workspace_bytes, gs_stream_t stream);

int gs_allreduce_multimem_f32(void* multicast_ptr, long long n_floats, int rank, int world,
                              gs_stream_t stream);

#define GS_MAX_PEERS 8
int gs_allreduce_p2p_f32(void* const* peer_ptrs, long long n_floats, int rank, int world,
                         gs_stream_t stream);

typedef struct gs_grad_push {
  int world, rank;
  long long per;
  float* bucket;
  float* staging[GS_MAX_PEERS];
} gs_grad_push;
int gs_ctx_set_grad_push(gs_ctx* ctx, const gs_grad_push* push);
int gs_allreduce_push_finish_f32(void* const* peer_buckets, const float* staging_local, long long n_floats,
                                 long long per, int rank, int world, gs_stream_t stream);
int gs_allreduce_push_finish_mc_f32(void* bucket_multicast, const float* bucket_local, const float* staging_local,
                                    long long n_floats, long long per, int rank, int world, gs_stream_t stream);

#ifdef __cplusplus
}
#endif
#endif
```

Before: 457.2.

## Schedule blend tiles heaviest-first via a cost-bucketed tile order

Adds a single-block kernel that bucket-sorts tiles by cost: instance count for the forward pass, and the forward's consumed-instance count for the backward pass. Heavy tiles come first, and the light tail keeps its natural order. All blend kernels read their tile index from this order instead of blockIdx, which is meant to reduce the end-of-launch tail caused by load imbalance across SMs. In exchange it adds two extra small single-block launches per frame and gives up the spatial locality of row-major tile order for the heavy tiles.

Measured after the change: 468.0 (median of 6 runs). 2.4% higher.

```diff
diff --git a/3d-gaussian-splatting_b200/csrc/bindings.cpp b/3d-gaussian-splatting_b200/csrc/bindings.cpp
--- a/3d-gaussian-splatting_b200/csrc/bindings.cpp
+++ b/3d-gaussian-splatting_b200/csrc/bindings.cpp
@@ -539,6 +539,14 @@
     check_rc(gs_frame_tile_consumed(ctx, out.data_ptr<int>(), cur_stream()), "gs_frame_tile_consumed");
     return out;
   }
+
+  torch::Tensor tile_order() {
+    gs_frame_info fi{};
+    check_rc(gs_frame_stats(ctx, &fi, cur_stream()), "gs_frame_stats");
+    auto out = torch::empty({(int64_t)fi.n_tiles}, torch::TensorOptions().device(torch::kCUDA, device).dtype(at::kInt));
+    check_rc(gs_frame_tile_order(ctx, out.data_ptr<int>(), cur_stream()), "gs_frame_tile_order");
+    return out;
+  }
 };
 
 void adam_step(torch::Tensor param, torch::Tensor grad, torch::Tensor exp_avg, torch::Tensor exp_avg_sq,
@@ -721,7 +729,8 @@
       .def("clear_grad_push", &RenderContext::clear_grad_push)
       .def("stage_ms", &RenderContext::stage_ms)
       .def("sorted_instances", &RenderContext::sorted_instances)
-      .def("tile_consumed", &RenderContext::tile_consumed);
+      .def("tile_consumed", &RenderContext::tile_consumed)
+      .def("tile_order", &RenderContext::tile_order);
   m.def("allreduce_push_finish", &allreduce_push_finish, "second half of the pushed gradient exchange");
   m.def("allreduce_push_finish_mc", &allreduce_push_finish_mc,
         "second half of the pushed gradient exchange, broadcast through the NVSwitch (multimem.st)");
diff --git a/3d-gaussian-splatting_b200/csrc/binning.cu b/3d-gaussian-splatting_b200/csrc/binning.cu
--- a/3d-gaussian-splatting_b200/csrc/binning.cu
+++ b/3d-gaussian-splatting_b200/csrc/binning.cu
@@ -208,6 +208,106 @@
 __global__ void __launch_bounds__(kBlock) iota_kernel(uint32_t* out, int n) {
   int i = blockIdx.x * kBlock + threadIdx.x;
   if (i < n) out[i] = (uint32_t)i;
+}
+
+constexpr int kOrderWarps = 32, kOrderBuckets = 256;
+__device__ __forceinline__ int tile_order_bucket(const int* __restrict__ tile_accum, const int* __restrict__ tile_cost,
+                                                 int t, int shift) {
+  const int c = tile_cost ? tile_cost[t] : tile_accum[t + 1] - tile_accum[t];
+  return kOrderBuckets - 1 - min(max(c, 0) >> shift, kOrderBuckets - 1);
+}
+
+__global__ void __launch_bounds__(32 * kOrderWarps) tile_order_kernel(const int* __restrict__ tile_accum,
+                                                                      const int* __restrict__ tile_cost, int n,
+                                                                      int shift, int tail, int* __restrict__ order) {
+  __shared__ int cnt[kOrderWarps][kOrderBuckets];
+  __shared__ int base[kOrderBuckets];
+  __shared__ int cut;
+  const int tid = threadIdx.x, warp = tid >> 5, lane = tid & 31;
+  const unsigned lt = (1u << lane) - 1u;
+  const int len = (n + kOrderWarps - 1) / kOrderWarps, lo = warp * len, hi = min(n, lo + len);
+  if (tid < kOrderBuckets) base[tid] = 0;
+  __syncthreads();
+  for (int t = tid; t < n; t += 32 * kOrderWarps) atomicAdd(&base[tile_order_bucket(tile_accum, tile_cost, t, shift)], 1);
+  __syncthreads();
+  if (warp == 0) {
+    constexpr int PL = kOrderBuckets / 32;
+    int v[PL], sum = 0;
+#pragma unroll
+    for (int k = 0; k < PL; ++k) {
+      v[k] = base[lane * PL + k];
+      sum += v[k];
+    }
+    int incl = sum;
+#pragma unroll
+    for (int o = 1; o < 32; o <<= 1) {
+      const int y = __shfl_down_sync(0xffffffffu, incl, o);
+      if (lane + o < 32) incl += y;
+    }
+    int lighter = incl - sum, c = -1;
+#pragma unroll
+    for (int k = PL - 1; k >= 0; --k) {
+      if (c < 0 && lighter >= tail) c = lane * PL + k;
+      lighter += v[k];
+    }
+    c = __reduce_max_sync(0xffffffffu, c);
+    if (lane == 0) cut = c;
+  }
+  for (int i = tid; i < kOrderWarps * kOrderBuckets; i += 32 * kOrderWarps) (&cnt[0][0])[i] = 0;
+  __syncthreads();
+  const int cb = cut;
+  for (int t0 = lo; t0 < hi; t0 += 32) {
+    const int t = t0 + lane;
+    const int b = t < hi ? max(tile_order_bucket(tile_accum, tile_cost, t, shift), cb) : kOrderBuckets;
+    const unsigned peers = __match_any_sync(0xffffffffu, b);
+    if (b < kOrderBuckets && (peers & lt) == 0) cnt[warp][b] += __popc(peers);
+    __syncwarp();
+  }
+  __syncthreads();
+  if (tid < kOrderBuckets) {
+    int run = 0;
+    for (int w = 0; w < kOrderWarps; ++w) {
+      const int v = cnt[w][tid];
+      cnt[w][tid] = run;
+      run += v;
+    }
+    base[tid] = run;
+  }
+  __syncthreads();
+  if (warp == 0) {
+    int v[kOrderBuckets / 32], sum = 0;
+#pragma unroll
+    for (int k = 0; k < kOrderBuckets / 32; ++k) {
+      v[k] = base[lane * (kOrderBuckets / 32) + k];
+      sum += v[k];
+    }
+    int incl = sum;
+#pragma unroll
+    for (int o = 1; o < 32; o <<= 1) {
+      const int y = __shfl_up_sync(0xffffffffu, incl, o);
+      if (lane >= o) incl += y;
+    }
+    int run = incl - sum;
+#pragma unroll
+    for (int k = 0; k < kOrderBuckets / 32; ++k) {
+      base[lane * (kOrderBuckets / 32) + k] = run;
+      run += v[k];
+    }
+  }
+  __syncthreads();
+  for (int i = tid; i < kOrderWarps * kOrderBuckets; i += 32 * kOrderWarps) (&cnt[0][0])[i] += base[i % kOrderBuckets];
+  __syncthreads();
+  for (int t0 = lo; t0 < hi; t0 += 32) {
+    const int t = t0 + lane;
+    const int b = t < hi ? max(tile_order_bucket(tile_accum, tile_cost, t, shift), cb) : kOrderBuckets;
+    const unsigned peers = __match_any_sync(0xffffffffu, b);
+    if (b < kOrderBuckets) {
+      order[cnt[warp][b] + __popc(peers & lt)] = t;
+      __syncwarp(peers);
+      if ((peers & lt) == 0) cnt[warp][b] += __popc(peers);
+    }
+    __syncwarp();
+  }
 }
 
 }
@@ -317,3 +417,10 @@
                                                           rec, offsets_g, pA, pB, pC, tile_accum);
   return cudaGetLastError();
 }
+
+cudaError_t gs_launch_tile_order(const int* tile_accum, const int* tile_cost, int n_tiles, int shift, int tail,
+                                 int* order, cudaStream_t st) {
+  if (n_tiles <= 0 || n_tiles > GS_TILE_ORDER_MAX) return cudaErrorInvalidValue;
+  tile_order_kernel<<<1, 32 * kOrderWarps, 0, st>>>(tile_accum, tile_cost, n_tiles, shift, tail, order);
+  return cudaGetLastError();
+}
diff --git a/3d-gaussian-splatting_b200/csrc/blend.cu b/3d-gaussian-splatting_b200/csrc/blend.cu
--- a/3d-gaussian-splatting_b200/csrc/blend.cu
+++ b/3d-gaussian-splatting_b200/csrc/blend.cu
@@ -113,11 +113,11 @@
                                                                  float* __restrict__ image,
                                                                  int* __restrict__ tile_neff,
                                                                  float* __restrict__ final_img, GsCrop crop,
-                                                                 GsAuxOut aux) {
+                                                                 GsAuxOut aux, const int* __restrict__ order) {
   static_assert(!AUX || GATHER, "the aux outputs read |p_c| from the gathered records");
   using Smem = typename std::conditional<GATHER, GatherRing<FWD_CH, FWD_STAGES, 3>, FwdSmem<FWD_CH>>::type;
   __shared__ __align__(16) Smem sm;
-  const int tile = blockIdx.x;
+  const int tile = gs_block_tile(order);
   const int tid = threadIdx.x;
   const int tx = tile % ntx, ty = tile / ntx;
   constexpr int FWD_PX = PX, TPR = GS_TILE / PX, NTHREADS = 256 / PX;
@@ -303,13 +303,14 @@
                                                                 const float* __restrict__ grad_image,
                                                                 float* __restrict__ grad_inst, int grad_is_final,
                                                                 GsCrop crop, uint32_t* __restrict__ row_epoch,
-                                                                uint32_t epoch, int* __restrict__ tile_neff_b) {
+                                                                uint32_t epoch, int* __restrict__ tile_neff_b,
+                                                                const int* __restrict__ order) {
   constexpr int THREADS = 32 * WARPS;
   constexpr int PX = 256 / THREADS;
   constexpr int TPR = GS_TILE / PX;
   using Smem = BwdSmem<WARPS, BWD_CH>;
   __shared__ __align__(16) Smem sm;
-  const int tile = blockIdx.x;
+  const int tile = gs_block_tile(order);
   const int tid = threadIdx.x, warp = tid >> 5, lane = tid & 31;
   const int tx = tile % ntx, ty = tile / ntx;
   const int start = tile_accum[tile];
@@ -557,10 +558,11 @@
                                                                       int hp, int ntx, float fx, float fy,
                                                                       float* __restrict__ image,
                                                                       int* __restrict__ tile_neff,
-                                                                      float* __restrict__ final_img, GsCrop crop) {
+                                                                      float* __restrict__ final_img, GsCrop crop,
+                                                                      const int* __restrict__ order) {
   using Smem = WsRing<WSF_STAGES>;
   __shared__ __align__(16) Smem sm;
-  const int tile = blockIdx.x;
+  const int tile = gs_block_tile(order);
   const int tid = threadIdx.x;
   const int start = tile_accum[tile];
   const int cnt = tile_accum[tile + 1] - start;
@@ -827,7 +829,7 @@
                       const float* __restrict__ image, const float* __restrict__ grad_image,
                       float* __restrict__ grad_inst, int grad_is_final, GsCrop crop, uint32_t* __restrict__ row_epoch,
                       uint32_t epoch, int* __restrict__ tile_neff_b, const float* __restrict__ aux,
-                      const float* __restrict__ grad_aux) {
+                      const float* __restrict__ grad_aux, const int* __restrict__ order) {
   using Cfg = Bwd2Cfg<PX, STAGES, RQ>;
   constexpr int NT = Cfg::NT, TPR = Cfg::TPR, R = Cfg::R, SQ = Cfg::SQ, QS = Cfg::QS, IS = Cfg::IS, ROWS = Cfg::ROWS;
   static_assert(IS % 2 == 0 && QS % 2 == 0 && IS % 32 == 2 && QS % 32 == 32 / RQ, "partial buffer strides");
@@ -839,7 +841,7 @@
   using Smem = typename std::conditional<AUX, Bwd2SmemAux<PX, STAGES, RQ, GATHER, CH>,
                                          Bwd2Smem<PX, STAGES, RQ, GATHER, CH>>::type;
   __shared__ __align__(16) Smem sm;
-  const int tile = blockIdx.x;
+  const int tile = gs_block_tile(order);
   const int tid = threadIdx.x, warp = tid >> 5, lane = tid & 31;
   const int start = tile_accum[tile];
   const int cnt = tile_accum[tile + 1] - start;
@@ -1278,18 +1280,19 @@
   const bool gather = grec != nullptr;
   if (aux) {
     blend_fwd_kernel<128, 4, true, true><<<g.n_tiles, 64, 0, st>>>(pA, pB, pC, grec, ids, tile_accum, g.wp, g.hp, g.ntx,
-                                                                  g.fx, g.fy, image, tile_neff, final_img, crop, *aux);
+                                                                  g.fx, g.fy, image, tile_neff, final_img, crop, *aux, g.order);
     return cudaGetLastError();
   }
   if (!gather && tn.fwd_kernel != 0) {
     blend_fwd_ws_kernel<<<g.n_tiles, WSF_CONS + 32, 0, st>>>(pA, pB, pC, tile_accum, g.wp, g.hp, g.ntx, g.fx, g.fy, image,
-                                                             tile_neff, final_img, crop);
+                                                             tile_neff, final_img, crop, g.order);
     return cudaGetLastError();
   }
   const int ch = tn.fwd_ch;
 #define GS_FWD_LAUNCH(CH, PX, GA)                                                                                   \
   blend_fwd_kernel<CH, PX, GA><<<g.n_tiles, 256 / PX, 0, st>>>(pA, pB, pC, grec, ids, tile_accum, g.wp, g.hp, g.ntx, \
-                                                               g.fx, g.fy, image, tile_neff, final_img, crop, GsAuxOut{})
+                                                               g.fx, g.fy, image, tile_neff, final_img, crop,     \
+                                                               GsAuxOut{}, g.order)
 #define GS_FWD_CH(PX, GA)                     \
   if (ch == 64) GS_FWD_LAUNCH(64, PX, GA);    \
   else if (ch == 256) GS_FWD_LAUNCH(256, PX, GA); \
@@ -1318,7 +1321,7 @@
 #define GS_BWD2_AUX(RP)                                                                                            \
   blend_bwd2_kernel<8, false, 4, 3, 10, 4, true, 32, true, RP><<<g.n_tiles, 32, 0, st>>>(                           \
       pA, pB, pC, grec, ids, goff, tile_accum, g.wp, g.hp, g.ntx, g.fx, g.fy, image, grad_image, grad_inst,         \
-      grad_is_final, crop, row_epoch, epoch, tile_neff_b, aux, grad_aux)
+      grad_is_final, crop, row_epoch, epoch, tile_neff_b, aux, grad_aux, g.order)
     if (tn.blend_repack) GS_BWD2_AUX(true);
     else GS_BWD2_AUX(false);
 #undef GS_BWD2_AUX
@@ -1329,7 +1332,7 @@
   blend_bwd2_kernel<PX, WS, UNR, ST, MINB, RQ, GA, CH><<<g.n_tiles, 256 / PX + (WS ? 32 : 0), 0, st>>>(              \
       pA, pB, pC, grec, ids, goff, tile_accum, g.wp, g.hp, g.ntx, g.fx, g.fy, image, grad_image, grad_inst,          \
       grad_is_final,                                                                                                 \
-      crop, row_epoch, epoch, tile_neff_b, nullptr, nullptr)
+      crop, row_epoch, epoch, tile_neff_b, nullptr, nullptr, g.order)
 #define GS_BWD2(PX, WS, UNR, ST, MINB, RQ, GA) GS_BWD2C(PX, WS, UNR, ST, MINB, RQ, GA, 64)
     const int key = ((((tn.bwd_px * 10 + tn.bwd_ws) * 10 + tn.bwd_unroll) * 10 + tn.bwd_stages) * 10 + tn.bwd_rq) * 100 +
                     tn.bwd_minb;
@@ -1338,7 +1341,7 @@
   if (tn.blend_repack)                                                                                             \
     blend_bwd2_kernel<8, false, 4, 3, 10, 4, true, 32, false, true><<<g.n_tiles, 32, 0, st>>>(                      \
         pA, pB, pC, grec, ids, goff, tile_accum, g.wp, g.hp, g.ntx, g.fx, g.fy, image, grad_image, grad_inst,       \
-        grad_is_final, crop, row_epoch, epoch, tile_neff_b, nullptr, nullptr);                                     \
+        grad_is_final, crop, row_epoch, epoch, tile_neff_b, nullptr, nullptr, g.order);                            \
   else                                                                                                             \
     GS_BWD2C(8, false, 4, 3, 10, 4, true, 32)
       switch (key) {
@@ -1400,7 +1403,7 @@
 #define GS_BWD_LAUNCH(W, CH)                                                                                         \
   blend_bwd_kernel<W, CH><<<g.n_tiles, 32 * W, 0, st>>>(pA, pB, pC, tile_accum, g.wp, g.hp, g.ntx, g.fx, g.fy, image, \
                                                         grad_image, grad_inst, grad_is_final, crop, row_epoch, epoch, \
-                                                        tile_neff_b)
+                                                        tile_neff_b, g.order)
   if (warps == 1) GS_BWD_LAUNCH(1, 64);
   else if (ch == 32) GS_BWD_LAUNCH(2, 32);
   else if (ch == 128) GS_BWD_LAUNCH(2, 128);
diff --git a/3d-gaussian-splatting_b200/csrc/blend_sh.cu b/3d-gaussian-splatting_b200/csrc/blend_sh.cu
--- a/3d-gaussian-splatting_b200/csrc/blend_sh.cu
+++ b/3d-gaussian-splatting_b200/csrc/blend_sh.cu
@@ -106,12 +106,13 @@
                                                            const float* __restrict__ vdx,
                                                            const float* __restrict__ vdy, float* __restrict__ image,
                                                            int* __restrict__ tile_neff,
-                                                           float* __restrict__ final_img, GsCrop crop, GsAuxOut aux) {
+                                                           float* __restrict__ final_img, GsCrop crop, GsAuxOut aux,
+                                                           const int* __restrict__ order) {
   constexpr int CH = 64, STAGES = 2, PX = 4, SW = sh_sw(K), NT = 64;
   static_assert(!AUX || GATHER, "the aux outputs read |p_c| from the gathered records");
   using SM = typename std::conditional<GATHER, ShGatherStage<K, CH, STAGES>, ShStage<K, CH, STAGES>>::type;
   __shared__ __align__(16) SM sm;
-  const int tile = blockIdx.x, tid = threadIdx.x;
+  const int tile = gs_block_tile(order), tid = threadIdx.x;
   const int tx = tile % ntx, ty = tile / ntx;
   const int ix0 = tx * GS_TILE + (tid & 3) * PX;
   const int iy = ty * GS_TILE + (tid >> 2);
@@ -275,13 +276,14 @@
                                                            GsCrop crop, uint32_t* __restrict__ row_epoch,
                                                            uint32_t epoch, int* __restrict__ tile_neff_b,
                                                            const float* __restrict__ aux,
-                                                           const float* __restrict__ grad_aux) {
+                                                           const float* __restrict__ grad_aux,
+                                                           const int* __restrict__ order) {
   constexpr int CH = 32, STAGES = 2, PX = 4, SW = sh_sw(K), NV = sh_nv(K), NVP = sh_nvp(K), THREADS = 64;
   constexpr int GREC = (NV + 3) / 4 * 4;
   static_assert(!AUX || (GATHER && NV < NVP && NV < GREC), "d_t needs a pad slot in the partial and gradient rows");
   __shared__ __align__(16) ShBwdSmem<K, GATHER> smem;
   auto& sm = smem.st;
-  const int tile = blockIdx.x, tid = threadIdx.x, warp = tid >> 5, lane = tid & 31;
+  const int tile = gs_block_tile(order), tid = threadIdx.x, warp = tid >> 5, lane = tid & 31;
   const int tx = tile % ntx, ty = tile / ntx;
   const int start = tile_accum[tile];
   const int cnt = tile_accum[tile + 1] - start;
@@ -495,7 +497,7 @@
 #define GS_SHF_A(K, GA, AX, AV)                                                                                     \
   blend_sh_fwd_kernel<K, GA, AX><<<g.n_tiles, 64, 0, st>>>(pA, pB, pS, grec, rgb, ids, goff, tile_accum, g.wp, g.hp,   \
                                                            g.ntx, g.fx, g.fy, r.rays_o, r.lefttop, r.dx, r.dy, image,  \
-                                                           tile_neff, final_img, crop, AV)
+                                                           tile_neff, final_img, crop, AV, g.order)
 #define GS_SHF(K, GA) GS_SHF_A(K, GA, false, GsAuxOut{})
   if ((grec || aux) && (gs_sh_tc_mode(d) & 1))
     return gs_launch_blend_sh_fwd_tc(grec, rgb, ids, d, tile_accum, g, r, image, tile_neff, final_img, crop, st, aux);
@@ -527,7 +529,7 @@
   blend_sh_bwd_kernel<K, GA, AX><<<g.n_tiles, 64, 0, st>>>(pA, pB, pS, grec, rgb, ids, goff, tile_accum, g.wp, g.hp,   \
                                                            g.ntx, g.fx, g.fy, r.rays_o, r.lefttop, r.dx, r.dy, image,  \
                                                            grad_image, grad_inst, grad_is_final, crop, row_epoch,      \
-                                                           epoch, tile_neff_b, aux, grad_aux)
+                                                           epoch, tile_neff_b, aux, grad_aux, g.order)
 #define GS_SHB(K, GA) GS_SHB_A(K, GA, false)
   if (grad_aux) {
     if (d == 27) GS_SHB_A(9, true, true); else GS_SHB_A(16, true, true);
diff --git a/3d-gaussian-splatting_b200/csrc/blend_sh_tc.cu b/3d-gaussian-splatting_b200/csrc/blend_sh_tc.cu
--- a/3d-gaussian-splatting_b200/csrc/blend_sh_tc.cu
+++ b/3d-gaussian-splatting_b200/csrc/blend_sh_tc.cu
@@ -173,11 +173,11 @@
                                                                 const float* __restrict__ vdx, const float* __restrict__ vdy,
                                                                 float* __restrict__ image, int* __restrict__ tile_neff,
                                                                 float* __restrict__ final_img, GsCrop crop,
-                                                                GsAuxOut aux) {
+                                                                GsAuxOut aux, const int* __restrict__ order) {
   constexpr int STAGES = 4;
   extern __shared__ __align__(128) uint8_t tc_smem_raw[];
   TcFwdSmem<K>& sm = *reinterpret_cast<TcFwdSmem<K>*>(tc_smem_raw);
-  const int tile = blockIdx.x, tid = threadIdx.x, warp = tid >> 5, lane = tid & 31;
+  const int tile = gs_block_tile(order), tid = threadIdx.x, warp = tid >> 5, lane = tid & 31;
   const int tx = tile % ntx, ty = tile / ntx;
   const int ix = tx * GS_TILE + (tid & 15), iy = ty * GS_TILE + (tid >> 4);
   const int start = tile_accum[tile];
@@ -402,13 +402,14 @@
                                                                 float* __restrict__ grad_inst, int grad_is_final, GsCrop crop,
                                                                 uint32_t* __restrict__ row_epoch, uint32_t epoch,
                                                                 int* __restrict__ tile_neff_b, const float* __restrict__ aux,
-                                                                const float* __restrict__ grad_aux) {
+                                                                const float* __restrict__ grad_aux,
+                                                                const int* __restrict__ order) {
   constexpr int STAGES = 3, NV = sh_nv(K), GREC = (NV + 3) / 4 * 4;
   static_assert(offsetof(TcBwdSmem<K>, img_hi) == 12 * 256 * 16 && offsetof(TcBwdSmem<K>, img_lo) == 14 * 256 * 16,
                 "the basis image must follow the gradient operand: descriptors address both as one region");
   extern __shared__ __align__(128) uint8_t tc_smem_raw[];
   TcBwdSmem<K>& sm = *reinterpret_cast<TcBwdSmem<K>*>(tc_smem_raw);
-  const int tile = blockIdx.x, tid = threadIdx.x, warp = tid >> 5, lane = tid & 31, wg = warp >> 2, wq = warp & 3;
+  const int tile = gs_block_tile(order), tid = threadIdx.x, warp = tid >> 5, lane = tid & 31, wg = warp >> 2, wq = warp & 3;
   const int tx = tile % ntx, ty = tile / ntx;
   const int ix = tx * GS_TILE + (tid & 15), iy = ty * GS_TILE + (tid >> 4);
   const int start = tile_accum[tile];
@@ -594,11 +595,12 @@
                                                                const float* __restrict__ grad_image,
                                                                float* __restrict__ grad_inst, int grad_is_final, GsCrop crop,
                                                                uint32_t* __restrict__ row_epoch, uint32_t epoch,
-                                                               int* __restrict__ tile_neff_b) {
+                                                               int* __restrict__ tile_neff_b,
+                                                               const int* __restrict__ order) {
   constexpr int NT = 128, STAGES = 3, NV = sh_nv(K), GREC = (NV + 3) / 4 * 4;
   extern __shared__ __align__(128) uint8_t tc_smem_raw[];
   TcBwdSmem<K>& sm = *reinterpret_cast<TcBwdSmem<K>*>(tc_smem_raw);
-  const int tile = blockIdx.x, tid = threadIdx.x, warp = tid >> 5, lane = tid & 31;
+  const int tile = gs_block_tile(order), tid = threadIdx.x, warp = tid >> 5, lane = tid & 31;
   const int tx = tile % ntx, ty = tile / ntx;
   const int ix = tx * GS_TILE + (tid & 15), iy0 = ty * GS_TILE + (tid >> 4), iy1 = iy0 + 8;
   const int start = tile_accum[tile];
@@ -783,7 +785,7 @@
     if (e != cudaSuccess) return e;                                                                                   \
     blend_sh_fwd_tc_kernel<K, AX><<<g.n_tiles, TC_NT, sizeof(TcFwdSmem<K>), st>>>(                                     \
         grec, rgb, ids, tile_accum, g.wp, g.hp, g.ntx, g.fx, g.fy, r.rays_o, r.lefttop, r.dx, r.dy, image, tile_neff,  \
-        final_img, crop, aux ? *aux : GsAuxOut{});                                                                    \
+        final_img, crop, aux ? *aux : GsAuxOut{}, g.order);                                                           \
   } while (0)
   if (aux) {
     if (d == 27) GS_SHF_TC(9, true); else GS_SHF_TC(16, true);
@@ -810,7 +812,7 @@
     if (e != cudaSuccess) return e;                                                                                   \
     blend_sh_bwd_tc_kernel<K, true><<<g.n_tiles, TC_NT, sizeof(TcBwdSmem<K>), st>>>(                                   \
         grec, rgb, ids, goff, tile_accum, g.wp, g.hp, g.ntx, g.fx, g.fy, r.rays_o, r.lefttop, r.dx, r.dy, image,       \
-        grad_image, grad_inst, grad_is_final, crop, row_epoch, epoch, tile_neff_b, aux, grad_aux);                    \
+        grad_image, grad_inst, grad_is_final, crop, row_epoch, epoch, tile_neff_b, aux, grad_aux, g.order);           \
   } while (0)
     if (d == 27) GS_SHB_TC_AUX(9); else GS_SHB_TC_AUX(16);
 #undef GS_SHB_TC_AUX
@@ -826,11 +828,11 @@
     if (two_px)                                                                                                       \
       blend_sh_bwd_tc2_kernel<K><<<g.n_tiles, 128, sizeof(TcBwdSmem<K>), st>>>(                                        \
           grec, rgb, ids, goff, tile_accum, g.wp, g.hp, g.ntx, g.fx, g.fy, r.rays_o, r.lefttop, r.dx, r.dy, image,     \
-          grad_image, grad_inst, grad_is_final, crop, row_epoch, epoch, tile_neff_b);                                 \
+          grad_image, grad_inst, grad_is_final, crop, row_epoch, epoch, tile_neff_b, g.order);                        \
     else                                                                                                              \
       blend_sh_bwd_tc_kernel<K><<<g.n_tiles, TC_NT, sizeof(TcBwdSmem<K>), st>>>(                                        \
           grec, rgb, ids, goff, tile_accum, g.wp, g.hp, g.ntx, g.fx, g.fy, r.rays_o, r.lefttop, r.dx, r.dy, image,     \
-          grad_image, grad_inst, grad_is_final, crop, row_epoch, epoch, tile_neff_b, nullptr, nullptr);               \
+          grad_image, grad_inst, grad_is_final, crop, row_epoch, epoch, tile_neff_b, nullptr, nullptr, g.order);      \
   } while (0)
   if (d == 27) GS_SHB_TC(9); else GS_SHB_TC(16);
 #undef GS_SHB_TC
diff --git a/3d-gaussian-splatting_b200/csrc/internal.h b/3d-gaussian-splatting_b200/csrc/internal.h
--- a/3d-gaussian-splatting_b200/csrc/internal.h
+++ b/3d-gaussian-splatting_b200/csrc/internal.h
@@ -10,6 +10,7 @@
 struct GsFrameGeom {
   int width, height, wp, hp, ntx, nty, n_tiles;
   float fx, fy;
+  const int* order;
 };
 
 struct GsCrop {
@@ -23,6 +24,9 @@
 };
 
 #ifdef __CUDACC__
+__device__ __forceinline__ int gs_block_tile(const int* __restrict__ order) {
+  return order ? __ldg(order + blockIdx.x) : (int)blockIdx.x;
+}
 __device__ __forceinline__ void gs_store_aux(const GsAuxOut& ax, int ix, int iy, int wp, const GsCrop& crop,
                                              float depth, float alpha) {
   if (ax.aux) *reinterpret_cast<float2*>(ax.aux + ((size_t)iy * wp + ix) * 2) = make_float2(depth, alpha);
@@ -73,6 +77,7 @@
   int gather;
   int sh_tc;
   int blend_repack;
+  int tile_order;
 };
 GsTuning& gs_tuning();
 
@@ -152,6 +157,9 @@
                                      int ntx, const GsRec* rec, const uint32_t* offsets_g, const float* rgb, int d, int sw,
                                      float4* pA, float2* pB, float* pS, int* tile_accum, cudaStream_t st);
 cudaError_t gs_launch_iota(uint32_t* out, int n, cudaStream_t st);
+#define GS_TILE_ORDER_MAX 16384
+cudaError_t gs_launch_tile_order(const int* tile_accum, const int* tile_cost, int n_tiles, int shift, int tail,
+                                 int* order, cudaStream_t st);
 
 cudaError_t gs_launch_blend_fwd(const float4* pA, const float2* pB, const float4* pC, const GsRec* grec,
                                 const uint32_t* ids, const int* tile_accum, const GsFrameGeom& g, float* image,
diff --git a/3d-gaussian-splatting_b200/csrc/render.cu b/3d-gaussian-splatting_b200/csrc/render.cu
--- a/3d-gaussian-splatting_b200/csrc/render.cu
+++ b/3d-gaussian-splatting_b200/csrc/render.cu
@@ -40,7 +40,8 @@
                        tune_env("GS_TUNE_BWD_PX", 8),      tune_env("GS_TUNE_BWD_WS", 0),     tune_env("GS_TUNE_BWD_UNROLL", 4),
                        tune_env("GS_TUNE_BWD_STAGES", 3),  tune_env("GS_TUNE_BWD_MINB", 10),  tune_env("GS_TUNE_BWD_RQ", 4),
                        tune_env("GS_TUNE_FWD_PX", 4),      tune_env("GS_TUNE_BWD_CH", 32),    tune_env("GS_TUNE_STRICT", 0),
-                       tune_env("GS_TUNE_GATHER", 1),      tune_env("GS_TUNE_SH_TC", -1),     tune_env("GS_TUNE_BLEND_REPACK", 1)};
+                       tune_env("GS_TUNE_GATHER", 1),      tune_env("GS_TUNE_SH_TC", -1),     tune_env("GS_TUNE_BLEND_REPACK", 1),
+                       tune_env("GS_TUNE_TILE_ORDER", 1)};
   return t;
 }
 extern "C" int gs_tune(const char* name, int value) {
@@ -53,7 +54,7 @@
                                              {"bwd_rq", &t.bwd_rq},         {"fwd_px", &t.fwd_px},
                                              {"gather", &t.gather},         {"bwd_ch", &t.bwd_ch},
                                              {"strict", &t.strict},         {"sh_tc", &t.sh_tc},
-                                             {"blend_repack", &t.blend_repack}};
+                                             {"blend_repack", &t.blend_repack}, {"tile_order", &t.tile_order}};
   for (auto& e : tab)
     if (!strcmp(e.k, name)) {
       *e.v = value;
@@ -113,12 +114,15 @@
 
 struct gs_ctx {
   int device = 0;
+  int n_sm = 1;
   GsAllocator allocator{};
   DevBuf rec, count, offsets, dkey_in, dkey_out, perm, iota, offsets_g;
   size_t iota_n = 0;
   DevBuf keys_in, keys_out, vals_in, vals_out, pA, pB, pC, grad_inst, row_epoch;
   uint32_t epoch = 0;
   DevBuf tile_accum, tile_neff, tile_neff_b, cub_tmp, counters, img_dev, gimg_dev, rays;
+  DevBuf tile_order;
+  bool order_on = false;
   DevBuf cam_part;
   float* host_rays = nullptr;
   unsigned long long* host_m = nullptr;
@@ -154,6 +158,7 @@
   gs_ctx* c = new (std::nothrow) gs_ctx();
   if (!c) return gs_set_error_msg(GS_ERR_INVALID_ARG, "gs_ctx_create: out of host memory");
   GS_CUDA_TRY(cudaGetDevice(&c->device));
+  GS_CUDA_TRY(cudaDeviceGetAttribute(&c->n_sm, cudaDevAttrMultiProcessorCount, c->device));
   cudaError_t e = cudaMallocHost(reinterpret_cast<void**>(&c->host_m), 64);
   if (e == cudaSuccess) e = cudaMallocHost(reinterpret_cast<void**>(&c->host_rays), 64);
   if (e == cudaSuccess) e = cudaEventCreateWithFlags(&c->ev_m, cudaEventDisableTiming);
@@ -172,7 +177,8 @@
   cudaDeviceSynchronize();
   DevBuf* bufs[] = {&c->rec, &c->count, &c->offsets, &c->dkey_in, &c->dkey_out, &c->perm, &c->iota, &c->offsets_g, &c->keys_in, &c->keys_out,
                     &c->vals_in, &c->vals_out, &c->pA, &c->pB, &c->pC, &c->grad_inst, &c->row_epoch, &c->tile_accum, &c->tile_neff,
-                    &c->tile_neff_b, &c->cub_tmp, &c->counters, &c->img_dev, &c->gimg_dev, &c->rays, &c->cam_part};
+                    &c->tile_neff_b, &c->cub_tmp, &c->counters, &c->img_dev, &c->gimg_dev, &c->rays, &c->cam_part,
+                    &c->tile_order};
   for (DevBuf* b : bufs) b->release();
   if (c->host_m) cudaFreeHost(c->host_m);
   if (c->host_rays) cudaFreeHost(c->host_rays);
@@ -198,6 +204,21 @@
   int b = 0;
   while ((1u << b) < v) ++b;
   return b;
+}
+
+constexpr int kFwdOrderShift = 5, kBwdOrderShift = 3, kFwdTailPerSm = 36, kBwdTailPerSm = 28;
+static cudaError_t build_tile_order(gs_ctx* c, GsFrameGeom& g, const int* tile_cost, int shift, int tail_per_sm,
+                                    cudaStream_t st) {
+  g.order = nullptr;
+  c->order_on = false;
+  if (!gs_tuning().tile_order || g.n_tiles > GS_TILE_ORDER_MAX) return cudaSuccess;
+  cudaError_t e = gs_launch_tile_order(c->tile_accum.as<int>(), tile_cost, g.n_tiles, shift, tail_per_sm * c->n_sm,
+                                       c->tile_order.as<int>(), st);
+  if (e != cudaSuccess) return e;
+  gs_count_launch();
+  g.order = c->tile_order.as<int>();
+  c->order_on = true;
+  return cudaSuccess;
 }
 
 static int render_forward_impl(gs_ctx* c, const float* pos, const float* rgb, const float* opa, const float* quat,
@@ -282,6 +303,7 @@
   GS_CUDA_TRY(c->tile_accum.reserve((size_t)(g.n_tiles + 1) * 4, st));
   GS_CUDA_TRY(c->tile_neff.reserve((size_t)g.n_tiles * 4, st));
   GS_CUDA_TRY(c->tile_neff_b.reserve((size_t)g.n_tiles * 4, st));
+  GS_CUDA_TRY(c->tile_order.reserve((size_t)g.n_tiles * 4, st));
   GS_CUDA_TRY(c->counters.reserve(64, st));
   if (c->iota_n < N) {
     GS_CUDA_TRY(c->iota.reserve(N * 4 + 4, st));
@@ -413,6 +435,7 @@
   if (m > 0) gs_count_launch();
   GsCrop crop{(g.wp - g.width) / 2, (g.hp - g.height) / 2, g.width, g.height};
   gs_mark(c, 5, st);
+  GS_CUDA_TRY(build_tile_order(c, g, nullptr, kFwdOrderShift, kFwdTailPerSm, st));
   if (blend_d == 3) {
     GS_CUDA_TRY(gs_launch_blend_fwd(c->pA.as<float4>(), c->pB.as<float2>(), c->pC.as<float4>(),
                                     gather ? c->rec.as<GsRec>() : nullptr, c->vals_out.as<uint32_t>(),
@@ -511,10 +534,12 @@
   GsCrop crop{(c->geom.wp - c->geom.width) / 2, (c->geom.hp - c->geom.height) / 2, c->geom.width, c->geom.height};
   gs_mark(c, 7, st);
   if (c->m > 0) {
+    GsFrameGeom g = c->geom;
+    GS_CUDA_TRY(build_tile_order(c, g, c->tile_neff.as<int>(), kBwdOrderShift, kBwdTailPerSm, st));
     if (blend_d == 3) {
       GS_CUDA_TRY(gs_launch_blend_bwd(c->pA.as<float4>(), c->pB.as<float2>(), c->pC.as<float4>(),
                                       c->gather ? c->rec.as<GsRec>() : nullptr, c->vals_out.as<uint32_t>(),
-                                      c->offsets_g.as<uint32_t>(), c->tile_accum.as<int>(), c->geom, image, grad_image,
+                                      c->offsets_g.as<uint32_t>(), c->tile_accum.as<int>(), g, image, grad_image,
                                       c->grad_inst.as<float>(),
                                       grad_is_final, crop, c->row_epoch.as<uint32_t>(), c->epoch,
                                       c->tile_neff_b.as<int>(), st, aux, grad_aux));
@@ -524,7 +549,7 @@
       GS_CUDA_TRY(gs_launch_blend_sh_bwd(c->pA.as<float4>(), c->pB.as<float2>(), c->pC.as<float>(),
                                          c->gather ? c->rec.as<GsRec>() : nullptr, rgb, c->vals_out.as<uint32_t>(),
                                          c->offsets_g.as<uint32_t>(), d,
-                                         c->tile_accum.as<int>(), c->geom, rays, image, grad_image,
+                                         c->tile_accum.as<int>(), g, rays, image, grad_image,
                                          c->grad_inst.as<float>(), grad_is_final, crop,
                                          c->row_epoch.as<uint32_t>(), c->epoch, c->tile_neff_b.as<int>(), st, aux,
                                          grad_aux));
@@ -730,6 +755,17 @@
   if (!c->have_forward) return gs_set_error_msg(GS_ERR_NO_FORWARD, "gs_frame_tile_consumed: no forward on this ctx");
   GS_CUDA_TRY(cudaMemcpyAsync(tile_consumed, c->tile_neff.p, sizeof(int) * (size_t)c->geom.n_tiles,
                               cudaMemcpyDeviceToDevice, (cudaStream_t)stream));
+  return 0;
+}
+
+extern "C" int gs_frame_tile_order(gs_ctx* c, int* order, gs_stream_t stream) {
+  if (!c || !order) return gs_set_error_msg(GS_ERR_INVALID_ARG, "gs_frame_tile_order: null argument");
+  if (!c->have_forward) return gs_set_error_msg(GS_ERR_NO_FORWARD, "gs_frame_tile_order: no forward on this ctx");
+  cudaStream_t st = (cudaStream_t)stream;
+  if (c->order_on)
+    GS_CUDA_TRY(cudaMemcpyAsync(order, c->tile_order.p, sizeof(int) * (size_t)c->geom.n_tiles, cudaMemcpyDeviceToDevice, st));
+  else
+    GS_CUDA_TRY(gs_launch_iota(reinterpret_cast<uint32_t*>(order), c->geom.n_tiles, st));
   return 0;
 }
 
diff --git a/include/gs_b200.h b/include/gs_b200.h
--- a/include/gs_b200.h
+++ b/include/gs_b200.h
@@ -152,6 +152,8 @@
 
 int gs_frame_tile_consumed(gs_ctx* ctx, int* tile_consumed, gs_stream_t stream);
 
+int gs_frame_tile_order(gs_ctx* ctx, int* order, gs_stream_t stream);
+
 int gs_render_forward_backward_host(gs_ctx* ctx, const float* pos, const float* rgb, const float* opa,
                                     const float* quat, const float* scale, int n, int d,
                                     int scale_activation, const gs_camera* cam_host,
```
